# edervishaj/GANMF

Hardware: AMD Instinct MI355X
Metric: GANMF training steps/sec (higher is better)
Workload: dtype f32

## Files before the change

ganmf_amd/csrc/gemm_bf16k.hpp:

```cpp
#pragma once
#include "gemm_bf16s.hpp"

namespace ganmf {

typedef float f32x4k __attribute__((ext_vector_type(4)));

struct SplitItemK {
  const float* zp;
  const float* ptr;
  long long inc;
  long long second;
  int aux, dst;
  int dst1 = 0;
  bool km;
  __device__ inline void init(bool km_, const float* __restrict__ base, int ld_, int r0, int rlimit, int kbeg, const float* zero, int w,
                              const int* __restrict__ gather = nullptr) {
    km = km_;
    const int ld = ld_;
    zp = zero + (w & 255) * 8;
    if (!km) {
      using S = SplitStage<64, 64, false>;
      const int row = w / S::CH, c8 = w % S::CH;
      const bool ok = (r0 + row) < rlimit;
      const int src_row = (ok && gather) ? gather[r0 + row] : r0 + row;
      ptr = ok ? base + (size_t)src_row * ld + kbeg + 8 * c8 : zp;
      inc = ok ? 64 : 0;
      second = 4;
      aux = 0;
      dst = row * 32 + 4 * (c8 ^ S::swz(row));
      dst1 = 0;
    } else {
      using S = SplitStage<64, 64, true>;
      const int kp = w / S::RQ, rq = w % S::RQ;
      const bool ok = (r0 + 4 * rq) < ld;
      ptr = ok ? base + (size_t)(kbeg + 2 * kp) * ld + r0 + 4 * rq : zp;
      inc = ok ? (long long)64 * ld : 0;
      second = ok ? ld : 0;
      aux = 2 * kp;
      dst = (2 * kp) * S::KROW + 4 * ((rq >> 1) ^ S::swzk(2 * kp)) + 2 * (rq & 1);
      dst1 = (2 * kp + 1) * S::KROW + 4 * ((rq >> 1) ^ S::swzk(2 * kp + 1)) + 2 * (rq & 1) - dst;
    }
  }
  __device__ inline void addresses(int kleft, const float*& s0, const float*& s1) {
    const float* const z = zp;
    const float* a0 = ptr;
    const float* a1 = ptr + second;
    const int k0 = aux;
    ptr += inc;
    if (kleft < 64 && km) {
      asm volatile("; partial last K-tile");
      a0 = k0 < kleft ? a0 : z;
      a1 = k0 + 1 < kleft ? a1 : z;
    }
    s0 = a0; s1 = a1;
  }
  template <int NPIECE, bool F16>
  __device__ inline void split(const f32x4k (&v)[2], u32x4 (&pc)[3], const int tok, const float scale) const {
    const f32x4k a = v[0], b = v[1];
    if constexpr (NPIECE == 3) {
      unsigned h, m, l;
      split_bf16x3_tok(a.x, a.y, h, m, l, tok); pc[0][0] = h; pc[1][0] = m; pc[2][0] = l;
      split_bf16x3_tok(a.z, a.w, h, m, l, tok); pc[0][1] = h; pc[1][1] = m; pc[2][1] = l;
      split_bf16x3_tok(b.x, b.y, h, m, l, tok); pc[0][2] = h; pc[1][2] = m; pc[2][2] = l;
      split_bf16x3_tok(b.z, b.w, h, m, l, tok); pc[0][3] = h; pc[1][3] = m; pc[2][3] = l;
    } else if constexpr (F16) {
      const float sc = __uint_as_float(__float_as_uint(scale) | (unsigned)tok);
      pc[0][0] = cvt_pk_f16(a.x * sc, a.y * sc); pc[0][1] = cvt_pk_f16(a.z * sc, a.w * sc);
      pc[0][2] = cvt_pk_f16(b.x * sc, b.y * sc); pc[0][3] = cvt_pk_f16(b.z * sc, b.w * sc);
    } else {
      pc[0][0] = cvt_pk_bf16_tok(a.x, a.y, tok); pc[0][1] = cvt_pk_bf16_tok(a.z, a.w, tok);
      pc[0][2] = cvt_pk_bf16_tok(b.x, b.y, tok); pc[0][3] = cvt_pk_bf16_tok(b.z, b.w, tok);
    }
  }
};

constexpr int BF16K_OPER = 3 * (64 * 64 / 2) * 2;
template <int NPIECE> constexpr int bf16k_oper() { return NPIECE * (64 * 64 / 2) * 2; }
template <int NPIECE> constexpr int bf16k_smem_dw() { return 2 * bf16k_oper<NPIECE>() > 4 * 64 * 64 ? 2 * bf16k_oper<NPIECE>() : 4 * 64 * 64; }
static_assert(bf16k_oper<3>() == BF16K_OPER && bf16k_smem_dw<3>() == 2 * BF16K_OPER && bf16k_smem_dw<1>() == 4 * 64 * 64, "plane buffers");
template <int NPIECE> constexpr int bf16k_pd() { return 2; }

__device__ __forceinline__ int bf16k_wait_vm(int n, const f32x4k& v0, const f32x4k& v1) {
  int tok;
#define GANMF_BF16K_WAIT(N) asm volatile("s_waitcnt vmcnt(" #N ")\n\ts_mov_b32 %0, 0" : "=s"(tok) : "v"(v0), "v"(v1))
  if (n >= 8) { if (n >= 9) GANMF_BF16K_WAIT(9); else GANMF_BF16K_WAIT(8); }
  else if (n >= 4) { if (n >= 6) { if (n >= 7) GANMF_BF16K_WAIT(7); else GANMF_BF16K_WAIT(6); } else { if (n >= 5) GANMF_BF16K_WAIT(5); else GANMF_BF16K_WAIT(4); } }
  else { if (n >= 2) { if (n >= 3) GANMF_BF16K_WAIT(3); else GANMF_BF16K_WAIT(2); } else { if (n >= 1) GANMF_BF16K_WAIT(1); else GANMF_BF16K_WAIT(0); } }
#undef GANMF_BF16K_WAIT
  return tok;
}

template <bool AKM, bool BKM, int NPIECE, bool F16, int EXTRA, class Entry>
__device__ __forceinline__ void bf16k_mainloop(const GemmP& p, const int tm, const int tn, const int sp, const int bz, float* __restrict__ smem,
                                               f32x16& acc_out, Entry&& at_entry) {
  static_assert(NPIECE == 3 || NPIECE == 1, "pieces per operand");
  static_assert(!F16 || NPIECE == 1, "fp16 pieces only in the single-piece mode");
  static_assert(2 * (bf16k_pd<NPIECE>() - 1) + EXTRA <= 9, "bf16k_wait_vm covers 0 .. 9");
  constexpr int BM = 64, BN = 64, BK = 64, PD = bf16k_pd<NPIECE>();
  const float sa = (F16 && p.a_scale != 0.f) ? p.a_scale : 1.f, sb = (F16 && p.b_scale != 0.f) ? p.b_scale : 1.f;
  using FA = SplitStage<64, 64, AKM>;
  using FB = SplitStage<64, 64, BKM>;
  const unsigned lds0 = lds_addr(smem);
  const int tid = threadIdx.x;
  const int lane = tid & 63;
  const int wave = __builtin_amdgcn_readfirstlane(tid >> 6);
  const int kg = wave >> 2;
  const int wr = (wave >> 1) & 1, wc = wave & 1;
  const int li = lane & 31, lh = lane >> 5;
  const bool stage_a = wave < 8;
  const int m0 = tm * BM, n0 = tn * BN;
  const int kbeg = sp * p.k_per_split;
  const int kend = min(p.K, kbeg + p.k_per_split);
  const int nt = (kend - kbeg + BK - 1) / BK;

  f32x16 acc, accl;
#pragma unroll
  for (int r = 0; r < 16; ++r) { acc[r] = 0.f; accl[r] = 0.f; }

  SplitItemK it;
  if (stage_a) it.init(AKM, p.A + (size_t)bz * p.a_batch_stride, p.lda, m0, p.M, kbeg, p.zero_page, tid,
                       (AKM || !p.a_gather) ? nullptr : p.a_gather + (size_t)bz * p.a_gather_batch);
  else it.init(BKM, p.B, p.ldb, n0, p.N, kbeg, p.zero_page, tid - 512);
  constexpr int OPER = bf16k_oper<NPIECE>();
  unsigned my_planes[2], my_planes1[2], frag_a[2], frag_b[2];
#pragma unroll
  for (int b = 0; b < 2; ++b) {
    my_planes[b] = lds_base<NPIECE == 3>(lds0 + 4u * (unsigned)(b * OPER + (stage_a ? 0 : NPIECE * FA::PLANE) + it.dst));
    my_planes1[b] = lds_base<NPIECE == 3>(my_planes[b] + 4u * (unsigned)it.dst1);
    frag_a[b] = lds_base<NPIECE == 3>(lds0 + 4u * (unsigned)(b * OPER) + FA::frag_off(wr * 32, kg, li, lh));
    frag_b[b] = lds_base<NPIECE == 3>(lds0 + 4u * (unsigned)(b * OPER + NPIECE * FA::PLANE) + FB::frag_off(wc * 32, kg, li, lh));
  }
  const float my_scale = stage_a ? sa : sb;

  f32x4k rg[PD][2];
#pragma unroll
  for (int s = 0; s < PD; ++s) { rg[s][0] = f32x4k{0.f, 0.f, 0.f, 0.f}; rg[s][1] = f32x4k{0.f, 0.f, 0.f, 0.f}; }
  int kleft = kend - kbeg;
  auto load_tile = [&](auto ss) {
    constexpr int s = decltype(ss)::value;
    const float *s0, *s1;
    it.addresses(kleft, s0, s1);
    f32x4k l0, l1;
    asm volatile("global_load_dwordx4 %0, %1, off" : "=v"(l0) : "v"(s0) : "memory");
    asm volatile("global_load_dwordx4 %0, %1, off" : "=v"(l1) : "v"(s1) : "memory");
    rg[s][0] = l0; rg[s][1] = l1;
    kleft -= BK;
  };
  auto store_tile = [&](auto ss, auto bb, int nwait) {
    constexpr int s = decltype(ss)::value;
    constexpr int b = decltype(bb)::value;
    const f32x4k v[2] = {rg[s][0], rg[s][1]};
    const int tok = bf16k_wait_vm(nwait, v[0], v[1]);
    u32x4 pc[3];
#ifdef GANMF_PERSIST_DIAG_BUILD
    if ((p.diag & 32) && stage_a) {
      pc[0] = __builtin_bit_cast(u32x4, v[0]); pc[1] = __builtin_bit_cast(u32x4, v[1]); pc[2] = pc[0];
      pc[0][0] += (unsigned)tok;
    } else
#endif
    it.template split<NPIECE, F16>(v, pc, tok, my_scale);
    if (it.km) {
      typedef unsigned u32x2 __attribute__((ext_vector_type(2)));
#pragma unroll
      for (int q = 0; q < NPIECE; ++q) {
        lds_write<u32x2>(my_planes[b] + 4u * (unsigned)(q * FA::PLANE), u32x2{pc[q][0], pc[q][1]});
        lds_write<u32x2>(my_planes1[b] + 4u * (unsigned)(q * FA::PLANE), u32x2{pc[q][2], pc[q][3]});
      }
    } else {
#pragma unroll
      for (int q = 0; q < NPIECE; ++q) lds_write<u32x4>(my_planes[b] + 4u * (unsigned)(q * FA::PLANE), pc[q]);
    }
  };
  static_for<0, PD>([&](auto ss) { if (decltype(ss)::value < nt) load_tile(ss); });
  store_tile(std::integral_constant<int, 0>{}, std::integral_constant<int, 0>{}, 2 * (min(nt, PD) - 1));
  if constexpr (PD == 4) asm volatile("s_waitcnt vmcnt(0)" :: "v"(rg[0][0]), "v"(rg[0][1]), "v"(rg[1][0]), "v"(rg[1][1]), "v"(rg[2][0]), "v"(rg[2][1]), "v"(rg[3][0]), "v"(rg[3][1]));
  else asm volatile("s_waitcnt vmcnt(0)" :: "v"(rg[0][0]), "v"(rg[0][1]), "v"(rg[1][0]), "v"(rg[1][1]));
  static_assert(PD == 4 || PD == 2, "the wait above names every prefetch register");
  at_entry();
  __syncthreads();
#ifdef GANMF_PERSIST_DIAG_BUILD
  if (p.stamps && tid == 0) p.stamps[(size_t)blockIdx.x * 4 + 1] = __builtin_amdgcn_s_memrealtime();
#endif

  auto step = [&](auto ss, int t) {
    constexpr int s = decltype(ss)::value, s1 = (s + 1) % PD;
    constexpr int b = s & 1;
    u32x4 pa[3], pb[3];
#pragma unroll
    for (int q = 0; q < NPIECE; ++q) pa[q] = FA::frag_at(frag_a[b] + 4u * (unsigned)(q * FA::PLANE));
#pragma unroll
    for (int q = 0; q < NPIECE; ++q) pb[q] = FB::frag_at(frag_b[b] + 4u * (unsigned)(q * FB::PLANE));
#ifdef GANMF_PERSIST_DIAG_BUILD
    if (p.diag & 16) { if (t + PD < nt) kleft -= BK; } else
#endif
    if (t + PD < nt) load_tile(ss);
    constexpr int ta[6] = {1, 0, 2, 1, 0, 0}, tb[6] = {1, 2, 0, 0, 1, 0};
#ifdef GANMF_PERSIST_DIAG_BUILD
    if (!(p.diag & 4))
#endif
    {
      if constexpr (NPIECE == 3) {
#pragma unroll
        for (int t6 = 0; t6 < 6; ++t6) {
          if (t6 < 5)
            accl = __builtin_amdgcn_mfma_f32_32x32x16_bf16(__builtin_bit_cast(bf16x8, pa[ta[t6]]), __builtin_bit_cast(bf16x8, pb[tb[t6]]), accl, 0, 0, 0);
          else
            acc = __builtin_amdgcn_mfma_f32_32x32x16_bf16(__builtin_bit_cast(bf16x8, pa[ta[t6]]), __builtin_bit_cast(bf16x8, pb[tb[t6]]), acc, 0, 0, 0);
        }
      } else if constexpr (F16) {
        acc = __builtin_amdgcn_mfma_f32_32x32x16_f16(__builtin_bit_cast(f16x8, pa[0]), __builtin_bit_cast(f16x8, pb[0]), acc, 0, 0, 0);
      } else {
        acc = __builtin_amdgcn_mfma_f32_32x32x16_bf16(__builtin_bit_cast(bf16x8, pa[0]), __builtin_bit_cast(bf16x8, pb[0]), acc, 0, 0, 0);
      }
    }
#ifdef GANMF_PERSIST_DIAG_BUILD
    if (!(p.diag & 2))
#endif
    if (t + 1 < nt) store_tile(std::integral_constant<int, s1>{}, std::integral_constant<int, (s1 & 1)>{}, 2 * (min(t + PD, nt - 1) - (t + 1)) + (t + 1 < PD ? EXTRA : 0));
    __syncthreads();
  };
  for (int t = 0; t < nt; t += PD)
    static_for<0, PD>([&](auto ss) { if (t + decltype(ss)::value < nt) step(ss, t + decltype(ss)::value); });

  if constexpr (NPIECE == 3) acc += accl;
  if constexpr (F16) {
    if (sa != 1.f || sb != 1.f) acc *= 1.f / (sa * sb);
  }
  acc_out = acc;
}

template <bool AKM, bool BKM, int NPIECE = 3, bool F16 = false>
__device__ __forceinline__ void gemm_bf16k_body(const GemmP& p, const int bid, const int nblk, float* __restrict__ smem) {
  int tm, tn, sp, bz;
  tile_coords(p, bid, nblk, tm, tn, sp, bz);
  f32x16 acc[1][1];
#ifdef GANMF_PERSIST_DIAG_BUILD
  if (p.stamps && threadIdx.x == 0) p.stamps[(size_t)blockIdx.x * 4 + 0] = __builtin_amdgcn_s_memrealtime();
#endif
  bf16k_mainloop<AKM, BKM, NPIECE, F16, 0>(p, tm, tn, sp, bz, smem, acc[0][0], [] {});
#ifdef GANMF_PERSIST_DIAG_BUILD
  if (p.stamps && threadIdx.x == 0) p.stamps[(size_t)blockIdx.x * 4 + 2] = __builtin_amdgcn_s_memrealtime();
#endif
  static_assert(4 * 64 * 64 <= bf16k_smem_dw<NPIECE>(), "the workgroup's LDS must hold the four staged partial tiles");
  gemm_epilogue<64, 64, 1, 1, 4, AKM && BKM>(p, acc, smem, TileCoord{tm, tn, sp, bz, tm * 64, tn * 64});
#ifdef GANMF_PERSIST_DIAG_BUILD
  if (p.stamps) { asm volatile("s_waitcnt vmcnt(0)" ::: "memory"); __builtin_amdgcn_s_barrier(); if (threadIdx.x == 0) p.stamps[(size_t)blockIdx.x * 4 + 3] = __builtin_amdgcn_s_memrealtime(); }
#endif
}

template <bool AKM, bool BKM, int NPIECE = 3, bool F16 = false>
__global__ __launch_bounds__(1024) void gemm_bf16k_mfma(const GemmP p) {
  __shared__ __attribute__((aligned(16))) float smem[bf16k_smem_dw<NPIECE>()];
  gemm_bf16k_body<AKM, BKM, NPIECE, F16>(p, (int)blockIdx.x, (int)gridDim.x, smem);
}

template <int NPIECE, bool F16>
inline hipError_t gemm_bf16k_launch(hipStream_t st, const GemmP& p0, bool akm, bool bkm) {
  GemmP p = p0;
#ifdef GANMF_PERSIST_DIAG_BUILD
  if (getenv("GANMF_BF16K_DIAG")) p.diag = atoi(getenv("GANMF_BF16K_DIAG"));
#endif
  const int grid = p.tiles_m * p.tiles_n * p.nsplit * p.nbatch;
  if (grid <= 0) return hipSuccess;
#ifdef GANMF_PERSIST_DIAG_BUILD
  const bool stamping = gemm_stamps_on() && gemm_stamps_begin(p, grid, st);
  struct Report { const GemmP& p; int grid; hipStream_t st; bool akm, bkm, on; ~Report() { if (on) gemm_stamps_report(p, grid, st, akm, bkm, NPIECE == 3 ? "gemm_bf16k_mfma (split-bf16, 16 waves)" : "gemm_bf16k_mfma (one piece)"); } } report{p, grid, st, akm, bkm, stamping};
#endif
  {
    if (!akm && !bkm) GANMF_LAUNCH((gemm_bf16k_mfma<false, false, NPIECE, F16>), dim3(grid), dim3(1024), 0, st, p);
    else if (!akm && bkm) GANMF_LAUNCH((gemm_bf16k_mfma<false, true, NPIECE, F16>), dim3(grid), dim3(1024), 0, st, p);
    else if (akm && bkm) GANMF_LAUNCH((gemm_bf16k_mfma<true, true, NPIECE, F16>), dim3(grid), dim3(1024), 0, st, p);
    else return hipErrorInvalidValue;
  }
  return hipGetLastError();
}

}
```

ganmf_amd/csrc/gemm_bf16w.hpp:

```cpp
#pragma once
#include "gemm_bf16k.hpp"

namespace ganmf {

constexpr int BF16W_BM = 64, BF16W_BN = 32, BF16W_BK = 128, BF16W_KG = 8, BF16W_PD = 2;
constexpr int BF16W_PA = BF16W_BM * BF16W_BK / 2;
constexpr int BF16W_PB = BF16W_BN * BF16W_BK / 2;
constexpr int BF16W_OPER = 3 * (BF16W_PA + BF16W_PB);

__device__ __forceinline__ int bf16w_wait_vm(int n, const f32x4k& v0, const f32x4k& v1, const f32x4k& v2) {
  int tok;
#define GANMF_BF16W_WAIT(N) asm volatile("s_waitcnt vmcnt(" #N ")\n\ts_mov_b32 %0, 0" : "=s"(tok) : "v"(v0), "v"(v1), "v"(v2))
  if (n >= 9) GANMF_BF16W_WAIT(9);
  else if (n >= 6) GANMF_BF16W_WAIT(6);
  else if (n >= 3) GANMF_BF16W_WAIT(3);
  else GANMF_BF16W_WAIT(0);
#undef GANMF_BF16W_WAIT
  return tok;
}

template <int NPIECE> constexpr int bf16w_oper() { return NPIECE * (BF16W_PA + BF16W_PB); }
template <int NPIECE> constexpr int bf16w_smem_dw() {
  return 2 * bf16w_oper<NPIECE>() > BF16W_KG * BF16W_BM * BF16W_BN ? 2 * bf16w_oper<NPIECE>() : BF16W_KG * BF16W_BM * BF16W_BN;
}
static_assert(bf16w_oper<3>() == BF16W_OPER && bf16w_smem_dw<3>() == 2 * BF16W_OPER && bf16w_smem_dw<1>() == BF16W_KG * BF16W_BM * BF16W_BN, "plane buffers");

template <bool BKM, int NPIECE = 3, bool F16 = false>
__device__ __forceinline__ void bf16w_mainloop(const GemmP& p, const int tm, const int tn, const int bz, float* __restrict__ smem, f32x16& acc_out) {
  static_assert(NPIECE == 3 || NPIECE == 1, "pieces per operand");
  static_assert(!F16 || NPIECE == 1, "fp16 pieces only in the single-piece mode");
  constexpr int BM = BF16W_BM, BN = BF16W_BN, BK = BF16W_BK, PD = BF16W_PD, PA = BF16W_PA, PB = BF16W_PB, OPER = bf16w_oper<NPIECE>();
  const float sa = (F16 && p.a_scale != 0.f) ? p.a_scale : 1.f, sb = (F16 && p.b_scale != 0.f) ? p.b_scale : 1.f;
  typedef unsigned u32x2 __attribute__((ext_vector_type(2)));
  const unsigned lds0 = lds_addr(smem);
  const int tid = threadIdx.x;
  const int lane = tid & 63;
  const int wave = __builtin_amdgcn_readfirstlane(tid >> 6);
  const int kg = wave >> 1, wr = wave & 1;
  const int li = lane & 31, lh = lane >> 5;
  const int m0 = tm * BM, n0 = tn * BN;
  const int nt = (p.K + BK - 1) / BK;

  f32x16 acc, accl;
#pragma unroll
  for (int r = 0; r < 16; ++r) { acc[r] = 0.f; accl[r] = 0.f; }

  const int row = tid >> 5, kq = tid & 31;
  const int arow = tid >> 4, c8 = tid & 15;
  const float* const zp = p.zero_page + (tid & 255) * 8;
  const bool ok0 = m0 + arow < p.M, ok2 = n0 + row < p.N;
  const float* s0 = ok0 ? p.A + (size_t)bz * p.a_batch_stride + (size_t)(m0 + arow) * p.lda + 8 * c8 : zp;
  const int kb = tid >> 3, nq = tid & 7;
  const bool okn = n0 + 4 * nq < p.ldb;
  const float* s2 = !BKM ? (ok2 ? p.B + (size_t)(n0 + row) * p.ldb + 4 * kq : zp) : (okn ? p.B + (size_t)kb * p.ldb + n0 + 4 * nq : zp);
  const int i0 = ok0 ? BK : 0;
  const long long i2 = !BKM ? (ok2 ? BK : 0) : (okn ? (long long)BK * p.ldb : 0);
  int kleft = p.K;
  const bool in_a = (nt - 1) * BK + 8 * c8 < p.lda, in_b = (nt - 1) * BK + 4 * kq < p.ldb;
  const int dsta = arow * (BK / 2) + ((c8 ^ (arow & 15)) << 2);
  const int dst = row * (BK / 2) + ((((kq >> 1) ^ (row & 15))) << 2) + ((kq & 1) << 1);
  const int dstb = !BKM ? dst : kb * (BN / 2) + 2 * nq;

  f32x4k rg[PD][3];
#pragma unroll
  for (int s = 0; s < PD; ++s) { rg[s][0] = f32x4k{0.f, 0.f, 0.f, 0.f}; rg[s][1] = rg[s][0]; rg[s][2] = rg[s][0]; }
  int tload = 0;
  auto load_tile = [&](auto ss) {
    constexpr int s = decltype(ss)::value;
    const float* const zp_ = zp;
    const float* const s0_ = s0;
    const float* const s2_ = s2;
    const int kleft_ = kleft;
    const float* a0 = s0_;
    const float* b0 = s2_;
    if (tload >= nt - 1) {
      asm volatile("; last K-tile");
      const bool last = tload == nt - 1, past = tload >= nt;
      a0 = ((last && !in_a) || past) ? zp_ : s0_;
      b0 = !BKM ? (((last && !in_b) || past) ? zp_ : s2_) : ((kb < kleft_) ? s2_ : zp_);
    }
    kleft -= BK;
    f32x4k l0, l1, l2;
    asm volatile("global_load_dwordx4 %0, %1, off" : "=v"(l0) : "v"(a0) : "memory");
    asm volatile("global_load_dwordx4 %0, %1, off offset:16" : "=v"(l1) : "v"(a0) : "memory");
    asm volatile("global_load_dwordx4 %0, %1, off" : "=v"(l2) : "v"(b0) : "memory");
    rg[s][0] = l0; rg[s][1] = l1; rg[s][2] = l2;
    s0 += i0; s2 += i2;
    ++tload;
  };
  unsigned st_a[2], st_b[2];
#pragma unroll
  for (int b = 0; b < 2; ++b) {
    st_a[b] = lds_base<NPIECE == 3>(lds0 + 4u * (unsigned)(b * OPER + dsta));
    st_b[b] = lds_base<NPIECE == 3>(lds0 + 4u * (unsigned)(b * OPER + NPIECE * PA + dstb));
  }
  auto store_tile = [&](auto ss, auto bb, int nwait) {
    constexpr int s = decltype(ss)::value;
    constexpr int b = decltype(bb)::value;
    const f32x4k v0 = rg[s][0], v1 = rg[s][1], v2 = rg[s][2];
    const int tok = bf16w_wait_vm(nwait, v0, v1, v2);
    const unsigned o = st_a[b], ob = st_b[b];
    if constexpr (NPIECE == 3) {
      unsigned h0, m0_, l0, h1, m1, l1, h2, m2, l2, h3, m3, l3;
      split_bf16x3_tok(v0.x, v0.y, h0, m0_, l0, tok); split_bf16x3_tok(v0.z, v0.w, h1, m1, l1, tok);
      split_bf16x3_tok(v1.x, v1.y, h2, m2, l2, tok); split_bf16x3_tok(v1.z, v1.w, h3, m3, l3, tok);
      lds_write<u32x4>(o, u32x4{h0, h1, h2, h3});
      lds_write<u32x4>(o + 4u * PA, u32x4{m0_, m1, m2, m3});
      lds_write<u32x4>(o + 8u * PA, u32x4{l0, l1, l2, l3});
      split_bf16x3_tok(v2.x, v2.y, h0, m0_, l0, tok); split_bf16x3_tok(v2.z, v2.w, h1, m1, l1, tok);
      lds_write<u32x2>(ob, u32x2{h0, h1});
      lds_write<u32x2>(ob + 4u * PB, u32x2{m0_, m1});
      lds_write<u32x2>(ob + 8u * PB, u32x2{l0, l1});
    } else if constexpr (F16) {
      const float ca = __uint_as_float(__float_as_uint(sa) | (unsigned)tok), cb = __uint_as_float(__float_as_uint(sb) | (unsigned)tok);
      lds_write<u32x4>(o, u32x4{cvt_pk_f16(v0.x * ca, v0.y * ca), cvt_pk_f16(v0.z * ca, v0.w * ca),
                                cvt_pk_f16(v1.x * ca, v1.y * ca), cvt_pk_f16(v1.z * ca, v1.w * ca)});
      lds_write<u32x2>(ob, u32x2{cvt_pk_f16(v2.x * cb, v2.y * cb), cvt_pk_f16(v2.z * cb, v2.w * cb)});
    } else {
      lds_write<u32x4>(o, u32x4{cvt_pk_bf16_tok(v0.x, v0.y, tok), cvt_pk_bf16_tok(v0.z, v0.w, tok),
                                cvt_pk_bf16_tok(v1.x, v1.y, tok), cvt_pk_bf16_tok(v1.z, v1.w, tok)});
      lds_write<u32x2>(ob, u32x2{cvt_pk_bf16_tok(v2.x, v2.y, tok), cvt_pk_bf16_tok(v2.z, v2.w, tok)});
    }
  };
  static_for<0, PD>([&](auto ss) { load_tile(ss); });
  store_tile(std::integral_constant<int, 0>{}, std::integral_constant<int, 0>{}, 3 * (PD - 1));
  asm volatile("s_waitcnt vmcnt(0)" :: "v"(rg[0][0]), "v"(rg[0][1]), "v"(rg[0][2]), "v"(rg[1][0]), "v"(rg[1][1]), "v"(rg[1][2]));
  static_assert(PD == 2, "the wait above names every prefetch register");
  __syncthreads();
#ifdef GANMF_PERSIST_DIAG_BUILD
  if (p.stamps && tid == 0) p.stamps[(size_t)blockIdx.x * 4 + 1] = __builtin_amdgcn_s_memrealtime();
#endif

  unsigned fa[2], fb[2];
#pragma unroll
  for (int b = 0; b < 2; ++b) {
    fa[b] = lds_base<NPIECE == 3>(lds0 + 4u * (unsigned)(b * OPER + (wr * 32 + li) * (BK / 2) + (((2 * kg + lh) ^ (li & 15)) << 2)));
    if constexpr (!BKM) fb[b] = lds_base<NPIECE == 3>(lds0 + 4u * (unsigned)(b * OPER + NPIECE * PA + li * (BK / 2) + (((2 * kg + lh) ^ (li & 15)) << 2)));
    else fb[b] = 0u;
  }
  unsigned fbt[2];
#pragma unroll
  for (int b = 0; b < 2; ++b)
    fbt[b] = !BKM ? 0u : lds_base<NPIECE == 3>(lds0 + 4u * (unsigned)(b * OPER + NPIECE * PA) + (unsigned)(((16 * kg + 8 * lh + ((li & 15) >> 2)) * (BN / 2) * 4) + 32 * (li >> 4) + 8 * (li & 3)));
  auto step = [&](auto ss, int t) {
    constexpr int s = decltype(ss)::value, s1_ = (s + 1) % PD;
    constexpr int b = s & 1;
    u32x4 pa[3], pb[3];
#pragma unroll
    for (int q = 0; q < NPIECE; ++q) pa[q] = lds_read<u32x4>(fa[b] + 4u * (unsigned)(q * PA));
    if constexpr (!BKM) {
#pragma unroll
      for (int q = 0; q < NPIECE; ++q) pb[q] = lds_read<u32x4>(fb[b] + 4u * (unsigned)(q * PB));
    } else {
#if defined(__HIP_DEVICE_COMPILE__)
      typedef __attribute__((address_space(3))) s16x4* lds_s16x4_p;
      const unsigned base = fbt[b];
#pragma unroll
      for (int q = 0; q < NPIECE; ++q) {
        const s16x4 lo = __builtin_amdgcn_ds_read_tr16_b64_v4i16((lds_s16x4_p)(base + q * PB * 4));
        const s16x4 hi = __builtin_amdgcn_ds_read_tr16_b64_v4i16((lds_s16x4_p)(base + q * PB * 4 + 4 * (BN / 2) * 4));
        pb[q] = __builtin_bit_cast(u32x4, __builtin_shufflevector(lo, hi, 0, 1, 2, 3, 4, 5, 6, 7));
      }
#else
      (void)fbt;
#pragma unroll
      for (int q = 0; q < NPIECE; ++q) pb[q] = u32x4{0u, 0u, 0u, 0u};
#endif
    }
    if (t + PD < nt) load_tile(ss);
    constexpr int ta[6] = {1, 0, 2, 1, 0, 0}, tb[6] = {1, 2, 0, 0, 1, 0};
    if constexpr (NPIECE == 3) {
#pragma unroll
      for (int t6 = 0; t6 < 6; ++t6) {
        if (t6 < 5)
          accl = __builtin_amdgcn_mfma_f32_32x32x16_bf16(__builtin_bit_cast(bf16x8, pa[ta[t6]]), __builtin_bit_cast(bf16x8, pb[tb[t6]]), accl, 0, 0, 0);
        else
          acc = __builtin_amdgcn_mfma_f32_32x32x16_bf16(__builtin_bit_cast(bf16x8, pa[ta[t6]]), __builtin_bit_cast(bf16x8, pb[tb[t6]]), acc, 0, 0, 0);
      }
    } else if constexpr (F16) {
      acc = __builtin_amdgcn_mfma_f32_32x32x16_f16(__builtin_bit_cast(f16x8, pa[0]), __builtin_bit_cast(f16x8, pb[0]), acc, 0, 0, 0);
    } else {
      acc = __builtin_amdgcn_mfma_f32_32x32x16_bf16(__builtin_bit_cast(bf16x8, pa[0]), __builtin_bit_cast(bf16x8, pb[0]), acc, 0, 0, 0);
    }
    if (t + 1 < nt) store_tile(std::integral_constant<int, s1_>{}, std::integral_constant<int, (s1_ & 1)>{}, 3 * (min(t + PD, nt - 1) - (t + 1)));
    __syncthreads();
  };
  for (int t = 0; t < nt; t += PD)
    static_for<0, PD>([&](auto ss) { if (t + decltype(ss)::value < nt) step(ss, t + decltype(ss)::value); });

  if constexpr (NPIECE == 3) acc += accl;
  if constexpr (F16) {
    if (sa != 1.f || sb != 1.f) acc *= 1.f / (sa * sb);
  }
  acc_out = acc;
}

template <bool BKM, int NPIECE = 3, bool F16 = false>
__device__ __forceinline__ void gemm_bf16w_body(const GemmP& p, const int bid, const int nblk, float* __restrict__ smem) {
  int tm, tn, sp, bz;
  tile_coords(p, bid, nblk, tm, tn, sp, bz);
  f32x16 acc[1][1];
#ifdef GANMF_PERSIST_DIAG_BUILD
  if (p.stamps && threadIdx.x == 0) p.stamps[(size_t)blockIdx.x * 4 + 0] = __builtin_amdgcn_s_memrealtime();
#endif
  bf16w_mainloop<BKM, NPIECE, F16>(p, tm, tn, bz, smem, acc[0][0]);
#ifdef GANMF_PERSIST_DIAG_BUILD
  if (p.stamps && threadIdx.x == 0) p.stamps[(size_t)blockIdx.x * 4 + 2] = __builtin_amdgcn_s_memrealtime();
#endif
  static_assert(BF16W_KG * BF16W_BM * BF16W_BN <= bf16w_smem_dw<NPIECE>(), "the workgroup's LDS must hold the staged partial tiles");
  const int lane = threadIdx.x & 63, wave = __builtin_amdgcn_readfirstlane(threadIdx.x >> 6);
  const int kg = wave >> 1, wr = wave & 1, li = lane & 31, lh = lane >> 5;
  float* ct = smem + kg * (BF16W_BM * BF16W_BN);
#pragma unroll
  for (int r = 0; r < 16; ++r) ct[(wr * 32 + (r & 3) + 8 * (r >> 2) + 4 * lh) * BF16W_BN + li] = acc[0][0][r];
  gemm_epilogue<BF16W_BM, BF16W_BN, 1, 1, 4, false, BF16W_KG, true>(p, acc, smem, TileCoord{tm, tn, sp, bz, tm * BF16W_BM, tn * BF16W_BN});
#ifdef GANMF_PERSIST_DIAG_BUILD
  if (p.stamps) { asm volatile("s_waitcnt vmcnt(0)" ::: "memory"); __builtin_amdgcn_s_barrier(); if (threadIdx.x == 0) p.stamps[(size_t)blockIdx.x * 4 + 3] = __builtin_amdgcn_s_memrealtime(); }
#endif
}

template <bool BKM, int NPIECE = 3, bool F16 = false>
__global__ __launch_bounds__(1024) void gemm_bf16w_mfma(const GemmP p) {
  __shared__ __attribute__((aligned(16))) float smem[bf16w_smem_dw<NPIECE>()];
  gemm_bf16w_body<BKM, NPIECE, F16>(p, (int)blockIdx.x, (int)gridDim.x, smem);
}

inline bool gemm_bf16w_eligible(const GemmP& p, bool akm, bool bkm) {
  return !akm && std::max(p.nbatch, 1) == 1 && !p.a_gather && !p.a_planes && !p.b_planes && !p.epi.csr_indptr && !p.epi.sp_rows &&
         p.epi.kind != EPI_ADAM && p.K >= 1 && (p.lda % 64) == 0 && (p.ldb % 64) == 0;
}
constexpr int BF16W_ZERO_PAGE_FLOATS = 255 * 8 + 8;
static_assert(BF16W_ZERO_PAGE_FLOATS <= 2048 + 64, "gemm_bf16w reads past the library's zero page");

inline bool plan_bf16w(GemmPlan& pl, const GemmP& g, bool akm, bool bkm, bool force) {
  if (!gemm_bf16w_eligible(g, akm, bkm)) return false;
  const int tm = (g.M + BF16W_BM - 1) / BF16W_BM, tn = (g.N + BF16W_BN - 1) / BF16W_BN;
  const bool lp = pl.mode == MFMA_F16 || pl.mode == MFMA_BF16;
  const double k64 = lp ? 0.45 : 0.94, k32 = lp ? 0.75 : 1.3;
  if (!force) {
    if (!((pl.mode == MFMA_BF16X3 || lp) && pl.tile == 64 && pl.kg == 4 && pl.nsplit >= 2 && !pl.persist && !pl.skinny && !pl.skinny_n)) return false;
    if ((long long)tm * tn > GEMM_CUS) return false;
    const double est64 = 5.3 + k64 * ((pl.kps + 63) / 64) + 4.7, est32 = 4.4 + k32 * ((g.K + BF16W_BK - 1) / BF16W_BK);
    if (est32 > est64 - 0.5) return false;
  }
  const bool wants_sq = pl.sq_count > 0 || g.epi.sq_partials != nullptr;
  pl.est_us = 4.4 + k32 * ((g.K + BF16W_BK - 1) / BF16W_BK);
  pl.wide32 = 1; pl.skinny = 0; pl.skinny_n = 0; pl.persist = 0;
  if (!lp) pl.mode = MFMA_BF16X3;
  pl.tile = 64; pl.kg = BF16W_KG; pl.ring = 2; pl.bk = BF16W_BK;
  pl.tiles_m = tm; pl.tiles_n = tn; pl.nsplit = 1; pl.kps = g.K;
  pl.sq_count = wants_sq ? tm * tn : 0;
  return true;
}

inline hipError_t gemm_dispatch_bf16w(hipStream_t st, const GemmP& p0, bool bkm, int mode) {
  GemmP p = p0;
  const int grid = p.tiles_m * p.tiles_n * std::max(p.nbatch, 1);
  if (grid <= 0) return hipSuccess;
#ifdef GANMF_PERSIST_DIAG_BUILD
  const bool stamping = gemm_stamps_on() && gemm_stamps_begin(p, grid, st);
  struct Report { const GemmP& p; int grid; hipStream_t st; bool bkm, on; ~Report() { if (on) gemm_stamps_report(p, grid, st, false, bkm, "gemm_bf16w_mfma (64 x 32 tiles, 128-deep K-tiles)"); } } report{p, grid, st, bkm, stamping};
#endif
  if (p.nsplit != 1 || p.tiles_m != (p.M + BF16W_BM - 1) / BF16W_BM || p.tiles_n != (p.N + BF16W_BN - 1) / BF16W_BN) return hipErrorInvalidValue;
  if (!p.zero_page || (p.lda % 64) != 0 || (p.ldb % 64) != 0) return hipErrorInvalidValue;
  if (mode == MFMA_F16) {
    if (bkm) GANMF_LAUNCH((gemm_bf16w_mfma<true, 1, true>), dim3(grid), dim3(1024), 0, st, p);
    else GANMF_LAUNCH((gemm_bf16w_mfma<false, 1, true>), dim3(grid), dim3(1024), 0, st, p);
  } else if (mode == MFMA_BF16) {
    if (bkm) GANMF_LAUNCH((gemm_bf16w_mfma<true, 1, false>), dim3(grid), dim3(1024), 0, st, p);
    else GANMF_LAUNCH((gemm_bf16w_mfma<false, 1, false>), dim3(grid), dim3(1024), 0, st, p);
  } else {
    if (bkm) GANMF_LAUNCH(gemm_bf16w_mfma<true>, dim3(grid), dim3(1024), 0, st, p);
    else GANMF_LAUNCH(gemm_bf16w_mfma<false>, dim3(grid), dim3(1024), 0, st, p);
  }
  return hipGetLastError();
}

}
```

ganmf_amd/csrc/gemm_f32.hpp:

```cpp
#pragma once
#include <hip/hip_runtime.h>
#include <hip/hip_ext.h>

#include <algorithm>
#include <cstdio>
#include <cstdlib>
#include <vector>
#include <cmath>
#include <type_traits>

#include "adam_touch.hpp"

namespace ganmf {

struct LaunchProf { hipEvent_t start = nullptr, stop = nullptr; int count = 0; };
inline LaunchProf& launch_prof() { static thread_local LaunchProf lp; return lp; }
inline hipEvent_t& launch_stop_event() { static thread_local hipEvent_t ev = nullptr; return ev; }
inline long long& launch_count() { static thread_local long long n = 0; return n; }

template <class F, class... Args>
inline void launch_kernel(F kernel, const dim3& grid, const dim3& block, unsigned shmem, hipStream_t st, Args... args) {
  LaunchProf& lp = launch_prof();
  hipEvent_t& stop = launch_stop_event();
  ++launch_count();
  if (lp.start && lp.count++ == 0) hipExtLaunchKernelGGL(kernel, grid, block, shmem, st, lp.start, lp.stop, 0, args...);
  else if (stop) { hipExtLaunchKernelGGL(kernel, grid, block, shmem, st, nullptr, stop, 0, args...); stop = nullptr; }
  else hipLaunchKernelGGL(kernel, grid, block, shmem, st, args...);
}
#define GANMF_LAUNCH(...) ::ganmf::launch_kernel(__VA_ARGS__)

typedef float f32x16 __attribute__((ext_vector_type(16)));
typedef float f32x2 __attribute__((ext_vector_type(2)));
typedef unsigned u32x4 __attribute__((ext_vector_type(4)));
typedef __bf16 bf16x8 __attribute__((ext_vector_type(8)));

enum MfmaMode : int { MFMA_AUTO = -1, MFMA_F32 = 0, MFMA_BF16 = 1, MFMA_F16 = 2, MFMA_BF16X3 = 3 };

typedef __bf16 bf16x2 __attribute__((ext_vector_type(2)));

__device__ inline unsigned cvt_pk_bf16(float x0, float x1) {
  unsigned r;
  asm("v_cvt_pk_bf16_f32 %0, %1, %2" : "=v"(r) : "v"(x0), "v"(x1));
  return r;
}

__device__ inline unsigned cvt_pk_bf16_tok(float x0, float x1, int tok) {
  unsigned r;
  asm("v_cvt_pk_bf16_f32 %0, %1, %2 ; behind wait token %3" : "=v"(r) : "v"(x0), "v"(x1), "s"(tok));
  return r;
}
__device__ inline void split_bf16x3_tok(float x0, float x1, unsigned& hi, unsigned& mid, unsigned& lo, int tok) {
  hi = cvt_pk_bf16_tok(x0, x1, tok);
  float r0 = x0 - __uint_as_float(hi << 16), r1 = x1 - __uint_as_float(hi & 0xffff0000u);
  mid = cvt_pk_bf16(r0, r1);
  r0 -= __uint_as_float(mid << 16);
  r1 -= __uint_as_float(mid & 0xffff0000u);
  lo = cvt_pk_bf16(r0, r1);
}

__device__ inline unsigned cvt_pk_f16(float x0, float x1) {
  unsigned r;
  x0 = __builtin_amdgcn_fmed3f(x0, -65504.f, 65504.f);
  x1 = __builtin_amdgcn_fmed3f(x1, -65504.f, 65504.f);
  asm("v_cvt_pk_f16_f32 %0, %1, %2" : "=v"(r) : "v"(x0), "v"(x1));
  return r;
}

__device__ inline void split_bf16x3(float x0, float x1, unsigned& hi, unsigned& mid, unsigned& lo) {
  hi = cvt_pk_bf16(x0, x1);
  float r0 = x0 - __uint_as_float(hi << 16), r1 = x1 - __uint_as_float(hi & 0xffff0000u);
  mid = cvt_pk_bf16(r0, r1);
  r0 -= __uint_as_float(mid << 16);
  r1 -= __uint_as_float(mid & 0xffff0000u);
  lo = cvt_pk_bf16(r0, r1);
}

template <int I, int N, class F>
__device__ inline void static_for(F&& f) {
  if constexpr (I < N) {
    f(std::integral_constant<int, I>{});
    static_for<I + 1, N>(f);
  }
}

constexpr int LD_ALIGN = 64;

enum GemmEpi : int {
  EPI_STORE = 0,
  EPI_SUB_AUX_SQ = 1,
  EPI_SUB_SCALED_AUX = 2,
  EPI_ROWSCALE = 3,
  EPI_G_DE = 4,
  EPI_ACT = 5,
  EPI_MUL_ACTGRAD = 6,
  EPI_ADAM = 7,
  EPI_GRAM_STATS = 8,
};

constexpr float ADAM_B1 = 0.9f, ADAM_B2 = 0.999f, ADAM_EPS = 1e-8f;

enum ActKind : int { ACT_LINEAR = 0, ACT_TANH = 1, ACT_RELU = 2, ACT_SIGMOID = 3 };

__device__ inline float act_apply(int act, float z) {
  switch (act) {
    case ACT_TANH: return tanhf(z);
    case ACT_RELU: return fmaxf(z, 0.f);
    case ACT_SIGMOID: return 1.f / (1.f + expf(-z));
    default: return z;
  }
}
__device__ inline float act_grad_out(int act, float a) {
  switch (act) {
    case ACT_TANH: return 1.f - a * a;
    case ACT_RELU: return a > 0.f ? 1.f : 0.f;
    case ACT_SIGMOID: return a * (1.f - a);
    default: return 1.f;
  }
}

struct EpiD {
  int kind;
  const float* aux;
  int ldaux;
  long long aux_batch_stride;
  const float* rowscale;
  float c;
  const float* er;
  const float* ef;
  float cfm;
  float* sq_partials;
  int sq_stride;
  int sq_m_half;
  int act;
  const float* r1_u;
  const float* r1_w;
  int r1_ld;
  float* adam_theta;
  float* adam_theta_out;
  float* adam_m;
  float* adam_v;
  const float* adam_alpha;
  float adam_reg;
  const long long* csr_indptr;
  const int* csr_indices;
  const float* csr_data;
  const int* csr_rows;
  const float* sp_rows;
  int sp_ld, sp_bias_row, sp_bias_parts;
  unsigned short* planes;
  long long plane_stride;
  double* gram_partials;
};

__device__ inline float4 csr_quad(const EpiD& e, int m, int col) {
  const int r = e.csr_rows[m];
  long long lo = e.csr_indptr[r];
  const long long en = e.csr_indptr[r + 1];
  long long hi = en;
  while (lo < hi) {
    const long long mid = (lo + hi) >> 1;
    if (e.csr_indices[mid] < col) lo = mid + 1; else hi = mid;
  }
  float4 x = make_float4(0.f, 0.f, 0.f, 0.f);
  for (long long j = lo; j < en; ++j) {
    const int c = e.csr_indices[j] - col;
    if (c > 3) break;
    const float v = e.csr_data[j];
    if (c == 0) x.x = v; else if (c == 1) x.y = v; else if (c == 2) x.z = v; else x.w = v;
  }
  return x;
}

__device__ inline float4 sparse_rows_quad(const EpiD& e, int row, int col) {
  if (row > e.sp_bias_row) return make_float4(0.f, 0.f, 0.f, 0.f);
  float4 s = *reinterpret_cast<const float4*>(e.sp_rows + (size_t)row * e.sp_ld + col);
  if (row == e.sp_bias_row)
    for (int q = 1; q < e.sp_bias_parts; ++q) {
      const float4 d = *reinterpret_cast<const float4*>(e.sp_rows + (size_t)(row + q) * e.sp_ld + col);
      s.x += d.x; s.y += d.y; s.z += d.z; s.w += d.w;
    }
  return s;
}

__device__ __forceinline__ float adam_step(float x, float ma, float v) {
#ifdef GANMF_ADAM_IEEE
  return x - ma / (sqrtf(v) + ADAM_EPS);
#else
  return __builtin_fmaf(-ma, __builtin_amdgcn_rcpf(__builtin_amdgcn_sqrtf(v) + ADAM_EPS), x);
#endif
}

__device__ inline void adam_update(float g, float alpha, float reg, float& th, float& m, float& v, float& sq) {
  const float x = th;
  sq += x * x;
  const float gr = g + reg * x;
  m += (gr - m) * (1.f - ADAM_B1);
  v += (gr * gr - v) * (1.f - ADAM_B2);
  th = adam_step(x, m * alpha, v);
}

__device__ inline float epi_apply(const EpiD& e, float v, int row, int col, int ldc, const float* __restrict__ aux,
                                  float& sq) {
  switch (e.kind) {
    case EPI_SUB_AUX_SQ:
      if (aux) v -= aux[(size_t)row * e.ldaux + col];
      sq += v * v;
      break;
    case EPI_SUB_SCALED_AUX:
      v -= e.c * aux[(size_t)row * e.ldaux + col];
      break;
    case EPI_ROWSCALE:
      v *= e.rowscale[row];
      break;
    case EPI_G_DE: {
      const float d = e.ef[(size_t)row * ldc + col] - e.er[(size_t)row * ldc + col];
      v = e.c * v + e.cfm * d;
      sq += d * d;
      break;
    }
    case EPI_ACT:
      if (e.r1_u) v += e.r1_u[(size_t)row * e.r1_ld] * e.r1_w[col];
      v = act_apply(e.act, v);
      break;
    case EPI_MUL_ACTGRAD:
      v *= act_grad_out(e.act, aux[(size_t)row * e.ldaux + col]);
      break;
    default: break;
  }
  return v;
}

struct GemmP {
  const float* A;
  const float* B;
  float* C;
  int lda, ldb, ldc;
  int M, N, K;
  const float* zero_page;
  int nsplit;
  int k_per_split;
  long long c_split_stride;
  int nbatch;
  long long a_batch_stride, c_batch_stride;
  EpiD epi;
  int tiles_m, tiles_n;
  unsigned* counters;
  float* Cf;
  long long cf_batch_stride;
  int c_pad_writable;
  const int* a_gather;
  int a_gather_batch;
  float a_scale, b_scale;
  int xb_m, xb_n, xb_band;
  int diag;
  unsigned long long* stamps;
  const unsigned short* a_planes;
  const unsigned short* b_planes;
  long long a_pstride, b_pstride;
  int n_fastest;
  int adam_touch;
};

#define GANMF_WAIT_VMCNT(N) asm volatile("s_waitcnt vmcnt(%0)" ::"n"(N) : "memory")

template <int BM, int BN, int NTHR>
struct AdamTouchRegs {
  static constexpr int NR = (adam_touch_slots(BM, BN) + NTHR - 1) / NTHR;
  float v[NR];
};

template <int BM, int BN, int NTHR>
__device__ __forceinline__ void adam_touch_issue(const GemmP& p, int m0, int n0, int tid, AdamTouchRegs<BM, BN, NTHR>& k) {
#pragma unroll
  for (int j = 0; j < AdamTouchRegs<BM, BN, NTHR>::NR; ++j) {
    k.v[j] = 0.f;
    const AdamTouch t = adam_touch_slot(BM, BN, j * NTHR + tid, m0, n0, p.M, p.N, p.ldc);
    if (t.arr >= 0) {
      const float* __restrict__ b = t.arr == 0 ? p.epi.adam_theta : t.arr == 1 ? p.epi.adam_m : p.epi.adam_v;
      k.v[j] = b[t.off];
    }
  }
}

template <int BM, int BN, int NTHR>
__device__ __forceinline__ void adam_touch_keep(const AdamTouchRegs<BM, BN, NTHR>& k) {
#pragma unroll
  for (int j = 0; j < AdamTouchRegs<BM, BN, NTHR>::NR; ++j) asm volatile("" ::"v"(k.v[j]));
}

template <int R, int BK, bool KM, int NTHR = 256>
struct Stage {
  static constexpr int F4 = R * BK / 4;
  static constexpr int NP = F4 / NTHR;
  static constexpr int SZ = R * BK;
  static constexpr int S = BK / 4;
  static constexpr int RC4 = R / 4;
  static_assert(F4 % NTHR == 0 && NP >= 1, "tile too small for the workgroup");
  static_assert(BK == 32 || BK == 64, "BK must be 32 or 64");

  __device__ static inline int swz(int row) { return (row / (64 / BK)) & (S - 1); }

  const float* zp;
  const float* ptr[NP];
  int aux[NP];

  __device__ inline void init(const float* __restrict__ base, int ld, int r0, int rlimit, int kbeg,
                              const float* zero, int tid, const int* __restrict__ gather = nullptr) {
    zero += (tid & 255) * 4;
    zp = zero;
#pragma unroll
    for (int j = 0; j < NP; ++j) {
      const int pos = j * NTHR + tid;
      if constexpr (!KM) {
        const int row = pos / S, slot = pos % S;
        const int c4 = slot ^ swz(row);
        const bool ok = (r0 + row) < rlimit;
        const int src_row = (ok && gather) ? gather[r0 + row] : r0 + row;
        ptr[j] = ok ? base + (size_t)src_row * ld + kbeg + 4 * c4 : zero;
        aux[j] = ok ? BK : 0;
      } else {
        const int krow = pos / RC4, c4 = pos % RC4;
        const bool ok = (r0 + 4 * c4) < ld;
        ptr[j] = base + (size_t)(kbeg + krow) * ld + r0 + 4 * c4;
        aux[j] = ok ? krow : -1;
      }
    }
  }

  template <int J>
  __device__ inline void issue_piece(float* s, int ld, int kleft, int wave) {
    const float* src;
    if constexpr (!KM) {
      src = kleft > 0 ? ptr[J] : zp;
      ptr[J] += aux[J];
    } else {
      src = (aux[J] >= 0 && aux[J] < kleft) ? ptr[J] : zp;
      ptr[J] += (size_t)BK * ld;
    }
    __builtin_amdgcn_global_load_lds((const __attribute__((address_space(1))) void*)src,
                                     (__attribute__((address_space(3))) void*)(s + (J * NTHR + wave * 64) * 4),
                                     16, 0, 0);
  }
  template <int J>
  __device__ inline void issue_piece_asm(float* s, int ld, int kleft, int wave) {
    const float* src;
    if constexpr (!KM) {
      src = kleft > 0 ? ptr[J] : zp;
      ptr[J] += aux[J];
    } else {
      src = (aux[J] >= 0 && aux[J] < kleft) ? ptr[J] : zp;
      ptr[J] += (size_t)BK * ld;
    }
    const unsigned dst = __builtin_amdgcn_readfirstlane(
        (unsigned)(size_t)(__attribute__((address_space(3))) void*)(s + (J * NTHR + wave * 64) * 4));
    unsigned keep;
    asm volatile("s_mov_b32 %0, m0\n\ts_mov_b32 m0, %2\n\ts_nop 0\n\tglobal_load_lds_dwordx4 %1, off\n\ts_mov_b32 m0, %0"
                 : "=&s"(keep) : "v"(src), "s"(dst) : "memory");
  }
  template <int J0, int J1>
  __device__ inline void issue_range_asm(float* s, int ld, int kleft, int wave) {
    if constexpr (J0 < J1) {
      issue_piece_asm<J0>(s, ld, kleft, wave);
      issue_range_asm<J0 + 1, J1>(s, ld, kleft, wave);
    }
  }
  template <int J0, int J1>
  __device__ inline void issue_range(float* s, int ld, int kleft, int wave) {
    if constexpr (J0 < J1) {
      issue_piece<J0>(s, ld, kleft, wave);
      issue_range<J0 + 1, J1>(s, ld, kleft, wave);
    }
  }
  __device__ inline void issue(float* s, int ld, int kleft, int wave) {
    issue_range<0, NP>(s, ld, kleft, wave);
  }

  __device__ static inline float4 frag(const float* __restrict__ s, int rb, int c, int i, int h) {
    if constexpr (!KM) {
      return *reinterpret_cast<const float4*>(s + (rb + i) * BK + 4 * ((2 * c + h) ^ swz(i)));
    } else {
      const float* q = s + (c * 8 + 4 * h) * R + rb + i;
      return make_float4(q[0], q[R], q[2 * R], q[3 * R]);
    }
  }
};

__device__ inline void tile_coords(const GemmP& p, int bid, int nblk, int& tm, int& tn, int& sp, int& bz) {
  tile_order(TileGrid{p.tiles_m, p.tiles_n, p.nsplit, p.xb_m, p.xb_n, p.xb_band, p.n_fastest}, bid, nblk, tm, tn, sp, bz);
}

#ifndef GANMF_ADAM_HOIST
#define GANMF_ADAM_HOIST 1
#endif

struct TileCoord { int tm, tn, sp, bz, m0, n0; };

__device__ inline void gram_tile_coords(const GemmP& p, int bid, int nblk, int& tm, int& tn);
template <int BM, int BN, int TM, int TN>
__device__ inline void gram_epilogue(const GemmP& p, const f32x16 (&acc)[TM][TN], float* smem, const TileCoord& tc_);
template <int BM, int BN, int TM, int TN>
__device__ inline void rowsq_epilogue(const GemmP& p, const f32x16 (&acc)[TM][TN], float* smem, const TileCoord& tc_);

template <int BM, int BN, int TM, int TN, int KG = 1, bool ADAM_OK = true, int NIMG = KG, bool STAGED = false>
__device__ inline void gemm_epilogue(const GemmP& p, const f32x16 (&acc)[TM][TN], float* smem, const TileCoord& tc_) {
  constexpr int WM = BM / 2, WN = BN / 2;
  constexpr int NTHR = 256 * KG;
  const int tid = threadIdx.x, lane = tid & 63;
  const int wave = __builtin_amdgcn_readfirstlane(tid >> 6);
  const int kg = wave >> 2;
  const int wr = (wave >> 1) & 1, wc = wave & 1;
  const int li = lane & 31, lh = lane >> 5;
  const int tm = tc_.tm, tn = tc_.tn, sp = tc_.sp, bz = tc_.bz, m0 = tc_.m0, n0 = tc_.n0;
  float* __restrict__ ct = smem + kg * (BM * BN);
  const bool deferred = p.nsplit > 1;
  const EpiD& e = p.epi;
  const bool csr0 = e.csr_indptr != nullptr && bz == 0 && e.kind == EPI_SUB_AUX_SQ;
  const float* __restrict__ aux = (e.aux && !csr0) ? e.aux + (size_t)bz * e.aux_batch_stride : nullptr;
  constexpr int C4 = BN / 4, RPP = NTHR / C4 < BM ? NTHR / C4 : BM;
  constexpr bool SPARE = NTHR / C4 > BM;
  static_assert(BM % RPP == 0, "row pass must cover the tile in whole steps");
  static_assert(!SPARE || !ADAM_OK, "the hoisted Adam streams assume every thread owns a row");
  const int tc = tid % C4, tr = tid / C4;
  const int col = n0 + tc * 4;
  float4 auxv = make_float4(0.f, 0.f, 0.f, 0.f);
  bool aux_pre = false;
  if constexpr (BM == RPP) {
    const int row = m0 + tr;
    if (!deferred && aux && (e.kind == EPI_SUB_AUX_SQ || e.kind == EPI_SUB_SCALED_AUX || e.kind == EPI_MUL_ACTGRAD) && row < p.M && col + 3 < p.N &&
        (!SPARE || tr < BM)) {
      auxv = *reinterpret_cast<const float4*>(aux + (size_t)row * e.ldaux + col);
      aux_pre = true;
    }
  }
  if constexpr (!STAGED) {
#pragma unroll
    for (int a = 0; a < TM; ++a)
#pragma unroll
      for (int b = 0; b < TN; ++b)
#pragma unroll
        for (int r = 0; r < 16; ++r)
          ct[(wr * WM + a * 32 + (r & 3) + 8 * (r >> 2) + 4 * lh) * BN + wc * WN + b * 32 + li] = acc[a][b][r];
  }
  __syncthreads();

  float* __restrict__ C = p.C + (size_t)sp * p.c_split_stride + (size_t)bz * p.c_batch_stride;
  const bool sp_add = !(p.nsplit > 1) && e.sp_rows != nullptr;
  float sq = 0.f;
  ct = smem;
  const bool adam = ADAM_OK && !deferred && e.kind == EPI_ADAM;
  const float alpha = adam ? *e.adam_alpha : 0.f;
  float* __restrict__ theta_out = e.adam_theta_out ? e.adam_theta_out : e.adam_theta;
#ifdef GANMF_PERSIST_DIAG_BUILD
  const bool inlaunch = deferred && p.counters != nullptr;
#else
  constexpr bool inlaunch = false;
#endif
  const bool publish = inlaunch;
  typedef unsigned u32x4 __attribute__((ext_vector_type(4)));
  const __amdgpu_buffer_rsrc_t slab_rsrc = __builtin_amdgcn_make_buffer_rsrc((void*)C, (short)0, 0x7fffffff, 0x00020000);
#ifdef GANMF_PERSIST_DIAG_BUILD
  if (adam && (p.diag & 8)) return;
#endif
  if (adam && GANMF_ADAM_HOIST) {
    constexpr int J = BM / RPP, JC = 1;
    static_assert(J % JC == 0, "row steps in whole chunks");
    for (int j0 = 0; j0 < J; j0 += JC) {
      float4 t4[JC], m4[JC], v4[JC];
#pragma unroll
      for (int jj = 0; jj < JC; ++jj) {
        const int row = m0 + tr + (j0 + jj) * RPP;
        if (row < p.M && col + 3 < p.N) {
          const size_t off = (size_t)row * p.ldc + col;
          t4[jj] = *reinterpret_cast<const float4*>(e.adam_theta + off);
          m4[jj] = *reinterpret_cast<const float4*>(e.adam_m + off);
          v4[jj] = *reinterpret_cast<const float4*>(e.adam_v + off);
        }
      }
#pragma unroll
      for (int jj = 0; jj < JC; ++jj) {
        const int row_l = tr + (j0 + jj) * RPP, row = m0 + row_l;
        if (row < p.M && col < p.N) {
          float4 v = *reinterpret_cast<const float4*>(ct + row_l * BN + tc * 4);
#pragma unroll
          for (int g = 1; g < NIMG; ++g) {
            const float4 w = *reinterpret_cast<const float4*>(ct + g * (BM * BN) + row_l * BN + tc * 4);
            v.x += w.x; v.y += w.y; v.z += w.z; v.w += w.w;
          }
          if (sp_add) {
            const float4 x = sparse_rows_quad(e, row, col);
            v.x += x.x; v.y += x.y; v.z += x.z; v.w += x.w;
          }
          const size_t off = (size_t)row * p.ldc + col;
          if (col + 3 < p.N) {
            adam_update(v.x, alpha, e.adam_reg, t4[jj].x, m4[jj].x, v4[jj].x, sq);
            adam_update(v.y, alpha, e.adam_reg, t4[jj].y, m4[jj].y, v4[jj].y, sq);
            adam_update(v.z, alpha, e.adam_reg, t4[jj].z, m4[jj].z, v4[jj].z, sq);
            adam_update(v.w, alpha, e.adam_reg, t4[jj].w, m4[jj].w, v4[jj].w, sq);
            *reinterpret_cast<float4*>(theta_out + off) = t4[jj];
            *reinterpret_cast<float4*>(e.adam_m + off) = m4[jj];
            *reinterpret_cast<float4*>(e.adam_v + off) = v4[jj];
          } else {
            const float o[4] = {v.x, v.y, v.z, v.w};
            for (int q = 0; q < 4 && col + q < p.N; ++q) {
              float th = e.adam_theta[off + q];
              adam_update(o[q], alpha, e.adam_reg, th, e.adam_m[off + q], e.adam_v[off + q], sq);
              theta_out[off + q] = th;
            }
          }
        }
      }
    }
  } else
#pragma unroll 4
  for (int j = 0; j < BM / RPP; ++j) {
    const int row_l = tr + j * RPP, row = m0 + row_l;
    if (row < p.M && col < p.N && (!SPARE || row_l < BM)) {
      float4 v = *reinterpret_cast<const float4*>(ct + row_l * BN + tc * 4);
#pragma unroll
      for (int g = 1; g < NIMG; ++g) {
        const float4 w = *reinterpret_cast<const float4*>(ct + g * (BM * BN) + row_l * BN + tc * 4);
        v.x += w.x; v.y += w.y; v.z += w.z; v.w += w.w;
      }
      if (sp_add) {
        const float4 x = sparse_rows_quad(e, row, col);
        v.x += x.x; v.y += x.y; v.z += x.z; v.w += x.w;
      }
      if (csr0 && !deferred) {
        const float4 x = csr_quad(e, row, col);
        v.x -= x.x; v.y -= x.y; v.z -= x.z; v.w -= x.w;
      }
      float o[4] = {v.x, v.y, v.z, v.w};
      if (adam) {
        const size_t off = (size_t)row * p.ldc + col;
        if (col + 3 < p.N) {
          float4 t4 = *reinterpret_cast<float4*>(e.adam_theta + off);
          float4 m4 = *reinterpret_cast<float4*>(e.adam_m + off);
          float4 v4 = *reinterpret_cast<float4*>(e.adam_v + off);
          adam_update(o[0], alpha, e.adam_reg, t4.x, m4.x, v4.x, sq);
          adam_update(o[1], alpha, e.adam_reg, t4.y, m4.y, v4.y, sq);
          adam_update(o[2], alpha, e.adam_reg, t4.z, m4.z, v4.z, sq);
          adam_update(o[3], alpha, e.adam_reg, t4.w, m4.w, v4.w, sq);
          *reinterpret_cast<float4*>(theta_out + off) = t4;
          *reinterpret_cast<float4*>(e.adam_m + off) = m4;
          *reinterpret_cast<float4*>(e.adam_v + off) = v4;
        } else {
          for (int q = 0; q < 4 && col + q < p.N; ++q) {
            float th = e.adam_theta[off + q];
            adam_update(o[q], alpha, e.adam_reg, th, e.adam_m[off + q], e.adam_v[off + q], sq);
            theta_out[off + q] = th;
          }
        }
        continue;
      }
      if (publish) {
        const int boff = (int)(((size_t)row * p.ldc + col) * sizeof(float));
        if (col + 3 < p.N) {
          u32x4 bits;
          bits[0] = __float_as_uint(o[0]); bits[1] = __float_as_uint(o[1]);
          bits[2] = __float_as_uint(o[2]); bits[3] = __float_as_uint(o[3]);
          __builtin_amdgcn_raw_buffer_store_b128(bits, slab_rsrc, boff, 0, 16 );
        } else {
// ... 625 lines not shown
```

ganmf_amd/csrc/lib/abi_core.inc:

```

int ganmf_abi_version(void) { return GANMF_ABI_VERSION; }
const char* ganmf_last_error(void) { return g_err.c_str(); }

static uint32_t g_crc_tab[8][256];
static std::once_flag g_crc_once;
static void crc_init() {
  for (uint32_t i = 0; i < 256; ++i) {
    uint32_t c = i;
    for (int k = 0; k < 8; ++k) c = (c & 1) ? (c >> 1) ^ 0x82F63B78u : c >> 1;
    g_crc_tab[0][i] = c;
  }
  for (uint32_t i = 0; i < 256; ++i)
    for (int t = 1; t < 8; ++t) g_crc_tab[t][i] = (g_crc_tab[t - 1][i] >> 8) ^ g_crc_tab[0][g_crc_tab[t - 1][i] & 0xff];
}
uint32_t ganmf_crc32c(uint32_t crc, const void* data, uint64_t n) {
  std::call_once(g_crc_once, crc_init);
  const uint8_t* p = static_cast<const uint8_t*>(data);
  uint32_t c = ~crc;
  while (n >= 8) {
    uint64_t w;
    memcpy(&w, p, 8);
    w ^= c;
    c = g_crc_tab[7][w & 0xff] ^ g_crc_tab[6][(w >> 8) & 0xff] ^ g_crc_tab[5][(w >> 16) & 0xff] ^
        g_crc_tab[4][(w >> 24) & 0xff] ^ g_crc_tab[3][(w >> 32) & 0xff] ^ g_crc_tab[2][(w >> 40) & 0xff] ^
        g_crc_tab[1][(w >> 48) & 0xff] ^ g_crc_tab[0][(w >> 56) & 0xff];
    p += 8; n -= 8;
  }
  while (n--) c = (c >> 8) ^ g_crc_tab[0][(c ^ *p++) & 0xff];
  return ~c;
}

int ganmf_device_count(void) {
  int n = 0;
  if (hipGetDeviceCount(&n) != hipSuccess) return 0;
  return n;
}

static int create_impl(const ganmf_cfg* cfg, ganmf_handle* h);

int ganmf_create(const ganmf_cfg* cfg, ganmf_handle** out) {
  if (!cfg || !out) return fail(-1, "ganmf_create: null argument");
  if (cfg->abi_version != GANMF_ABI_VERSION) return fail(-1, "ganmf_create: ABI version %d != %d", cfg->abi_version, GANMF_ABI_VERSION);
  if (cfg->model != GANMF_MODEL_GANMF && cfg->model != GANMF_MODEL_DISGANMF && cfg->model != GANMF_MODEL_MF && cfg->model != GANMF_MODEL_ITEMSIM && cfg->model != GANMF_MODEL_CFGAN && cfg->model != GANMF_MODEL_CAAE) return fail(-1, "ganmf_create: unknown model %d", cfg->model);
  if (cfg->model == GANMF_MODEL_DISGANMF && (cfg->d_layers < 1 || cfg->d_layers > 16 || cfg->d_act < 0 || cfg->d_act > 3))
    return fail(-1, "ganmf_create: DisGANMF needs 1 <= d_layers <= 16 and a known activation");
  if (cfg->model == GANMF_MODEL_CFGAN) {
    if (cfg->d_layers < 1 || cfg->d_layers > 16 || cfg->d_act < 0 || cfg->d_act > 3)
      return fail(-1, "ganmf_create: CFGAN needs 1 <= d_layers <= 16 and a known activation");
    if (cfg->world_size > 1) return fail(-1, "ganmf_create: GANMF_MODEL_CFGAN is single-GPU (world_size %d)", cfg->world_size);
    if (cfg->flags & (GANMF_FLAG_MFMA_BF16 | GANMF_FLAG_MFMA_F16))
      return fail(-1, "ganmf_create: GANMF_MODEL_CFGAN runs the fp32-accurate products only (the bf16 / fp16 MFMA flags are refused)");
    if (cfg->num_items > (1LL << 29)) return fail(-1, "ganmf_create: CFGAN's discriminator input is 2 x num_items wide: dimension too large");
  }
  if (cfg->model == GANMF_MODEL_CAAE) {
    if (cfg->world_size > 1) return fail(-1, "ganmf_create: GANMF_MODEL_CAAE is single-GPU (world_size %d)", cfg->world_size);
    if (cfg->flags & (GANMF_FLAG_MFMA_BF16 | GANMF_FLAG_MFMA_F16))
      return fail(-1, "ganmf_create: GANMF_MODEL_CAAE runs the fp32-accurate products only (the bf16 / fp16 MFMA flags are refused)");
    if (cfg->num_factors > GANMF_CAAE_MAX_FACTORS) return fail(-1, "ganmf_create: GANMF_MODEL_CAAE holds at most %d factors", GANMF_CAAE_MAX_FACTORS);
  }
  if (cfg->num_users < 1 || cfg->num_items < 1 || cfg->num_factors < 1 || cfg->emb_dim < 1 || cfg->batch_size < 1)
    return fail(-1, "ganmf_create: non-positive dimension");
  if (cfg->num_users > (1LL << 30) || cfg->num_items > (1LL << 30)) return fail(-1, "ganmf_create: dimension too large");
  int ndev = 0;
  HIP_TRY(hipGetDeviceCount(&ndev));
  if (ndev < 1) return fail(-2, "ganmf_create: no HIP device (the HIP path is the only path; there is no CPU fallback)");
  if (cfg->device < 0 || cfg->device >= ndev) return fail(-1, "ganmf_create: device %d out of range [0,%d)", cfg->device, ndev);
  HIP_TRY(hipSetDevice(cfg->device));
  ganmf_handle* h = new ganmf_handle();
  const int rc = create_impl(cfg, h);
  if (rc != 0) {
    const std::string msg = g_err;
    ganmf_destroy(h);
    (void)hipGetLastError();
    g_err = msg;
    *out = nullptr;
    return rc;
  }
  *out = h;
  return 0;
}

static int create_impl(const ganmf_cfg* cfg, ganmf_handle* h) {
  h->cfg = *cfg;
  h->dev = cfg->device;
  h->U = (int)cfg->num_users; h->N = (int)cfg->num_items; h->k = cfg->num_factors; h->e = cfg->emb_dim;
  h->B = (int)std::min<int64_t>(cfg->batch_size, cfg->num_users);
  h->ldN = round_up(h->N + 2, LD_ALIGN); h->ldk = round_up(h->k + 1, LD_ALIGN); h->lde = round_up(h->e + 1, LD_ALIGN);
  h->tune.tile = tune_env_int("tile", 0);
  if (h->tune.tile != 0 && h->tune.tile != 64 && h->tune.tile != 128) h->tune.tile = 0;
  h->tune.ring = tune_env_int("ring", 0);
  if (h->tune.ring != 0 && h->tune.ring != 2 && h->tune.ring != 3 && h->tune.ring != 4) h->tune.ring = 0;
  h->tune.nsplit = std::max(0, tune_env_int("nsplit", 0));
  h->tune.mode = env_mfma_mode((cfg->flags & GANMF_FLAG_MFMA_F16) ? MFMA_F16 : (cfg->flags & GANMF_FLAG_MFMA_BF16) ? MFMA_BF16 : (cfg->flags & GANMF_FLAG_MFMA_F32) ? MFMA_F32 : MFMA_DEFAULT);
  h->tune.persist = tune_env_int("persist", -1);
  if (h->tune.persist > 1) h->tune.persist = experiment_int("GANMF_PERSIST_WAVES", 1);
  h->tune.kg = tune_env_int("kg", 0);
  h->tune.tile_order = tune_env_int("tile_order", 0);
  h->pass_stage = tune_env_int("pass_stage", 1) != 0;
  h->skinny = tune_env_int("skinny", 1) != 0;
  h->skinny_n = h->skinny && tune_env_int("skinny_n", 1) != 0;
  h->lazy_rows = tune_env_int("lazy_rows", 1) != 0;
#ifdef GANMF_ASM_PREFETCH_UNTESTED
  constexpr int kAsmPrefetchDefault = 0;
#else
  constexpr int kAsmPrefetchDefault = 1;
#endif
  h->bf16w = tune_env_int("bf16w", kAsmPrefetchDefault);
  h->wgrad_xb = std::max(0, tune_env_int("wgrad_xb", 16));
  h->wd_lane = std::max(0, tune_env_int("wd_lane", 0));
  h->g_rows_staged = std::max(0, std::min(2, tune_env_int("g_rows_staged", 1)));
  h->pair_kg = tune_env_int("pair_kg", 4) == 1 ? 1 : 4;
  h->wgrad_seam = tune_env_int("wgrad_seam", 0);
  h->adam_touch = tune_env_int("adam_touch", 1) != 0 ? 1 : 0;
  h->gram_arith = tune_env_int("gram", 1) == 0 ? 0 : 1;
  HIP_TRY(hipMalloc((void**)&h->seam_cnt, 2 * sizeof(unsigned long long)));
  HIP_TRY(hipMemset(h->seam_cnt, 0, 2 * sizeof(unsigned long long)));
  if (h->tune.kg != 0 && h->tune.kg != 1 && h->tune.kg != 2 && h->tune.kg != 4) h->tune.kg = 0;
  h->debug_plan = env_int("GANMF_DEBUG_PLAN", 0) != 0;
  h->fused_mode = experiment_int("GANMF_FUSED_X3", 1) ? MFMA_BF16X3 : MFMA_F32;
  h->fused_tile = experiment_int("GANMF_FUSED_TILE", 64) == 128 ? 128 : 64;
  h->fused_bk = experiment_int("GANMF_FUSED_BK", 32);
  HIP_TRY(hipStreamCreateWithFlags(&h->st, hipStreamNonBlocking));
  HIP_TRY(hipStreamCreateWithFlags(&h->st2, hipStreamNonBlocking));
  const bool lane_fence = env_int("GANMF_LANE_EVENT_FENCE", cfg->world_size > 1 ? 1 : 0) != 0;
  const unsigned lane_flags = lane_fence ? hipEventDisableTiming : (hipEventDisableTiming | hipEventDisableSystemFence);
  HIP_TRY(hipEventCreateWithFlags(&h->ev_fork, lane_flags));
  HIP_TRY(hipEventCreateWithFlags(&h->ev_join, lane_flags));
  HIP_TRY(hipEventCreateWithFlags(&h->ev_mid, lane_flags));
  HIP_TRY(hipEventCreateWithFlags(&h->ev_we, lane_flags));
  HIP_TRY(hipEventCreateWithFlags(&h->ev_wd, lane_flags));
  h->fuse_adam = experiment_int("GANMF_FUSE_ADAM", 1) != 0;
  const int multi_env = env_int("GANMF_MULTI", 127);
  h->multi = multi_env & 31;
  h->defer_gub = (multi_env & 32) != 0;
  h->dis_fuse_hidden = (multi_env & 64) != 0;
  h->x3kg = env_int("GANMF_X3KG", kAsmPrefetchDefault ? 7 : 0);
  h->dcoef_spread = experiment_int("GANMF_DCOEF_SPREAD", 1) != 0;
  h->pair_ring = experiment_int("GANMF_PAIR_RING", 2) == 3 ? 3 : 2;
  h->inkernel_reduce = experiment_int("GANMF_INKERNEL_REDUCE", 0) != 0;
  h->inlaunch_max = experiment_int("GANMF_INLAUNCH_MAX", 4);
  h->inlaunch_tags = experiment_int("GANMF_INLAUNCH_TAGS", 0);
  h->force_coll = env_int("GANMF_FORCE_COLLECTIVES", 0) != 0;
  h->score_presplit = env_int("GANMF_SCORE_PRESPLIT", 1) != 0;
  h->fork_attach = experiment_int("GANMF_FORK_ATTACH", 1) != 0;
  h->adam_nfast = experiment_int("GANMF_ADAM_NFAST", 3);
  h->red_elems = experiment_int("GANMF_RED_ELEMS", 0);
  h->merge_decode = experiment_int("GANMF_MERGE_DECODE", 1) != 0;
  TRY(dalloc((float**)&h->counters, COUNTER_CAP));
  TRY(dalloc((float**)&h->counters2, COUNTER_CAP));
  const int U = h->U, N = h->N, k = h->k, e = h->e, B = h->B;
  const bool dis = cfg->model == GANMF_MODEL_DISGANMF;
  const bool sim = cfg->model == GANMF_MODEL_ITEMSIM;
  const bool cfgan = cfg->model == GANMF_MODEL_CFGAN;
  const bool caae = cfg->model == GANMF_MODEL_CAAE;
  const bool mf = cfg->model == GANMF_MODEL_MF || sim || caae;
  if (caae && low_precision(h)) return fail(-1, "ganmf_create: GANMF_MODEL_CAAE runs the fp32-accurate products only (GANMF_MFMA asks for bf16 / f16)");
  const int world = std::max(1, (int)cfg->world_size);
  if (!sim && !cfgan) {
    TRY(alloc_tensor(h->Ue, U, k, false, 1));
    TRY(alloc_tensor(h->V, N, k, true, world));
    TRY(dalloc(&h->V_alt, h->V.cap));
  }
  if (mf) {
  } else if (cfgan) {
    TRY(cfgan_create(h));
  } else if (!dis) {
    TRY(alloc_tensor(h->We, N + 1, e, false, world));
    TRY(alloc_tensor(h->Wd, e + 1, N, false, world, h->ldN));
    h->gD_elems = h->We.cap + h->Wd.cap;
    TRY(dalloc(&h->gD, h->gD_elems));
    h->We.g = h->gD;
    h->Wd.g = h->We.g + h->We.cap;
  } else {
    h->L = cfg->d_layers; h->act = cfg->d_act;
    h->Wl.resize(h->L);
    h->dis_fused.assign(h->L, 0);
    h->dis_regn.assign(h->L, ADAM_GRID);
    h->gD_elems = 0;
    for (int l = 0; l < h->L; ++l) {
      TRY(alloc_tensor(h->Wl[l], l == 0 ? N + 2 : e + 1, e, false, world));
      h->gD_elems += h->Wl[l].cap;
    }
    TRY(alloc_tensor(h->Wo, 1, e + 1, false, world));
    h->gD_elems += h->Wo.cap;
    TRY(dalloc(&h->gD, h->gD_elems));
    float* gp = h->gD;
    for (int l = 0; l < h->L; ++l) { h->Wl[l].g = gp; gp += h->Wl[l].cap; }
    h->Wo.g = gp;
  }
  TRY(dalloc(&h->zero_page, 2048 + 64));
  TRY(dalloc((float**)&h->perm, (size_t)3 * U));
  h->pos = h->perm + U;
  h->pos_step = h->perm + 2 * (size_t)U;
  if (!mf && !cfgan) {
    TRY(dalloc(&h->XF, (size_t)2 * B * h->ldN));
    h->XF_own = h->XF;
    TRY(dalloc(&h->Ub, (size_t)B * h->ldk));
    h->Ub_own = h->Ub;
    TRY(dalloc(&h->dF, (size_t)B * h->ldN));
    TRY(dalloc(&h->gUb, (size_t)B * h->ldk));
    h->gUb_own = h->gUb;
    std::vector<float> ones((size_t)2 * B, 1.0f);
    HIP_TRY(hipMemcpy2D(h->XF + N, (size_t)h->ldN * 4, ones.data(), 4, 4, (size_t)2 * B, hipMemcpyHostToDevice));
    if (!dis) {
      TRY(dalloc(&h->E, (size_t)2 * B * h->lde));
      TRY(dalloc(&h->Es, (size_t)2 * B * h->lde));
      TRY(dalloc(&h->Dl, (size_t)2 * B * h->ldN));
      TRY(dalloc(&h->dE, (size_t)2 * B * h->lde));
      HIP_TRY(hipMemcpy2D(h->E + e, (size_t)h->lde * 4, ones.data(), 4, 4, (size_t)2 * B, hipMemcpyHostToDevice));
#ifdef GANMF_PERSIST_DIAG_BUILD
      h->wgrad_stream = env_int("GANMF_WGRAD_STREAM", 0) != 0;
#endif
      if (h->wgrad_stream) {
        h->ps_N = (long long)2 * B * h->ldN; h->ps_e = (long long)2 * B * h->lde;
        TRY(dalloc((float**)&h->pl_XF, (size_t)(3 * h->ps_N + 1) / 2));
        TRY(dalloc((float**)&h->pl_Dl, (size_t)(3 * h->ps_N + 1) / 2));
        TRY(dalloc((float**)&h->pl_Es, (size_t)(3 * h->ps_e + 1) / 2));
        TRY(dalloc((float**)&h->pl_dE, (size_t)(3 * h->ps_e + 1) / 2));
        TRY(dalloc(&h->wgs_dump, 2048 + 64));
      }
    } else {
      h->Al.resize(h->L, nullptr);
      for (int l = 0; l < h->L; ++l) {
        TRY(dalloc(&h->Al[l], (size_t)2 * B * h->lde));
        HIP_TRY(hipMemcpy2D(h->Al[l] + e, (size_t)h->lde * 4, ones.data(), 4, 4, (size_t)2 * B, hipMemcpyHostToDevice));
      }
      TRY(dalloc(&h->dz0, (size_t)2 * B * h->lde));
      TRY(dalloc(&h->dz1, (size_t)2 * B * h->lde));
      TRY(dalloc(&h->dlogit, (size_t)2 * B));
    }
  }
  TRY(dalloc(&h->rs, (size_t)2 * B));
  h->tab_cap = (int)(U / std::max(B, 1)) + 2;
  TRY(dalloc(&h->scal, (size_t)S_TAB + 4 * (size_t)h->tab_cap));
  TRY(dalloc(&h->sqp, (size_t)2 * std::max(GEMM_RED_GRID, ((B + 63) / 64) * ((N + 63) / 64)) + 16));
  {
    auto t64 = [](int a, int b) { return ((a + 63) / 64) * ((b + 63) / 64); };
    h->reg_cap = std::max({ADAM_GRID, (int)GEMM_RED_GRID, t64(N + 2, e), t64(e + 1, N), t64(N, k), t64(B, N), t64(B, e)});
    h->reg_cap = round_up(h->reg_cap + (e + 63) / 64, 64);
    h->dis_cap = round_up(std::max({h->reg_cap, B, dis_dz_top_blocks(e) + 1}), 64);
  }
  const float pw[4] = {ADAM_B1, ADAM_B2, ADAM_B1, ADAM_B2};
  HIP_TRY(hipMemcpy(h->scal, pw, sizeof pw, hipMemcpyHostToDevice));
  HIP_TRY(hipDeviceSynchronize());
  return 0;
}

int ganmf_destroy(ganmf_handle* h) {
  if (!h) return 0;
  hipSetDevice(h->dev);
  if (h->st) hipStreamSynchronize(h->st);
  if (h->has_comm && !h->local && !h->comm_aborted) ncclCommDestroy(h->comm);
  if (h->local) {
    std::lock_guard<std::mutex> lk(h->local->mu);
    h->local->failed = true;
    h->local->cv.notify_all();
  }
  free_tensor(h->We, false); free_tensor(h->Wd, false); hipFree(h->zero_page); hipFree(h->Es); hipFree(h->seam_cnt);
  for (auto& t : h->Wl) free_tensor(t, false);
  free_tensor(h->Wo, false);
  for (float* a : h->Al) hipFree(a);
  hipFree(h->dz0); hipFree(h->dz1); hipFree(h->dlogit);
  free_tensor(h->Ue, false); free_tensor(h->V, true); hipFree(h->V_alt);
  hipFree(h->gD); hipFree(h->indptr); hipFree(h->indices); hipFree(h->data); hipFree(h->perm);
  hipFree(h->csc_colptr); hipFree(h->csc_rowidx); hipFree(h->csc_val); hipFree(h->sp_rows);
  if (h->stage_i) hipHostFree(h->stage_i);
  if (h->stage_f) hipHostFree(h->stage_f);
  hipFree(h->test_indptr); hipFree(h->test_indices); hipFree(h->test_gain); hipFree(h->eval_buf);
  hipFree(h->cand_indptr); hipFree(h->cand_indices);
  hipFree(h->test_rating); hipFree(h->eval_w); hipFree(h->eval_rmse); hipFree(h->eval_counts); hipFree(h->eval_grp);
  hipFree(h->XF_own); hipFree(h->XF_pass); hipFree(h->Ub_pass); hipFree(h->Ub_own); hipFree(h->Ub_sched); hipFree(h->lazy_tab);
  for (auto& ch : h->lazy_chunks) hipFree(ch.first);
  if (h->lazy_stage) hipHostFree(h->lazy_stage);
  h->lazy_chunks.clear();
  hipFree(h->E); hipFree(h->Dl); hipFree(h->dE); hipFree(h->dF); hipFree(h->gUb_own);
  hipFree(h->slab); hipFree(h->rs); hipFree(h->scal); hipFree(h->sqp);
  hipFree(h->seen_indptr); hipFree(h->seen_indices); hipFree(h->item_mask); hipFree(h->topk_items); hipFree(h->topk_vals); hipFree(h->sc_ids);
  hipFree(h->colbuf); hipFree(h->parts_all); hipFree(h->sc_rows); hipFree(h->sc_out); hipFree(h->sc_pa); hipFree(h->sc_pb);
  hipFree(h->sim_mat); hipFree(h->sim_pool); hipFree(h->sim_part); hipFree(h->sim_zero);
  hipFree(h->rank_mask); hipFree(h->div_mat);
  for (AlsSide& s : h->als) { hipFree(s.indptr); hipFree(s.indices); hipFree(s.conf); }
  hipFree(h->als_G); hipFree(h->als_bad);
  hipFree(h->knn_indptr); hipFree(h->knn_nbr); hipFree(h->knn_val); hipFree(h->knn_dense);
  hipFree(h->slim.S); hipFree(h->slim.st0); hipFree(h->slim.st1); hipFree(h->slim.indptr); hipFree(h->slim.items); hipFree(h->slim.eligible);
  hipFree(h->svd_P[0]); hipFree(h->svd_P[1]); hipFree(h->svd_G); hipFree(h->svd_X); hipFree(h->svd_Wl);
  hipFree(h->svd_lam); hipFree(h->svd_flag);
  hipFree(h->dr_ids); hipFree(h->dr_X); hipFree(h->dr_Ub); hipFree(h->dr_E); hipFree(h->dr_A); hipFree(h->dr_part); hipFree(h->dr_val);
  cfgan_free(h);
  caae_free(h);
  for (auto& r : h->recs) { hipEventDestroy(r.a); hipEventDestroy(r.b); }
  if (h->st2) hipStreamSynchronize(h->st2);
  if (h->ev_fork) hipEventDestroy(h->ev_fork);
  if (h->ev_join) hipEventDestroy(h->ev_join);
  if (h->ev_mid) hipEventDestroy(h->ev_mid);
  if (h->ev_t0) hipEventDestroy(h->ev_t0);
  if (h->ev_t1) hipEventDestroy(h->ev_t1);
  if (h->ev_we) hipEventDestroy(h->ev_we);
  if (h->ev_wd) hipEventDestroy(h->ev_wd);
  if (h->st2) hipStreamDestroy(h->st2);
  if (h->st) hipStreamDestroy(h->st);
  hipFree(h->slab2); hipFree(h->counters); hipFree(h->counters2);
  hipFree(h->pl_XF); hipFree(h->pl_Dl); hipFree(h->pl_Es); hipFree(h->pl_dE); hipFree(h->wgs_dump); hipFree(h->wgs_table);
  delete h;
  return 0;
}

int ganmf_comm_unique_id(uint8_t out128[128]) {
  static_assert(sizeof(ncclUniqueId) == 128, "ncclUniqueId is expected to be 128 bytes");
  ncclUniqueId id;
  NCCL_TRY(ncclGetUniqueId(&id));
  memcpy(out128, &id, 128);
  return 0;
}

int ganmf_comm_init_local(ganmf_handle* h, int32_t group_id) {
  if (!h) return fail(-1, "null handle");
  TRY(not_cfgan(h, "ganmf_comm_init_local"));
  if (h->has_comm) return fail(-1, "ganmf_comm_init_local: handle already has a communicator");
  const int world = h->cfg.world_size, rank = h->cfg.rank;
  if (world < 1 || world > LOCAL_MAX_WORLD || rank < 0 || rank >= world)
    return fail(-1, "ganmf_comm_init_local: world_size %d / rank %d out of range (max %d)", world, rank, LOCAL_MAX_WORLD);
  std::lock_guard<std::mutex> lk(g_local_mu);
  std::shared_ptr<LocalGroup>& slot = g_local_groups[group_id];
  if (!slot || slot->joined == slot->world || slot->failed) {
    slot = std::make_shared<LocalGroup>();
    slot->world = world; slot->dev = h->dev;
  }
  if (slot->world != world || slot->dev != h->dev)
    return fail(-1, "ganmf_comm_init_local: group %d is for world_size %d on device %d", group_id, slot->world, slot->dev);
  ++slot->joined;
  h->local = slot;
  h->has_comm = true;
  return 0;
}

int ganmf_comm_init(ganmf_handle* h, const uint8_t id128[128]) {
  if (!h) return fail(-1, "null handle");
  TRY(not_cfgan(h, "ganmf_comm_init"));
  HIP_TRY(hipSetDevice(h->dev));
  ncclUniqueId id;
  memcpy(&id, id128, 128);
  NCCL_TRY(ncclCommInitRank(&h->comm, h->cfg.world_size, id, h->cfg.rank));
  h->has_comm = true;
  return 0;
}

int ganmf_comm_info(ganmf_handle* h, int32_t* world_size, int32_t* rank) {
  if (!h || !world_size || !rank) return fail(-1, "ganmf_comm_info: null argument");
  *world_size = 0; *rank = -1;
  if (!h->has_comm) return 0;
  if (h->local) { *world_size = h->local->world; *rank = h->cfg.rank; return 0; }
  int n = 0, r = -1;
  std::lock_guard<std::mutex> comm_lk(h->comm_mu);
  if (h->comm_aborted.load(std::memory_order_acquire)) return fail(-3, "ganmf_comm_info: communicator aborted (ganmf_comm_abort)");
  NCCL_TRY(ncclCommCount(h->comm, &n));
  NCCL_TRY(ncclCommUserRank(h->comm, &r));
  *world_size = n; *rank = r;
  return 0;
}

int ganmf_comm_abort(ganmf_handle* h) {
  if (!h) return fail(-1, "ganmf_comm_abort: null handle");
  if (!h->has_comm) return 0;
  if (h->local) {
    std::lock_guard<std::mutex> lk(h->local->mu);
    h->local->failed = true;
    h->local->cv.notify_all();
    return 0;
  }
  if (!h->comm_aborted.exchange(true, std::memory_order_acq_rel)) {
    std::lock_guard<std::mutex> comm_lk(h->comm_mu);
    NCCL_TRY(ncclCommAbort(h->comm));
  }
  return 0;
}

int ganmf_set_urm_csr(ganmf_handle* h, const int64_t* indptr, const int32_t* indices, const float* data,
                      int64_t n_rows, int64_t n_cols) {
  if (!h || !indptr || ((!indices || !data) && indptr[n_rows] > 0)) return fail(-1, "ganmf_set_urm_csr: null argument");
  if (n_rows != h->U || n_cols != h->N) return fail(-1, "ganmf_set_urm_csr: shape %lldx%lld != handle %dx%d", (long long)n_rows, (long long)n_cols, h->U, h->N);
  int64_t nnz = indptr[n_rows];
  if (indptr[0] != 0 || nnz < 0) return fail(-1, "ganmf_set_urm_csr: bad indptr");
  for (int64_t r = 0; r < n_rows; ++r)
    if (indptr[r + 1] < indptr[r]) return fail(-1, "ganmf_set_urm_csr: indptr not monotone at row %lld", (long long)r);
  for (int64_t j = 0; j < nnz; ++j)
    if (indices[j] < 0 || indices[j] >= n_cols) return fail(-1, "ganmf_set_urm_csr: column index %d out of range at %lld", indices[j], (long long)j);
  std::vector<int64_t> c_indptr;
  std::vector<int> c_indices;
  std::vector<float> c_data;
  bool canonical = true;
  for (int64_t r = 0; r < n_rows && canonical; ++r)
    for (int64_t j = indptr[r] + 1; j < indptr[r + 1]; ++j)
      if (indices[j] <= indices[j - 1]) { canonical = false; break; }
  if (!canonical) {
    c_indptr.assign((size_t)n_rows + 1, 0);
    c_indices.reserve((size_t)nnz);
    c_data.reserve((size_t)nnz);
    std::vector<int64_t> order;
    for (int64_t r = 0; r < n_rows; ++r) {
      order.resize((size_t)(indptr[r + 1] - indptr[r]));
      for (size_t i = 0; i < order.size(); ++i) order[i] = indptr[r] + (int64_t)i;
      std::stable_sort(order.begin(), order.end(), [&](int64_t a, int64_t b) { return indices[a] < indices[b]; });
      for (size_t i = 0; i < order.size(); ++i) {
        const int64_t j = order[i];
        if (i > 0 && indices[j] == c_indices.back()) c_data.back() += data[j];
        else { c_indices.push_back(indices[j]); c_data.push_back(data[j]); }
      }
      c_indptr[(size_t)r + 1] = (int64_t)c_indices.size();
    }
    indptr = c_indptr.data();
    indices = c_indices.data();
    data = c_data.data();
    nnz = (int64_t)c_indices.size();
  }
  HIP_TRY(hipSetDevice(h->dev));
  if (h->indptr) { hipFree(h->indptr); hipFree(h->indices); hipFree(h->data); h->indptr = nullptr; }
  HIP_TRY(hipMalloc((void**)&h->indptr, (n_rows + 1) * sizeof(long long)));
  HIP_TRY(hipMalloc((void**)&h->indices, std::max<int64_t>(nnz, 1) * sizeof(int)));
  HIP_TRY(hipMalloc((void**)&h->data, std::max<int64_t>(nnz, 1) * sizeof(float)));
  HIP_TRY(hipMemcpy(h->indptr, indptr, (n_rows + 1) * sizeof(long long), hipMemcpyHostToDevice));
  if (nnz) {
    HIP_TRY(hipMemcpy(h->indices, indices, nnz * sizeof(int), hipMemcpyHostToDevice));
    HIP_TRY(hipMemcpy(h->data, data, nnz * sizeof(float), hipMemcpyHostToDevice));
  }
  h->nnz = nnz;
  h->has_urm = true;
  h->ca.iu_src = nullptr;
  const double density = (double)nnz / ((double)n_rows * (double)n_cols);
  const int force = env_int("GANMF_SPARSE", -1);
  h->sparse_g = h->cfg.model == GANMF_MODEL_GANMF && (force >= 0 ? force != 0 : density < 0.005);
  const int force_d = env_int("GANMF_SPARSE_D", -1);
  const double flops_saved = 4.0 * (double)h->B * (double)h->N * (double)h->e;
  h->sparse_d = h->cfg.model == GANMF_MODEL_GANMF && force != 0 &&
                (force_d >= 0 ? force_d != 0 : (density < 0.005 && flops_saved >= 2.0e9));
  if (h->debug_plan)
    fprintf(stderr, "[ganmf urm] set_urm_csr %lldx%lld nnz=%lld%s density %.5f -> sparse_g %d sparse_d %d\n", (long long)n_rows,
            (long long)n_cols, (long long)nnz, canonical ? "" : " (made canonical)", density, (int)h->sparse_g, (int)h->sparse_d);
  hipFree(h->csc_colptr); hipFree(h->csc_rowidx); hipFree(h->csc_val);
  h->csc_colptr = nullptr; h->csc_rowidx = nullptr; h->csc_val = nullptr;
  if (h->sparse_d) {
    std::vector<long long> colptr((size_t)n_cols + 1, 0);
    for (int64_t j = 0; j < nnz; ++j) ++colptr[(size_t)indices[j] + 1];
    for (int64_t c = 0; c < n_cols; ++c) colptr[c + 1] += colptr[c];
    std::vector<long long> fill(colptr.begin(), colptr.end() - 1);
    std::vector<int> rowidx((size_t)std::max<int64_t>(nnz, 1));
    std::vector<float> val((size_t)std::max<int64_t>(nnz, 1));
    for (int64_t r = 0; r < n_rows; ++r)
      for (int64_t j = indptr[r]; j < indptr[r + 1]; ++j) {
        const long long at = fill[indices[j]]++;
        rowidx[at] = (int)r; val[at] = data[j];
      }
    HIP_TRY(hipMalloc((void**)&h->csc_colptr, (size_t)(n_cols + 1) * sizeof(long long)));
    HIP_TRY(hipMalloc((void**)&h->csc_rowidx, rowidx.size() * sizeof(int)));
    HIP_TRY(hipMalloc((void**)&h->csc_val, val.size() * sizeof(float)));
    HIP_TRY(hipMemcpy(h->csc_colptr, colptr.data(), (size_t)(n_cols + 1) * sizeof(long long), hipMemcpyHostToDevice));
    HIP_TRY(hipMemcpy(h->csc_rowidx, rowidx.data(), rowidx.size() * sizeof(int), hipMemcpyHostToDevice));
    HIP_TRY(hipMemcpy(h->csc_val, val.data(), val.size() * sizeof(float), hipMemcpyHostToDevice));
    if (!h->sp_rows) TRY(dalloc(&h->sp_rows, (size_t)(h->N + CSC_BIAS_PARTS) * h->lde));
  }
  return 0;
}

int ganmf_tensor_shape(ganmf_handle* h, int tensor_id, int64_t* rows, int64_t* cols) {
  View v;
  if (h) TRY(needs_tensors(h, "ganmf_tensor_shape"));
  if (!h || !find_view(h, tensor_id, &v)) return fail(-1, "unknown tensor id %d", tensor_id);
  if (rows) *rows = v.rows;
  if (cols) *cols = v.cols;
  return 0;
}

static int copy_view(ganmf_handle* h, int tensor_id, int slot, float* host, int64_t n, bool to_device, const char* who) {
  View v;
  if (h) TRY(needs_tensors(h, who));
  if (!h || !host || !find_view(h, tensor_id, &v)) return fail(-1, "%s: unknown tensor id %d", who, tensor_id);
  if (n != (int64_t)v.rows * v.cols) return fail(-1, "%s: tensor %d has %lld elements, got %lld", who, tensor_id, (long long)v.rows * v.cols, (long long)n);
  if ((slot == GANMF_SLOT_ADAM_M || slot == GANMF_SLOT_ADAM_V) && h->has_comm && h->cfg.world_size > 1 && tensor_id != GANMF_T_USER_EMB)
    return fail(-1, "%s: the Adam moments of replicated tensor %d are sharded over the %d ranks of a data-parallel run "
                    "(each rank holds its slice only); only user_embeddings' moments are whole on their rank", who, tensor_id, h->cfg.world_size);
  HIP_TRY(hipSetDevice(h->dev));
  HIP_TRY(hipStreamSynchronize(h->st));
  for (int i = 0; i < v.nseg; ++i) {
    const Seg& sg = v.seg[i];
    float* d = slot_ptr(sg.t, slot);
    if (!d) return fail(-1, "%s: bad slot %d", who, slot);
    d += (size_t)sg.row0 * sg.t->ld + sg.col0;
    float* hp = host + (size_t)sg.host_row0 * v.cols;
    const size_t hpitch = (size_t)sg.cols * 4, dpitch = (size_t)sg.t->ld * 4;
    if (to_device) HIP_TRY(hipMemcpy2D(d, dpitch, hp, hpitch, (size_t)sg.cols * 4, sg.rows, hipMemcpyHostToDevice));
    else HIP_TRY(hipMemcpy2D(hp, hpitch, d, dpitch, (size_t)sg.cols * 4, sg.rows, hipMemcpyDeviceToHost));
  }
  return 0;
}

int ganmf_set_tensor(ganmf_handle* h, int tensor_id, int slot, const float* host, int64_t n) {
  if (h) ++h->param_version;
  return copy_view(h, tensor_id, slot, const_cast<float*>(host), n, true, "ganmf_set_tensor");
}

int ganmf_get_tensor(ganmf_handle* h, int tensor_id, int slot, float* host, int64_t n) {
  return copy_view(h, tensor_id, slot, host, n, false, "ganmf_get_tensor");
}

int ganmf_get_adam_powers(ganmf_handle* h, float out4[4]) {
  if (!h) return fail(-1, "null handle");
  HIP_TRY(hipSetDevice(h->dev));
  HIP_TRY(hipStreamSynchronize(h->st));
  HIP_TRY(hipMemcpy(out4, h->scal, 4 * sizeof(float), hipMemcpyDeviceToHost));
  return 0;
}

int ganmf_set_adam_powers(ganmf_handle* h, const float in4[4]) {
  if (!h) return fail(-1, "null handle");
  HIP_TRY(hipSetDevice(h->dev));
  HIP_TRY(hipStreamSynchronize(h->st));
  HIP_TRY(hipMemcpy(h->scal, in4, 4 * sizeof(float), hipMemcpyHostToDevice));
  return 0;
}
```

ganmf_amd/csrc/lib/abi_misc.inc:

```
int ganmf_snapshot_best(ganmf_handle* h) {
  if (!h) return fail(-1, "null handle");
  TRY(needs_tensors(h, "ganmf_snapshot_best"));
  HIP_TRY(hipSetDevice(h->dev));
  for (Tensor* t : all_tensors(h))
    HIP_TRY(hipMemcpyAsync(t->best, t->p, t->padded() * sizeof(float), hipMemcpyDeviceToDevice, h->st));
  HIP_TRY(hipStreamSynchronize(h->st));
  return 0;
}

int ganmf_restore_best(ganmf_handle* h) {
  if (!h) return fail(-1, "null handle");
  TRY(needs_tensors(h, "ganmf_restore_best"));
  HIP_TRY(hipSetDevice(h->dev));
  ++h->param_version;
  for (Tensor* t : all_tensors(h))
    HIP_TRY(hipMemcpyAsync(t->p, t->best, t->padded() * sizeof(float), hipMemcpyDeviceToDevice, h->st));
  HIP_TRY(hipStreamSynchronize(h->st));
  return 0;
}

int ganmf_stream_timer(ganmf_handle* h, int stop, double* ms) {
  if (!h) return fail(-1, "null handle");
  HIP_TRY(hipSetDevice(h->dev));
  if (!h->ev_t0) { HIP_TRY(hipEventCreate(&h->ev_t0)); HIP_TRY(hipEventCreate(&h->ev_t1)); }
  if (!stop) { HIP_TRY(hipEventRecord(h->ev_t0, h->st)); return 0; }
  if (!ms) return fail(-1, "ganmf_stream_timer: null result pointer");
  HIP_TRY(hipEventRecord(h->ev_t1, h->st));
  HIP_TRY(hipEventSynchronize(h->ev_t1));
  float f = 0.f;
  HIP_TRY(hipEventElapsedTime(&f, h->ev_t0, h->ev_t1));
  *ms = (double)f;
  return 0;
}

int ganmf_profile_enable(ganmf_handle* h, int on) {
  if (!h) return fail(-1, "null handle");
  HIP_TRY(hipSetDevice(h->dev));
  HIP_TRY(hipStreamSynchronize(h->st));
  for (auto& r : h->recs) { hipEventDestroy(r.a); hipEventDestroy(r.b); }
  h->recs.clear();
  h->prof = on != 0;
  return 0;
}

int ganmf_profile_read(ganmf_handle* h, ganmf_prof_entry* out, int32_t cap, int32_t* n_out) {
  if (!h || !out || !n_out) return fail(-1, "null argument");
  HIP_TRY(hipSetDevice(h->dev));
  HIP_TRY(hipStreamSynchronize(h->st));
  std::vector<ganmf_prof_entry> acc(T_COUNT);
  for (int i = 0; i < T_COUNT; ++i) {
    memset(&acc[i], 0, sizeof acc[i]);
    snprintf(acc[i].name, sizeof acc[i].name, "%s", kTagName[i]);
  }
  for (auto& r : h->recs) {
    float ms = 0.f;
    if (hipEventElapsedTime(&ms, r.a, r.b) != hipSuccess) continue;
    acc[r.tag].launches += 1; acc[r.tag].ms += ms; acc[r.tag].flops += r.flops; acc[r.tag].bytes += r.bytes;
  }
  int n = 0;
  for (int i = 0; i < T_COUNT && n < cap; ++i)
    if (acc[i].launches) out[n++] = acc[i];
  *n_out = n;
  return 0;
}

static int gemm_f32_entry(int device, const float* A, const float* B, float* C, int64_t M, int64_t N, int64_t K,
                          int a_kmajor, int b_kmajor, int tile, int nsplit, int iters, float* ms,
                          const int32_t* a_gather, int64_t a_rows, int bk, float* adam_m) {
  if (!A || !B || !C || M < 1 || N < 1 || K < 1) return fail(-1, "ganmf_gemm_f32: bad argument");
  if (a_gather && (a_kmajor || a_rows < 1)) return fail(-1, "ganmf_gemm_f32_ex: a row list needs a K-contiguous A with a_rows >= 1 rows");
  if (bk != 0 && bk != 32) return fail(-1, "ganmf_gemm_f32_ex: bk must be 0 or 32");
  if (adam_m && (iters > 1 || ms)) return fail(-1, "ganmf_gemm_f32_ex: the Adam epilogue updates its state: one launch, no timing (iters = 1, ms = NULL)");
  if (a_gather)
    for (int64_t r = 0; r < M; ++r)
      if (a_gather[r] < 0 || a_gather[r] >= a_rows) return fail(-1, "ganmf_gemm_f32_ex: row id out of range");
  if (a_kmajor && !b_kmajor) return fail(-1, "ganmf_gemm_f32: the TT layout is not part of the GANMF path");
  if (tile != 0 && tile != 64 && tile != 128) return fail(-1, "ganmf_gemm_f32: tile must be 0, 64 or 128");
  HIP_TRY(hipSetDevice(device));
  const int ar = a_kmajor ? K : (a_gather ? (int)a_rows : M), ac = a_kmajor ? M : K;
  const int br = b_kmajor ? K : N, bc = b_kmajor ? N : K;
  const int lda = round_up(ac, LD_ALIGN), ldb = round_up(bc, LD_ALIGN), ldc = round_up((int)N, LD_ALIGN);
  float *dA = nullptr, *dB = nullptr, *dC = nullptr, *slab = nullptr, *zp = nullptr, *dIds = nullptr, *dMom = nullptr, *dAlpha = nullptr;
  TRY(dalloc(&zp, 2048 + 64));
  TRY(dalloc(&dA, (size_t)ar * lda)); TRY(dalloc(&dB, (size_t)br * ldb)); TRY(dalloc(&dC, (size_t)M * ldc));
  HIP_TRY(hipMemcpy2D(dA, (size_t)lda * 4, A, (size_t)ac * 4, (size_t)ac * 4, ar, hipMemcpyHostToDevice));
  HIP_TRY(hipMemcpy2D(dB, (size_t)ldb * 4, B, (size_t)bc * 4, (size_t)bc * 4, br, hipMemcpyHostToDevice));
  GemmP g{};
  g.A = dA; g.lda = lda; g.B = dB; g.ldb = ldb; g.C = dC; g.ldc = ldc;
  g.M = (int)M; g.N = (int)N; g.K = (int)K; g.nbatch = 1; g.epi.kind = EPI_STORE; g.zero_page = zp; g.c_pad_writable = 1;
  if (a_gather) {
    TRY(dalloc(&dIds, (size_t)M));
    HIP_TRY(hipMemcpy(dIds, a_gather, (size_t)M * 4, hipMemcpyHostToDevice));
    g.a_gather = reinterpret_cast<const int*>(dIds);
  }
  if (adam_m) {
    const float alpha = 1e-3f;
    TRY(dalloc(&dMom, 2 * (size_t)M * ldc)); TRY(dalloc(&dAlpha, 64));
    HIP_TRY(hipMemcpy(dAlpha, &alpha, 4, hipMemcpyHostToDevice));
    g.epi.kind = EPI_ADAM; g.epi.adam_theta = dC; g.epi.adam_m = dMom; g.epi.adam_v = dMom + (size_t)M * ldc;
    g.epi.adam_alpha = dAlpha; g.epi.adam_reg = 0.f;
  }
  GemmTune tune;
  tune.tile = tile; tune.nsplit = adam_m ? 1 : nsplit; tune.bk = bk;
  tune.mode = env_mfma_mode(MFMA_DEFAULT);
  tune.ring = tune_env_int("ring", 0);
  if (tune.ring != 0 && tune.ring != 2 && tune.ring != 3 && tune.ring != 4) tune.ring = 0;
  tune.persist = tune_env_int("persist", -1);
  if (tune.persist > 1) tune.persist = experiment_int("GANMF_PERSIST_WAVES", 1);
  tune.kg = tune_env_int("kg", 0);
  tune.tile_order = tune_env_int("tile_order", 0);
  if (tune.kg != 0 && tune.kg != 1 && tune.kg != 2 && tune.kg != 4) tune.kg = 0;
  GemmPlan pl = gemm_plan(g.M, g.N, g.K, 1, false, tune, adam_m != nullptr);
  pl.persist = gemm_persist_eligible(g, a_kmajor, b_kmajor, pl, tune.persist) ? (tune.persist >= 2 ? tune.persist : 1) : 0;
  if (tune_env_int("skinny", 1) && tile == 0 && nsplit == 0) { if (!plan_skinny(pl, g, a_kmajor != 0) && tune_env_int("skinny_n", 1)) plan_skinny_n(pl, g, a_kmajor != 0); }
  if (env_int("GANMF_X3KG", 0) && pl.mode == MFMA_F32 && pl.tile == 64 && pl.kg == 4 && pl.ring == 3 && !pl.persist) pl.mode = MFMA_BF16X3;
  if (tune_env_int("bf16w", 0) && tile == 0 && nsplit == 0) plan_bf16w(pl, g, a_kmajor != 0, b_kmajor != 0, tune_env_int("bf16w", 0) >= 2);
  if (env_int("GANMF_DEBUG_PLAN", 0))
    fprintf(stderr, "[ganmf plan] %-28s M=%d N=%d K=%d batch=1 -> tile %d ring %d kg %d nsplit %d (kps %d) mfma %s wgs %d est %.1f us%s\n", "ganmf_gemm_f32",
            g.M, g.N, g.K, pl.tile, pl.ring, pl.kg, pl.nsplit, pl.kps,
            pl.mode == MFMA_BF16X3 ? "bf16x3" : pl.mode == MFMA_BF16 ? "bf16" : pl.mode == MFMA_F16 ? "f16" : "f32", pl.tiles_m * pl.tiles_n * pl.nsplit, pl.est_us,
            pl.skinny ? " (skinny-K stream)" : pl.skinny_n ? " (skinny-N stream)" : pl.wide32 ? " (64 x 32 tiles, 128-deep K-tiles)" : pl.persist ? " (persistent tile walk)" : "");
  if (a_gather && !(pl.tile == 64 && pl.kg == 4 && !pl.persist && !pl.skinny && !pl.skinny_n && !pl.wide32))
    return fail(-1, "ganmf_gemm_f32_ex: a row list needs a 16-wave 64 x 64 plan (tile = 64, GANMF_TUNE kg=4,ring=3)");
  bf16raw *plA = nullptr, *plB = nullptr;
#ifdef GANMF_PERSIST_DIAG_BUILD
  if (tune_env_int("planes", 0) && !a_kmajor) {
    const size_t ea = (size_t)ar * lda, eb = (size_t)br * ldb;
    TRY(dalloc((float**)&plA, (3 * ea + 1) / 2 + 64));
    TRY(dalloc((float**)&plB, (3 * eb + 1) / 2 + 64));
    GANMF_LAUNCH(planes_of_kernel, dim3(512), dim3(256), 0, (hipStream_t) nullptr, (const float*)dA, plA, (long long)ea, (long long)(ea / 4));
    GANMF_LAUNCH(planes_of_kernel, dim3(512), dim3(256), 0, (hipStream_t) nullptr, (const float*)dB, plB, (long long)eb, (long long)(eb / 4));
    HIP_TRY(hipDeviceSynchronize());
    g.a_planes = plA; g.a_pstride = (long long)ea; g.b_planes = plB; g.b_pstride = (long long)eb;
  }
#endif
  const size_t slab_elems = gemm_slab_elems(pl, g.M, ldc, 1);
  if (slab_elems) TRY(dalloc(&slab, slab_elems));
  unsigned* counters = nullptr;
  const bool inl = experiment_int("GANMF_INKERNEL_REDUCE", 0) != 0;
  if (inl) TRY(dalloc((float**)&counters, COUNTER_CAP));
  hipStream_t st = nullptr;
  HIP_TRY(gemm_run(st, g, a_kmajor, b_kmajor, pl, slab, slab_elems, counters, COUNTER_CAP));
  HIP_TRY(hipDeviceSynchronize());
  if (iters > 1 || ms) {
    hipEvent_t a, b;
    hipEventCreate(&a); hipEventCreate(&b);
    hipEventRecord(a, st);
    for (int i = 0; i < std::max(iters, 1); ++i) gemm_run(st, g, a_kmajor, b_kmajor, pl, slab, slab_elems, counters, COUNTER_CAP);
    hipEventRecord(b, st);
    hipEventSynchronize(b);
    float t = 0.f;
    hipEventElapsedTime(&t, a, b);
    if (ms) *ms = t / std::max(iters, 1);
    hipEventDestroy(a); hipEventDestroy(b);
  }
  HIP_TRY(hipMemcpy2D(C, (size_t)N * 4, dC, (size_t)ldc * 4, (size_t)N * 4, M, hipMemcpyDeviceToHost));
  if (adam_m) HIP_TRY(hipMemcpy2D(adam_m, (size_t)N * 4, dMom, (size_t)ldc * 4, (size_t)N * 4, M, hipMemcpyDeviceToHost));
  hipFree(dA); hipFree(dB); hipFree(dC); hipFree(zp); hipFree(plA); hipFree(plB); hipFree(dIds); hipFree(dMom); hipFree(dAlpha);
  if (slab) hipFree(slab);
  if (counters) hipFree(counters);
  return 0;
}

int ganmf_gemm_f32(int device, const float* A, const float* B, float* C, int64_t M, int64_t N, int64_t K,
                   int a_kmajor, int b_kmajor, int tile, int nsplit, int iters, float* ms) {
  return gemm_f32_entry(device, A, B, C, M, N, K, a_kmajor, b_kmajor, tile, nsplit, iters, ms, nullptr, 0, 0, nullptr);
}

int ganmf_gemm_f32_ex(int device, const float* A, const float* B, float* C, int64_t M, int64_t N, int64_t K,
                      int a_kmajor, int b_kmajor, int tile, int nsplit, int iters, float* ms,
                      const int32_t* a_gather, int64_t a_rows, int bk, float* adam_m) {
  return gemm_f32_entry(device, A, B, C, M, N, K, a_kmajor, b_kmajor, tile, nsplit, iters, ms, a_gather, a_rows, bk, adam_m);
}
```

ganmf_amd/csrc/lib/abi_train.inc:

```
int ganmf_train_epoch(ganmf_handle* h, const int32_t* perm, int64_t n, int32_t d_steps, int32_t g_steps,
                      int64_t n_steps_per_pass, const int32_t* global_batch_rows, float* d_losses,
                      float* g_losses) {
  return ganmf_train_epoch_ragged(h, perm, n, d_steps, g_steps, n_steps_per_pass, global_batch_rows, nullptr, d_losses, g_losses);
}

int ganmf_train_epoch_ragged(ganmf_handle* h, const int32_t* perm, int64_t n, int32_t d_steps, int32_t g_steps,
                             int64_t n_steps_per_pass, const int32_t* global_batch_rows,
                             const int32_t* local_batch_rows, float* d_losses, float* g_losses) {
  if (!h || (!perm && n > 0)) return fail(-1, "ganmf_train_epoch: null argument");
  TRY(needs_tensors(h, "ganmf_train_epoch"));
  TRY(not_cfgan(h, "ganmf_train_epoch"));
  if (h->cfg.model == GANMF_MODEL_MF) return fail(-1, "ganmf_train_epoch: a GANMF_MODEL_MF handle holds factors only and has no adversarial training; its factors come from ganmf_als_half_sweep or ganmf_set_tensor");
  if (!h->has_urm) return fail(-1, "ganmf_train_epoch: ganmf_set_urm_csr has not been called");
  if (n < 0 || n > h->U) return fail(-1, "ganmf_train_epoch: n=%lld out of range", (long long)n);
  if (d_steps < 0 || g_steps < 0) return fail(-1, "ganmf_train_epoch: negative step count");
  const bool dist = h->has_comm && h->cfg.world_size > 1;
  if (dist && !global_batch_rows) return fail(-1, "ganmf_train_epoch: global_batch_rows required when world_size > 1");
  HIP_TRY(hipSetDevice(h->dev));
  ++h->param_version;
  prealloc_pass_buffers(h, local_batch_rows != nullptr);
  static const bool time_it = experiment_int("GANMF_TIME_EPOCH", 0) != 0;
  const auto tp0 = std::chrono::steady_clock::now();
  auto since = [&]() { return std::chrono::duration<double, std::micro>(std::chrono::steady_clock::now() - tp0).count(); };
  double t_prep = 0, t_first = 0, t_enq = 0, t_sync = 0;
  const int B = h->B;
  const int64_t local_steps = local_batch_rows ? n_steps_per_pass : (n + B - 1) / B;
  const int64_t per_pass = std::max(local_steps, n_steps_per_pass);
  if (per_pass == 0) return 0;
  std::vector<int64_t> slice_at(per_pass);
  std::vector<int> slice_nb(per_pass);
  {
    int64_t at = 0;
    for (int64_t i = 0; i < per_pass; ++i) {
      int nb;
      if (local_batch_rows) {
        nb = local_batch_rows[i];
        if (nb < 0 || nb > B || at + nb > n) return fail(-1, "ganmf_train_epoch_ragged: local_batch_rows[%lld]=%d (batch_size %d, %lld of %lld rows used)", (long long)i, nb, B, (long long)at, (long long)n);
      } else {
        nb = (int)std::max<int64_t>(0, std::min<int64_t>(B, n - i * B));
        at = std::min<int64_t>(i * B, n);
      }
      slice_at[i] = at; slice_nb[i] = nb;
      at += nb;
    }
    if (local_batch_rows && at != n) return fail(-1, "ganmf_train_epoch_ragged: local_batch_rows sum to %lld, n = %lld", (long long)at, (long long)n);
  }
  TRY(ensure_stage(h, (size_t)3 * h->U, 0));
  int* const stage_perm = h->stage_i;
  int* const pos = h->stage_i + h->U;
  int* const pos_step = h->stage_i + 2 * (size_t)h->U;
  std::fill(pos, pos + h->U, -1);
  for (int64_t i = 0; i < per_pass; ++i) std::fill(pos_step + slice_at[i], pos_step + slice_at[i] + slice_nb[i], (int)i);
  for (int64_t i = 0; i < n; ++i) {
    const int r = perm[i];
    if (r < 0 || r >= h->U) return fail(-1, "ganmf_train_epoch: row id %d out of range at %lld", r, (long long)i);
    if (pos[r] != -1) return fail(-1, "ganmf_train_epoch: row id %d appears twice in the permutation", r);
    pos[r] = (int)i;
    stage_perm[i] = r;
  }
  std::vector<int> bglob(per_pass);
  for (int64_t i = 0; i < per_pass; ++i) {
    const int nb = slice_nb[i];
    bglob[i] = global_batch_rows ? global_batch_rows[i] : nb;
    if (bglob[i] < nb || bglob[i] < 1) return fail(-1, "ganmf_train_epoch: global_batch_rows[%lld]=%d < local %d", (long long)i, bglob[i], nb);
  }
  t_prep = since();
  HIP_TRY(hipMemcpyAsync(h->perm, stage_perm, (size_t)3 * h->U * sizeof(int), hipMemcpyHostToDevice, h->st));
  const int64_t nd = (int64_t)d_steps * per_pass, ng = (int64_t)g_steps * per_pass;
  TRY(parts_begin(h, nd, ng));
  t_first = since();
  const int64_t nfull = (local_batch_rows || d_steps == 0) ? 0 : n / B;
  GemmPlan stage_pl{};
  bool stage_front = false;
  const bool staged = nfull > 0 && stage_pass_plan(h, nfull, &stage_pl, &stage_front);
  const bool lazy = g_steps > 0 && lazy_pass_ok(h, per_pass, n);
  bool gen_front = false;
  if (g_steps > 0 && h->g_rows_staged == 1) (void)generator_plan(h, B, &gen_front);
  const int64_t nfull_g = (local_batch_rows || g_steps == 0 || !lazy || h->sparse_g || !h->g_rows_staged || gen_front) ? 0 : n / B;
  GemmPlan gonly_pl{};
  bool gonly_front = false;
  const bool rows_only = !staged && d_steps == 0 && nfull_g > 0 && !h->sparse_d && stage_pass_plan(h, nfull_g, &gonly_pl, &gonly_front);
  const bool gx = nfull_g > 0 && (staged || rows_only);
  struct PassGuard {
    ganmf_handle* h;
    bool g_opened_early = false;
    ~PassGuard() {
      h->front_staged = false; h->x_staged = false; h->XF = h->XF_own; h->d_alpha = S_ALPHA_D;
      if (h->lazy_pass) lazy_pass_abort(h);
      if (g_opened_early) {
        GANMF_LAUNCH(restore_g_powers_kernel, dim3(1), dim3(64), 0, h->st, h->scal);
        (void)hipGetLastError();
      }
    }
  } guard{h};
  if (staged) {
    const bool dis = h->cfg.model == GANMF_MODEL_DISGANMF;
    TRY(stage_pass(h, h->perm, nfull, stage_pl, stage_front, dis ? h->N + 1 : -1, dis ? (int)h->cfg.row_offset : 0, lazy ? (int)per_pass : 0,
                   &guard.g_opened_early));
  } else if (rows_only) {
    const bool dis = h->cfg.model == GANMF_MODEL_DISGANMF;
    TRY(stage_pass(h, h->perm, nfull_g, gonly_pl, gonly_front, dis ? h->N + 1 : -1, dis ? (int)h->cfg.row_offset : 0, 0, nullptr, false));
  }
  int64_t idx = 0;
  for (int p = 0; p < d_steps; ++p) {
    const int tab = S_TAB + (p & 1) * h->tab_cap;
    if (staged && p > 0) {
      GANMF_LAUNCH(open_steps_kernel, dim3(1), dim3(64), 0, h->st, h->scal, 0, tab, (int)nfull, h->cfg.d_lr);
      HIP_TRY(hipGetLastError());
    }
    for (int64_t i = 0; i < per_pass; ++i, ++idx) {
      const int64_t a = slice_at[i];
      const int nb = slice_nb[i];
      const bool st = staged && i < nfull;
      h->front_staged = st;
      h->XF = st ? h->XF_pass + (size_t)i * 2 * B * h->ldN : h->XF_own;
      if (st) h->d_alpha = tab + (int)i;
      else if (staged) h->d_alpha = S_ALPHA_D;
      TRY(any_d_step(h, h->perm + std::min<int64_t>(a, std::max<int64_t>(n - 1, 0)), nb, bglob[i], idx));
    }
  }
  if (staged) { h->front_staged = false; h->XF = h->XF_own; h->d_alpha = S_ALPHA_D; }
  idx = 0;
  for (int p = 0; p < g_steps; ++p) {
    if (lazy) TRY(lazy_pass_begin(h, p, per_pass, n, staged && p == 0));
    guard.g_opened_early = false;
    for (int64_t i = 0; i < per_pass; ++i, ++idx) {
      const int64_t a = slice_at[i];
      const int nb = slice_nb[i];
      if (lazy) { h->lazy_step = (int)i; h->g_alpha = lazy_tab_slot(h, p) + (int)i; h->Ub = h->Ub_sched + (size_t)std::min<int64_t>(a, std::max<int64_t>(n - 1, 0)) * h->ldk; }
      const bool xst = gx && i < nfull_g;
      h->x_staged = xst;
      h->XF = xst ? h->XF_pass + (size_t)i * 2 * B * h->ldN : h->XF_own;
      TRY(any_g_step(h, h->perm + std::min<int64_t>(a, std::max<int64_t>(n - 1, 0)), nb, (int)a, bglob[i], idx));
    }
    if (lazy) TRY(lazy_pass_end(h, p, per_pass));
  }
  h->x_staged = false; h->XF = h->XF_own;
  TRY(dp_join(h));
  TRY(arenas_finish(h, nd, ng));
  if (dist && nd > 0) {
    if (h->cfg.model == GANMF_MODEL_DISGANMF) TRY(allreduce(h, h->d_parts, (size_t)nd * 4));
    else {
      const int grid = (int)std::min<int64_t>(256, (nd + 255) / 256);
      GANMF_LAUNCH(col_copy_kernel, dim3(grid), dim3(256), 0, h->st, h->d_parts, h->colbuf, (long long)nd, 2, 1);
      HIP_TRY(hipGetLastError());
      TRY(allreduce(h, h->colbuf, (size_t)nd));
      GANMF_LAUNCH(col_copy_kernel, dim3(grid), dim3(256), 0, h->st, h->d_parts, h->colbuf, (long long)nd, 2, 0);
      HIP_TRY(hipGetLastError());
    }
  }
  if (dist && ng > 0) TRY(allreduce(h, h->g_parts, (size_t)ng * 4));
  const size_t ndp = (size_t)std::max<int64_t>(nd, 1) * 4, ngp = (size_t)std::max<int64_t>(ng, 1) * 4;
  TRY(ensure_stage(h, 0, ndp + ngp + 4));
  HIP_TRY(hipMemcpyAsync(h->stage_f, h->d_parts, (ndp + ngp) * sizeof(float), hipMemcpyDeviceToHost, h->st));
  const size_t seam_at = (ndp + ngp + 1) & ~(size_t)1;
  if (h->wgrad_seam) HIP_TRY(hipMemcpyAsync(h->stage_f + seam_at, h->seam_cnt + 1, sizeof(unsigned long long), hipMemcpyDeviceToHost, h->st));
  t_enq = since();
  HIP_TRY(hipStreamSynchronize(h->st));
  t_sync = since();
  if (h->wgrad_seam) {
    unsigned long long gave_up = 0;
    memcpy(&gave_up, h->stage_f + seam_at, sizeof gave_up);
    if (gave_up) return fail(-2, "wgrad_seam_kernel: a weight-gradient block gave up waiting for the slab sum of dE (results of this call are invalid)");
  }
  const std::vector<float> dp(h->stage_f, h->stage_f + ndp), gp(h->stage_f + ndp, h->stage_f + ndp + ngp);
  finish_losses(h, dp, gp, bglob, nd, ng, per_pass, d_losses, g_losses);
  if (time_it)
    fprintf(stderr, "[ganmf epoch] %lld D + %lld G steps: host prep %.0f us, first step enqueued at %.0f, all enqueued at %.0f, synced at %.0f, done at %.0f us\n",
            (long long)nd, (long long)ng, t_prep, t_first, t_enq, t_sync, since());
  return 0;
}

int ganmf_train_step(ganmf_handle* h, int kind, const int32_t* uids, int32_t n, float* loss) {
  if (!h || !uids) return fail(-1, "ganmf_train_step: null argument");
  TRY(needs_tensors(h, "ganmf_train_step"));
  TRY(not_cfgan(h, "ganmf_train_step"));
  if (h->cfg.model == GANMF_MODEL_MF) return fail(-1, "ganmf_train_step: a GANMF_MODEL_MF handle holds factors only and has no adversarial training; its factors come from ganmf_als_half_sweep or ganmf_set_tensor");
  if (!h->has_urm) return fail(-1, "ganmf_train_step: ganmf_set_urm_csr has not been called");
  if (n < 1 || n > h->B) return fail(-1, "ganmf_train_step: batch of %d rows (handle batch_size %d)", n, h->B);
  if (kind != 0 && kind != 1) return fail(-1, "ganmf_train_step: kind must be 0 (D) or 1 (G)");
  if (h->has_comm && h->cfg.world_size > 1) return fail(-1, "ganmf_train_step: single-GPU entry; use ganmf_train_epoch");
  HIP_TRY(hipSetDevice(h->dev));
  ++h->param_version;
  std::vector<int> pos(h->U, -1);
  for (int i = 0; i < n; ++i) {
    if (uids[i] < 0 || uids[i] >= h->U) return fail(-1, "ganmf_train_step: row id %d out of range", uids[i]);
    if (pos[uids[i]] != -1) return fail(-1, "ganmf_train_step: duplicate row id %d", uids[i]);
    pos[uids[i]] = i;
  }
  HIP_TRY(hipMemcpyAsync(h->perm, uids, n * sizeof(int), hipMemcpyHostToDevice, h->st));
  HIP_TRY(hipMemcpyAsync(h->pos, pos.data(), (size_t)h->U * sizeof(int), hipMemcpyHostToDevice, h->st));
  TRY(parts_begin(h, kind == 0, kind == 1));
  if (kind == 0) TRY(any_d_step(h, h->perm, n, n, 0));
  else TRY(any_g_step(h, h->perm, n, 0, n, 0));
  TRY(dp_join(h));
  TRY(arenas_finish(h, kind == 0, kind == 1));
  std::vector<float> dp(4), gp(4);
  HIP_TRY(hipMemcpyAsync(dp.data(), h->d_parts, 4 * sizeof(float), hipMemcpyDeviceToHost, h->st));
  HIP_TRY(hipMemcpyAsync(gp.data(), h->g_parts, 4 * sizeof(float), hipMemcpyDeviceToHost, h->st));
  HIP_TRY(hipStreamSynchronize(h->st));
  std::vector<int> bglob(1, n);
  float dl = 0.f, gl = 0.f;
  finish_losses(h, dp, gp, bglob, kind == 0 ? 1 : 0, kind == 1 ? 1 : 0, 1, &dl, &gl);
  if (loss) *loss = kind == 0 ? dl : gl;
  return 0;
}
```

ganmf_amd/csrc/lib/handle.inc:

```

constexpr int LOCAL_MAX_WORLD = 8;
struct LocalPtrs { float* p[LOCAL_MAX_WORLD]; };
enum LocalOp : int { LOCAL_ALLREDUCE = 0, LOCAL_REDUCE_SCATTER = 1, LOCAL_ALLGATHER = 2 };
__global__ void local_collective_kernel(LocalPtrs b, int world, size_t count, int op) {
  const size_t slice = count / (size_t)world;
  for (size_t i = (size_t)blockIdx.x * blockDim.x + threadIdx.x; i < count; i += (size_t)gridDim.x * blockDim.x) {
    if (op == LOCAL_ALLGATHER) {
      const float v = b.p[i / slice][i];
      for (int r = 0; r < world; ++r) b.p[r][i] = v;
      continue;
    }
    float s = b.p[0][i];
    for (int r = 1; r < world; ++r) s += b.p[r][i];
    if (op == LOCAL_ALLREDUCE) { for (int r = 0; r < world; ++r) b.p[r][i] = s; }
    else b.p[i / slice][i] = s;
  }
}
struct LocalGroup {
  std::mutex mu;
  std::condition_variable cv;
  int world = 0, dev = -1, arrived = 0, joined = 0;
  long long generation = 0;
  size_t count = 0;
  int op = 0;
  bool failed = false;
  LocalPtrs bufs{};
};

struct AlsSide {
  long long* indptr = nullptr;
  int* indices = nullptr;
  float* conf = nullptr;
  int64_t rows = 0, nnz = 0;
  bool canonical = false;
};

struct SlimState {
  bool ready = false;
  int symmetric = 0, sgd = 0;
  double lr = 0, li = 0, lj = 0, gamma = 0, b1 = 0, b2 = 0, b1_pow = 0, b2_pow = 0;
  uint64_t seed = 0;
  int64_t epoch = 0;
  size_t cells = 0;
  double *S = nullptr, *st0 = nullptr, *st1 = nullptr;
  long long* indptr = nullptr;
  int* items = nullptr;
  int* eligible = nullptr;
  int n_eligible = 0;
};

struct ProfileMlp {
  int g = 0, Lg = 0, act = 0, ldg = 0;
  int out_act = -1;
  std::vector<Tensor> Gl;
  Tensor Go;
  std::vector<float*> Hl;
  float *sc_C = nullptr, *sc_H0 = nullptr, *sc_H1 = nullptr, *sc_F = nullptr;
  size_t sc_rows = 0;
  std::vector<Tensor*> tensors() {
    std::vector<Tensor*> v;
    for (auto& t : Gl) v.push_back(&t);
    v.push_back(&Go);
    return v;
  }
};

struct CfganState {
  bool ready = false;
  int d_batch = 0, g_batch = 0, scheme = 0, Bm = 0, ldx = 0, words = 0;
  float zr_coef = 0.f;
  uint64_t seed = 0;
  ProfileMlp gen;
  float *C = nullptr, *fake = nullptr, *dfake = nullptr, *DX = nullptr, *dh0 = nullptr, *dh1 = nullptr;
  float *zr_part = nullptr, *loss_rows = nullptr, *sq = nullptr, *loss_dev = nullptr;
  size_t loss_cap = 0;
  unsigned* planes = nullptr;
  int* k_rows = nullptr;
  float* cache = nullptr;
  long long cache_version = -1;
};

struct CaaeState {
  bool ready = false;
  int Bm = 0, n_s = 0, words = 0, d_bsize = 0;
  float lmbda = 0.f, beta = 0.f, lr = 0.f;
  uint64_t seed = 0;
  ProfileMlp gen[2];
  Tensor bias;
  int* k_rows = nullptr;
  float* cdf[2] = {nullptr, nullptr};
  int* iu = nullptr;
  const void* iu_src = nullptr;
  int *perm = nullptr, *tu = nullptr, *ti = nullptr;
  long long order_cap = 0;
  int* neg = nullptr;
  size_t neg_cap = 0;
  int* users = nullptr;
  unsigned* nu = nullptr;
  int* items = nullptr;
  int step_slots = 0, rec_passes = 0, rec_steps[2] = {0, 0};
  long long rec_nnz = 0;
  int* xt = nullptr;
  int* first = nullptr;
  int *xu = nullptr, *xi = nullptr;
  unsigned* xn = nullptr;
  float *Pg = nullptr, *Qi = nullptr, *Qj = nullptr, *coef = nullptr, *lt = nullptr, *rt = nullptr;
  float *C = nullptr, *R = nullptr, *Rp = nullptr, *cdfb = nullptr, *dz = nullptr, *dh0 = nullptr, *dh1 = nullptr;
  float *lse = nullptr, *reward = nullptr, *la = nullptr, *ae = nullptr, *sq = nullptr, *loss_dev = nullptr;
  size_t loss_cap = 0;
  float* lse_all = nullptr;
};

struct ganmf_handle {
  ganmf_cfg cfg;
  int dev = 0;
  hipStream_t st = nullptr;
  hipStream_t st2 = nullptr;
  hipEvent_t ev_fork = nullptr, ev_join = nullptr, ev_mid = nullptr;
  hipEvent_t ev_t0 = nullptr, ev_t1 = nullptr;
  hipEvent_t ev_we = nullptr, ev_wd = nullptr;
  int U = 0, N = 0, k = 0, e = 0, B = 0;
  int ldN = 0, ldk = 0, lde = 0;
  int L = 0, act = 0;
  std::vector<Tensor> Wl;
  Tensor Wo;
  std::vector<float*> Al;
  float *dz0 = nullptr, *dz1 = nullptr, *dlogit = nullptr;
  Tensor We, Wd, Ue, V;
  float* gD = nullptr;
  size_t gD_elems = 0;
  long long* indptr = nullptr;
  int* indices = nullptr;
  float* data = nullptr;
  long long nnz = 0;
  bool has_urm = false;
  bool sparse_g = false;
  bool sparse_d = false;
  long long* csc_colptr = nullptr;
  int* csc_rowidx = nullptr;
  float* csc_val = nullptr;
  float* sp_rows = nullptr;
  int* perm = nullptr;
  int* pos = nullptr;
  int* stage_i = nullptr;
  float* stage_f = nullptr;
  size_t stage_i_cap = 0, stage_f_cap = 0;
  float *XF = nullptr, *Ub = nullptr, *E = nullptr, *Es = nullptr, *Dl = nullptr, *dE = nullptr, *dF = nullptr, *gUb = nullptr;
  float* XF_own = nullptr;
  float* XF_pass = nullptr;
  size_t XF_pass_elems = 0;
  float* Ub_pass = nullptr;
  size_t Ub_pass_elems = 0;
  bool skinny = true;
  int bf16w = 1;
  bool skinny_n = true;
  bool pass_stage = true;
  bool pass_buffers_tried = false;
  bool x_staged = false;
  bool front_staged = false;
  int tab_cap = 0;
  bool lazy_rows = true;
  bool lazy_pass = false;
  int g_alpha = S_ALPHA_G;
  float* Ub_own = nullptr;
  float* gUb_own = nullptr;
  float* Ub_sched = nullptr;
  size_t Ub_sched_elems = 0;
  int* pos_step = nullptr;
  std::vector<std::pair<float*, size_t>> lazy_chunks;
  size_t lazy_chunk = 0, lazy_used = 0;
  std::vector<LazyStep> lazy_steps;
  int lazy_step = 0;
  LazyStep* lazy_stage = nullptr;
  size_t lazy_stage_cap = 0;
  LazyStep* lazy_tab = nullptr;
  size_t lazy_tab_cap = 0;
  float* zero_page = nullptr;
  float* slab = nullptr;
  size_t slab_elems = 0;
  float* slab2 = nullptr;
  size_t slab2_elems = 0;
  unsigned *counters = nullptr, *counters2 = nullptr;
  int x3kg = 7;
  bool inkernel_reduce = true;
  int inlaunch_tags = 0;
  int inlaunch_max = 4;
  float* rs = nullptr;
  float* scal = nullptr;
  float *sqp = nullptr;
  int sqp_stride = 0;
  int reg_cap = 0;
  int pair_ring = 2;
  bool dis_colsum_pending = false;
  ColSumP dis_colsum{};
  bool dis_uid_done = false;
  int dis_cap = 0;
  float* dis_slot = nullptr;
  std::vector<char> dis_fused;
  std::vector<int> dis_regn;
  bool defer_gub = true;
  int multi = 31;
  float* V_alt = nullptr;
  bool fuse_adam = true;
  bool dis_fuse_hidden = true;
  bool dcoef_spread = true;
  float* parts_all = nullptr;
  float *d_parts = nullptr, *g_parts = nullptr;
  float* colbuf = nullptr;
  float *d_arena = nullptr, *g_arena = nullptr;
  int64_t parts_cap = 0;
  long long* seen_indptr = nullptr;
  int* seen_indices = nullptr;
  int64_t seen_rows = 0, seen_cols = 0;
  unsigned char* item_mask = nullptr;
  size_t item_mask_cap = 0;
  int64_t item_mask_w = 0;
  bool mask_cold = false;
  std::vector<unsigned char> filter_host, ignore_host;
  int64_t ignore_w = 0;
  unsigned char* rank_mask = nullptr;
  size_t rank_mask_cap = 0;
  int* topk_items = nullptr;
  float* topk_vals = nullptr;
  size_t topk_cap = 0;
  float* div_mat = nullptr;
  int64_t div_w = 0;
  long long* test_indptr = nullptr;
  int* test_indices = nullptr;
  double* test_gain = nullptr;
  int64_t test_rows = 0, test_cols = 0;
  double* eval_buf = nullptr;
  size_t eval_cap = 0;
  int64_t test_nnz = 0;
  float* test_rating = nullptr;
  bool test_rating_ok = false;
  double* eval_w = nullptr;
  int64_t eval_w_width = 0;
  float* eval_rmse = nullptr;
  size_t eval_rmse_cap = 0;
  unsigned* eval_counts = nullptr;
  size_t eval_counts_cap = 0;
  int* eval_grp = nullptr;
  size_t eval_grp_cap = 0;
  long long* cand_indptr = nullptr;
  int* cand_indices = nullptr;
  std::vector<long long> cand_indptr_host;
  int64_t cand_rows = 0, cand_cols = 0;
  int* sc_ids = nullptr;
  size_t sc_ids_cap = 0;
  float *sc_rows = nullptr, *sc_out = nullptr;
  size_t sc_rows_cap = 0, sc_out_cap = 0;
  unsigned *sc_pa = nullptr, *sc_pb = nullptr;
  size_t sc_pa_cap = 0, sc_pb_cap = 0;
  const float* sc_pb_src = nullptr;
  long long sc_pb_version = -1, param_version = 0;
  int sc_pb_rows = 0;
  float *sim_mat = nullptr, *sim_pool = nullptr;
  double* sim_part = nullptr;
  int* sim_zero = nullptr;
  size_t sim_mat_cap = 0, sim_pool_cap = 0, sim_part_cap = 0, sim_zero_cap = 0;
  int* dr_ids = nullptr;
  float *dr_X = nullptr, *dr_Ub = nullptr, *dr_E = nullptr, *dr_A = nullptr;
  double *dr_part = nullptr, *dr_val = nullptr;
  size_t dr_ids_cap = 0, dr_X_cap = 0, dr_Ub_cap = 0, dr_E_cap = 0, dr_A_cap = 0, dr_part_cap = 0, dr_val_cap = 0;
  int64_t disc_block = 0;
  AlsSide als[2];
  float* als_G = nullptr;
  int* als_bad = nullptr;
  long long* knn_indptr = nullptr;
  int* knn_nbr = nullptr;
  float* knn_val = nullptr;
  int64_t knn_nnz = -1;
  float* knn_dense = nullptr;
  size_t knn_dense_cap = 0;
  SlimState slim;
  CfganState cf;
  CaaeState ca;
  float* svd_P[2] = {nullptr, nullptr};
  float *svd_G = nullptr, *svd_X = nullptr, *svd_Wl = nullptr, *svd_lam = nullptr;
  int* svd_flag = nullptr;
  int svd_ldl = 0;
  int gram_arith = 1;
  bool score_presplit = true;
  ncclComm_t comm = nullptr;
  bool has_comm = false;
  std::atomic<bool> comm_aborted{false};
  std::mutex comm_mu;
  std::shared_ptr<LocalGroup> local;
  int d_alpha = S_ALPHA_D;
  int side_pending = 0;
  bool merge_decode = true;
  int red_elems = 0;
  bf16raw *pl_XF = nullptr, *pl_Dl = nullptr, *pl_Es = nullptr, *pl_dE = nullptr;
  long long ps_N = 0, ps_e = 0;
  float* wgs_dump = nullptr;
  int* wgs_table = nullptr;
  int wgs_key[5] = {0, 0, 0, 0, 0}, wgs_rounds = 0;
  size_t wgs_table_cap = 0;
  bool wgrad_stream = false;
  int adam_nfast = 3;
  int wgrad_xb = 16;
  int wgrad_seam = 0;
  int adam_touch = 1;
  unsigned long long* seam_cnt = nullptr;
  unsigned long long seam_target = 0;
  int pair_kg = 4;
  bool gub_x3 = false;
  int g_rows_staged = 1;
  int wd_lane = 0;
  long long fork_armed_at = 0;
  bool fork_attach = true;
  bool force_coll = false;
  GemmTune tune;
  bool debug_plan = false;
  int fused_bk = 0;
  int fused_tile = 64;
  int fused_mode = MFMA_BF16X3;
  std::vector<long long> seen_plans;
  bool prof = false;
  std::vector<ProfRec> recs;
};
```

ganmf_amd/csrc/lib/step_ganmf.inc:

```
GemmPlan generator_plan(ganmf_handle* h, int nb, bool* front) {
  const int N = h->N, k = h->k;
  GemmP g{};
  g.A = h->Ub; g.lda = h->ldk; g.B = h->V.p; g.ldb = h->ldk;
  g.C = h->XF + (size_t)nb * h->ldN; g.ldc = h->ldN;
  g.M = nb; g.N = N; g.K = k; g.epi.kind = EPI_STORE; g.nbatch = 1;
  g.zero_page = h->zero_page;
  GemmPlan pl = gemm_plan(g.M, g.N, g.K, 1, false, h->tune, (h->multi & 1) != 0 && k <= 256);
  pl.persist = gemm_persist_eligible(g, false, false, pl, h->tune.persist) ? 1 : 0;
  *front = (h->multi & 1) && plan_is_f32_64_kg(pl, 4) && pl.nsplit == 1;
  if (!*front && (h->multi & 1) && (h->x3kg & 4) && low_precision(h) && plan_is_lp_64(pl) && pl.nsplit == 1) { pl.kg = 4; *front = true; }
  if (*front) return pl;
  return plan_gemm(h, T_GEMM_GEN, g, false, false, nullptr);
}

inline int lazy_tab_slot(const ganmf_handle* h, int p);
bool stage_pass_plan(ganmf_handle* h, int64_t nfull, GemmPlan* pl, bool* front) {
  if (!h->pass_stage || nfull < 4 || h->sparse_d || nfull > h->tab_cap) return false;
  *pl = generator_plan(h, h->B, front);
  if (!*front && (pl->persist || pl->nsplit != 1)) return false;
  const size_t need = (size_t)nfull * 2 * h->B * h->ldN;
  if (need > h->XF_pass_elems) {
    size_t free_b = 0, total_b = 0;
    if (hipMemGetInfo(&free_b, &total_b) != hipSuccess) return false;
    if ((need - h->XF_pass_elems) * sizeof(float) > free_b / 4) return false;
  }
  return true;
}

static bool lazy_chunk_alloc(ganmf_handle* h, size_t elems) {
  float* p = nullptr;
  if (hipMalloc((void**)&p, elems * sizeof(float)) != hipSuccess) return false;
  if (hipMemsetAsync(p, 0, elems * sizeof(float), h->st) != hipSuccess) { hipFree(p); return false; }
  h->lazy_chunks.emplace_back(p, elems);
  return true;
}
struct BestEffort {
  std::string saved;
  BestEffort() : saved(g_err) {}
  ~BestEffort() { (void)hipGetLastError(); g_err = saved; }
};
static bool fits_quarter_of_free(size_t bytes) {
  size_t free_b = 0, total_b = 0;
  return hipMemGetInfo(&free_b, &total_b) == hipSuccess && bytes <= free_b / 4;
}
void prealloc_pass_buffers(ganmf_handle* h, bool ragged) {
  if (h->pass_buffers_tried) return;
  h->pass_buffers_tried = true;
  const int64_t nfull = h->U / std::max(h->B, 1);
  if (nfull < 4) return;
  BestEffort guard;
  GemmPlan pl{};
  bool front = false;
  if (!ragged && stage_pass_plan(h, nfull, &pl, &front)) {
    const size_t need = (size_t)nfull * 2 * h->B * h->ldN;
    if (need > h->XF_pass_elems) {
      hipFree(h->XF_pass); h->XF_pass = nullptr; h->XF_pass_elems = 0;
      if (dalloc(&h->XF_pass, need) == 0) h->XF_pass_elems = need;
      else h->XF_pass = nullptr;
    }
    const size_t need_u = front ? 0 : (size_t)nfull * h->B * h->ldk;
    if (need_u > h->Ub_pass_elems && fits_quarter_of_free((need_u - h->Ub_pass_elems) * sizeof(float))) {
      hipFree(h->Ub_pass); h->Ub_pass = nullptr; h->Ub_pass_elems = 0;
      if (dalloc(&h->Ub_pass, need_u) == 0) h->Ub_pass_elems = need_u;
      else h->Ub_pass = nullptr;
    }
  }
  if (h->lazy_rows && h->cfg.g_reg == 0.f) {
    const size_t need = (size_t)h->U * h->ldk;
    if (need > h->Ub_sched_elems && fits_quarter_of_free((need - h->Ub_sched_elems) * sizeof(float))) {
      hipFree(h->Ub_sched); h->Ub_sched = nullptr; h->Ub_sched_elems = 0;
      if (dalloc(&h->Ub_sched, need) == 0) h->Ub_sched_elems = need;
      else h->Ub_sched = nullptr;
    }
    if (h->lazy_chunks.empty()) {
      const size_t want = std::min<size_t>((size_t)128 << 20, std::max<size_t>((size_t)16 << 20, (size_t)(nfull + 1) * 16 * h->B * h->ldk));
      if (fits_quarter_of_free(want * sizeof(float))) lazy_chunk_alloc(h, want);
    }
    const size_t T = (size_t)nfull + 2;
    if (2 * T > h->lazy_stage_cap && hipHostMalloc((void**)&h->lazy_stage, 2 * (T + 16) * sizeof(LazyStep), hipHostMallocDefault) == hipSuccess)
      h->lazy_stage_cap = 2 * (T + 16);
    if (2 * T > h->lazy_tab_cap && hipMalloc((void**)&h->lazy_tab, 2 * (T + 16) * sizeof(LazyStep)) == hipSuccess) h->lazy_tab_cap = 2 * (T + 16);
  }
}

int stage_pass(ganmf_handle* h, const int* rows_dev, int64_t nfull, const GemmPlan& pl0, bool front, int uid_col, int row_offset, int open_g,
               bool* g_opened, bool gen = true) {
  const int N = h->N, k = h->k, B = h->B;
  const size_t need = (size_t)nfull * 2 * B * h->ldN;
  if (need > h->XF_pass_elems) {
    HIP_TRY(hipStreamSynchronize(h->st));
    HIP_TRY(hipStreamSynchronize(h->st2));
    hipFree(h->XF_pass); h->XF_pass = nullptr; h->XF_pass_elems = 0;
    TRY(dalloc(&h->XF_pass, need));
    h->XF_pass_elems = need;
  }
  const size_t need_u = (front || !gen) ? 0 : (size_t)nfull * B * h->ldk;
  if (need_u > h->Ub_pass_elems) {
    HIP_TRY(hipStreamSynchronize(h->st));
    hipFree(h->Ub_pass); h->Ub_pass = nullptr; h->Ub_pass_elems = 0;
    TRY(dalloc(&h->Ub_pass, need_u));
    h->Ub_pass_elems = need_u;
  }
  const int rows = (int)(nfull * B);
  {
    DensP d{h->indptr, h->indices, h->data, rows_dev, rows, N, h->XF_pass, h->ldN, h->Ue.p, h->ldk, (front || !gen) ? nullptr : h->Ub_pass,
            h->scal, 0, 0, 0.f, uid_col, row_offset};
    d.stage_b = B;
    d.open_d_slot = S_TAB; d.open_d_count = gen ? (int)nfull : 0; d.lr_d = h->cfg.d_lr;
    d.open_g_slot = lazy_tab_slot(h, 0); d.open_g_count = open_g; d.lr_g = h->cfg.g_lr;
    d.nseg = std::max(1, std::min(16, (h->ldN + 8191) / 8192));
    Scope s(h, T_DENSIFY, 0, 4.0 * rows * (N + 2 * k));
    GANMF_LAUNCH(densify_rows_kernel, dim3(rows * d.nseg), dim3(256), 0, h->st, d);
    HIP_TRY(hipGetLastError());
    if (open_g > 0 && g_opened) *g_opened = true;
  }
  if (!gen) return 0;
  GemmP g{};
  g.B = h->V.p; g.ldb = h->ldk; g.lda = h->ldk;
  g.C = h->XF_pass + (size_t)B * h->ldN; g.ldc = h->ldN; g.c_batch_stride = (long long)2 * B * h->ldN;
  g.M = B; g.N = N; g.K = k; g.epi.kind = EPI_STORE; g.nbatch = (int)nfull;
  g.zero_page = h->zero_page;
  if (front) {
    g.A = h->Ue.p; g.a_gather = rows_dev; g.a_gather_batch = B;
    GemmPlan pl = pl0;
    if (combined_x3(h)) pl.mode = MFMA_BF16X3;
    fill_plan(g, pl);
    Scope s(h, T_GEMM_GEN, nfull * gemm_flops(g.M, g.N, g.K), gemm_bytes((double)nfull * g.M, g.N, g.K));
    HIP_TRY(gemm_dispatch(h->st, g, false, false, pl));
    return 0;
  }
  g.A = h->Ub_pass; g.a_batch_stride = (long long)B * h->ldk;
  return run_gemm(h, T_GEMM_GEN, T_RED_GEN, g, false, false, nullptr, 0, 0, nullptr, nullptr, nullptr, nullptr, &pl0);
}

int rows_and_generator(ganmf_handle* h, const int* rows_dev, int nb, int which, int aslot, int uid_col, int row_offset) {
  if (which == 0 && h->front_staged) return 0;
  const bool xs = which == 1 && h->x_staged && h->lazy_pass;
  const int N = h->N, k = h->k;
  const bool lazy = which == 1 && h->lazy_pass;
  DensP d{h->indptr, h->indices, h->data, rows_dev, nb, N, h->XF, h->ldN, h->Ue.p, h->ldk, lazy ? nullptr : h->Ub, h->scal, which,
          lazy ? -1 : aslot, which ? h->cfg.g_lr : h->cfg.d_lr, uid_col, row_offset};
  GemmP g{};
  g.A = h->Ub; g.lda = h->ldk; g.B = h->V.p; g.ldb = h->ldk;
  g.C = h->XF + (size_t)nb * h->ldN; g.ldc = h->ldN;
  g.M = nb; g.N = N; g.K = k; g.epi.kind = EPI_STORE; g.nbatch = 1;
  g.zero_page = h->zero_page;
  bool is_front = false;
  GemmPlan pl = generator_plan(h, nb, &is_front);
  if (is_front) {
    if (h->debug_plan) {
      const long long key = ((long long)T_GEMM_GEN << 48) ^ ((long long)g.M << 32) ^ ((long long)g.N << 16) ^ g.K;
      if (std::find(h->seen_plans.begin(), h->seen_plans.end(), key) == h->seen_plans.end()) {
        h->seen_plans.push_back(key);
        fprintf(stderr, "[ganmf plan] %-28s M=%d N=%d K=%d batch=1 -> tile 64 ring 3 kg 4 nsplit 1 (kps %d) mfma %s wgs %d est %.1f us (one launch with the %d CSR rows)\n",
                kTagName[T_GEMM_GEN], g.M, g.N, g.K, pl.kps, pl.mode == MFMA_F16 ? "f16" : pl.mode == MFMA_BF16 ? "bf16" : combined_x3(h) ? "bf16x3" : "f32",
                pl.tiles_m * pl.tiles_n, pl.est_us, nb);
      }
    }
    Scope s(h, T_FRONT, gemm_flops(g.M, g.N, g.K), gemm_bytes(g.M, g.N, g.K) + 4.0 * nb * (N + 2 * k));
    if (!lazy) { g.A = h->Ue.p; g.a_gather = rows_dev; }
    fill_plan(g, pl);
    const int nrow_blocks = xs ? 0 : nb;
    if (pl.mode == MFMA_F16) GANMF_LAUNCH(front_lp_kernel<true>, dim3(pl.tiles_m * pl.tiles_n + nrow_blocks), dim3(1024), 0, h->st, g, d);
    else if (pl.mode == MFMA_BF16) GANMF_LAUNCH(front_lp_kernel<false>, dim3(pl.tiles_m * pl.tiles_n + nrow_blocks), dim3(1024), 0, h->st, g, d);
    else if (combined_x3(h)) GANMF_LAUNCH((front_kernel<4, true>), dim3(pl.tiles_m * pl.tiles_n + nrow_blocks), dim3(1024), 0, h->st, g, d);
    else GANMF_LAUNCH(front_kernel<4>, dim3(pl.tiles_m * pl.tiles_n + nrow_blocks), dim3(1024), 0, h->st, g, d);
    HIP_TRY(hipGetLastError());
    return 0;
  }
  if (!xs) {
    Scope s(h, T_DENSIFY, 0, 4.0 * nb * (N + 2 * k));
    d.nseg = std::max(1, std::min(16, (h->ldN + 8191) / 8192));
    GANMF_LAUNCH(densify_rows_kernel, dim3(nb * d.nseg), dim3(256), 0, h->st, d);
    HIP_TRY(hipGetLastError());
  }
  return run_gemm(h, T_GEMM_GEN, T_RED_GEN, g, false, false);
}

int step_front(ganmf_handle* h, const int* rows_dev, int nb, int which) {
  const int N = h->N, k = h->k, e = h->e;
  const int aslot = which ? h->g_alpha : h->d_alpha;
  const bool lazy = which == 1 && h->lazy_pass;
  if ((which == 1 && h->sparse_g) || (which == 0 && h->sparse_d)) {
    TRY(dp_join(h, PEND_WE));
    {
      Scope s(h, T_DENSIFY, 0, 4.0 * nb * (2 * k + e) + 4.0 * (double)h->nnz / std::max(h->U, 1) * nb * e);
      GANMF_LAUNCH(sparse_front_kernel, dim3(nb), dim3(256), 0, h->st, h->indptr, h->indices, h->data, rows_dev, nb, N,
                         h->XF, h->ldN, h->Ue.p, h->ldk, lazy ? nullptr : h->Ub, h->scal, which, lazy ? -1 : aslot, which ? h->cfg.g_lr : h->cfg.d_lr, h->We.p, h->lde, e, h->E);
      HIP_TRY(hipGetLastError());
    }
    {
      GemmP g{};
      g.A = h->Ub; g.lda = h->ldk; g.B = h->V.p; g.ldb = h->ldk;
      g.C = h->XF + (size_t)nb * h->ldN; g.ldc = h->ldN;
      g.M = nb; g.N = N; g.K = k; g.epi.kind = EPI_STORE;
      TRY(run_gemm(h, T_GEMM_GEN, T_RED_GEN, g, false, false));
    }
    {
      TRY(dp_join(h, PEND_WE));
      GemmP g{};
      g.A = h->XF + (size_t)nb * h->ldN; g.lda = h->ldN; g.B = h->We.p; g.ldb = h->lde;
      g.C = h->E + (size_t)nb * h->lde; g.ldc = h->lde; g.M = nb; g.N = e; g.K = N + 1; g.epi.kind = EPI_STORE;
      TRY(run_gemm(h, T_GEMM_ENC, T_RED_ENC, g, false, true));
    }
    return 0;
  }
  TRY(rows_and_generator(h, rows_dev, nb, which, aslot, -1, 0));
  {
    TRY(dp_join(h, PEND_WE));
    GemmP g{};
    g.A = h->XF; g.lda = h->ldN; g.B = h->We.p; g.ldb = h->lde;
    g.C = h->E; g.ldc = h->lde; g.M = 2 * nb; g.N = e; g.K = N + 1; g.epi.kind = EPI_STORE;
    TRY(run_gemm(h, T_GEMM_ENC, T_RED_ENC, g, false, true));
  }
  return 0;
}

int d_step(ganmf_handle* h, const int* rows_dev, int nb, int b_global, float* parts, float* arena) {
  float* regWe = arena + 2 * (size_t)h->reg_cap;
  float* regWd = arena + 3 * (size_t)h->reg_cap;
  const int N = h->N, e = h->e;
  const bool dist = h->has_comm;
  if ((dist || h->wd_lane) && !h->front_staged) h->d_alpha = h->d_alpha == S_ALPHA_D ? S_ALPHA_D_ALT : S_ALPHA_D;
  const int aslot = h->d_alpha;
  const float inv_bn = 1.0f / ((float)b_global * (float)N);
  int sqn = 0;
  bool fused = false;
  int regn[2] = {ADAM_GRID, ADAM_GRID};
  if (nb > 0) {
    TRY(step_front(h, rows_dev, nb, 0));
    TRY(dp_join(h, PEND_WD));
    {
      GemmP g{};
      g.A = h->E; g.lda = h->lde; g.B = h->Wd.p; g.ldb = h->ldN;
      g.C = h->Dl; g.ldc = h->ldN; g.M = nb; g.N = N; g.K = e + 1;
      g.nbatch = 2; g.a_batch_stride = (long long)nb * h->lde; g.c_batch_stride = (long long)nb * h->ldN;
      g.epi.kind = EPI_SUB_AUX_SQ; g.epi.aux = h->XF; g.epi.ldaux = h->ldN;
      g.epi.aux_batch_stride = (long long)nb * h->ldN; g.epi.sq_partials = h->sqp;
      if (h->sparse_d) {
        g.epi.csr_indptr = h->indptr; g.epi.csr_indices = h->indices; g.epi.csr_data = h->data; g.epi.csr_rows = rows_dev;
      }
      bool merged = false;
      if (!h->sparse_d && nb % 64 == 0 && h->merge_decode) {
        const GemmPlan p1 = gemm_plan(2 * nb, g.N, g.K, 1, true, h->tune), p2 = gemm_plan(g.M, g.N, g.K, 2, true, h->tune);
        if (p1.tile == 64 && p2.tile == 64 && p1.nsplit == 1 && p2.nsplit == 1 && p1.mode == p2.mode && p1.kg == p2.kg && p1.ring == p2.ring) {
          GemmP q = g;
          q.M = 2 * nb; q.nbatch = 1; q.a_batch_stride = 0; q.c_batch_stride = 0; q.epi.aux_batch_stride = 0;
          q.epi.sq_m_half = nb / 64;
          int cnt = 0;
          TRY(run_gemm(h, T_GEMM_DEC, T_RED_DEC, q, false, true, &cnt, 4.0 * 2 * nb * N));
          sqn = p2.sq_count;
          merged = true;
        }
      }
      if (!merged)
      TRY(run_gemm(h, T_GEMM_DEC, T_RED_DEC, g, false, true, &sqn, 4.0 * 2 * nb * N));
    }
  } else {
    GANMF_LAUNCH(open_step_kernel, dim3(1), dim3(64), 0, h->st, h->scal, 0, aslot, h->cfg.d_lr);
    HIP_TRY(hipGetLastError());
  }
  if (dist) {
    MultiRed mr{};
    mr.count = 2; mr.out = h->scal;
    mr.e[0] = {h->sqp, sqn, S_SUM_REAL, 0};
    mr.e[1] = {h->sqp + sqn, sqn, S_SUM_FAKE, 0};
    {
      Scope s(h, T_MULTIRED, 0, 0);
      GANMF_LAUNCH(multi_reduce_kernel, dim3(S_SUM_FAKE + 1), dim3(256), 0, h->st, mr);
      HIP_TRY(hipGetLastError());
    }
    TRY(allreduce(h, h->scal + S_SUM_REAL, 2));
  }
  const DCoefP dc{h->scal, h->sqp, sqn, sqn, dist ? 1 : 0, h->cfg.m, nb, inv_bn, h->E, h->Es, h->lde, h->rs, parts};
  const long long dc_total = (long long)2 * nb * (h->lde / 4);
  bool dcoef_done = false;
  GemmP gde{};
  GemmPlan pde;
  if (nb > 0 && (h->multi & 4) && (h->multi & 8)) {
    gde.A = h->Dl; gde.lda = h->ldN; gde.B = h->Wd.p; gde.ldb = h->ldN;
    gde.C = h->dE; gde.ldc = h->lde; gde.M = 2 * nb; gde.N = e; gde.K = N; gde.nbatch = 1;
    gde.epi.kind = EPI_ROWSCALE; gde.epi.rowscale = h->rs; gde.zero_page = h->zero_page;
    pde = gemm_plan(gde.M, gde.N, gde.K, 1, false, h->tune);
    pde.persist = 0;
    GemmPlan pskn = pde;
    const bool de_stream = h->skinny_n && plan_skinny_n(pskn, gde, false);
    if (!de_stream && plan_is_f32_64_kg(pde, 4) && pde.nsplit > 1 && !(h->inkernel_reduce && pde.nsplit <= h->inlaunch_max)) {
      TRY(ensure_slab(h, gemm_slab_elems(pde, gde.M, gde.ldc, 1), 0));
      Scope s(h, T_DE_DCOEF, gemm_flops(gde.M, gde.N, gde.K), gemm_bytes(gde.M, gde.N, gde.K) + 8.0 * 2 * nb * e);
      GemmP q = gde;
      fill_plan(q, pde);
      q.C = h->slab; q.c_split_stride = (long long)gde.M * gde.ldc; q.c_batch_stride = (long long)gde.M * gde.ldc;
      const int ng = pde.tiles_m * pde.tiles_n * pde.nsplit;
      const int nd = h->dcoef_spread ? 0 : (int)std::max<long long>(1, std::min<long long>(32, (dc_total + 4095) / 4096));
      if (combined_x3(h)) GANMF_LAUNCH((de_dcoef_kernel<4, true>), dim3(ng + nd), dim3(1024), 0, h->st, q, dc, nd);
      else GANMF_LAUNCH(de_dcoef_kernel<4>, dim3(ng + nd), dim3(1024), 0, h->st, q, dc, nd);
      HIP_TRY(hipGetLastError());
      dcoef_done = true;
    }
  }
  if (!dcoef_done) {
    Scope s(h, T_DCOEF, 0, 8.0 * 2 * nb * e);
    const int grid = (int)std::max<long long>(1, std::min<long long>(128, (dc_total + 1023) / 1024));
    GANMF_LAUNCH(d_coef_kernel, dim3(grid), dim3(256), 0, h->st, dc);
    HIP_TRY(hipGetLastError());
  }
  if (nb > 0) {
    const bool regD = h->cfg.d_reg != 0.f;
    fused = h->fuse_adam && !dist;
    GemmTune ft;
    ft.tile = h->fused_tile; ft.ring = 2; ft.nsplit = 1;
    ft.mode = h->tune.mode != MFMA_AUTO ? h->tune.mode : h->fused_mode;
    ft.bk = h->fused_bk;
    const GemmTune* wg_tune = &ft;
    const int start = (int)(rows_dev - h->perm);
    auto sparse_gWe = [&](GemmP& g) {
      if (!h->sparse_d) return;
      g.A = h->XF + (size_t)nb * h->ldN; g.B = h->dE + (size_t)nb * h->lde; g.K = nb;
      g.epi.sp_rows = h->sp_rows; g.epi.sp_ld = h->lde; g.epi.sp_bias_row = N; g.epi.sp_bias_parts = CSC_BIAS_PARTS;
    };
    auto sparse_rows = [&]() -> int {
      if (!h->sparse_d) return 0;
      Scope s(h, T_DENSIFY, 0, 4.0 * ((double)h->nnz / std::max(h->U, 1) * nb * e + 2.0 * (N + CSC_BIAS_PARTS) * e));
      GANMF_LAUNCH(csc_rows_kernel, dim3(N + CSC_BIAS_PARTS), dim3(256), 0, h->st, h->csc_colptr, h->csc_rowidx, h->csc_val,
                   h->pos, start, nb, N, h->dE, h->lde, e, h->sp_rows);
      HIP_TRY(hipGetLastError());
      return 0;
    };
    RedP dE_red{};
    auto gemm_gWd = [&]() -> int {
      GemmP g{};
      g.A = h->Es; g.lda = h->lde; g.B = h->Dl; g.ldb = h->ldN;
      g.C = h->Wd.g; g.ldc = h->ldN; g.M = e + 1; g.N = N; g.K = 2 * nb; g.epi.kind = EPI_STORE;
      g.a_scale = grad_scale(h, b_global);
      if (fused) {
        g.epi.kind = EPI_ADAM; g.epi.adam_theta = h->Wd.p; g.epi.adam_m = h->Wd.m; g.epi.adam_v = h->Wd.v;
        g.epi.adam_alpha = h->scal + aslot; g.epi.adam_reg = h->cfg.d_reg;
        g.epi.sq_partials = regD ? regWd : nullptr;
      }
      return run_gemm(h, T_GEMM_GWD, T_RED_GWD, g, true, true, &regn[1], fused ? 24.0 * h->Wd.count() : 0, 0, wg_tune, nullptr,
                      nullptr, dE_red.part ? &dE_red : nullptr);
    };
    if (dcoef_done) {
      dE_red = RedP{};
      dE_red.part = h->slab; dE_red.nsplit = pde.nsplit; dE_red.out = gde.C; dE_red.ld = gde.ldc; dE_red.M = gde.M; dE_red.N = gde.N;
      dE_red.batch_stride = 0; dE_red.epi = gde.epi; dE_red.epi.sq_stride = GEMM_RED_GRID;
      dE_red.split_stride = (long long)gde.M * gde.ldc;
    } else {
      GemmP g{};
      g.A = h->Dl; g.lda = h->ldN; g.B = h->Wd.p; g.ldb = h->ldN;
// ... 243 lines not shown
    }
    if (dist) {
      TRY(dp_update(h, T_ADAM_D, h->We, aslot, h->cfg.d_reg, regD ? regWe : nullptr, 1));
      TRY(dp_mark(h, PEND_WE));
      const bool armed = fork_arm(h);
      TRY(gemm_gWd());
      TRY(fork_wait(h, armed));
      TRY(dp_update(h, T_ADAM_D, h->Wd, aslot, h->cfg.d_reg, regD ? regWd : nullptr, 1));
      TRY(dp_mark(h, PEND_WD));
      (void)regn; (void)parts;
      return 0;
    }
  } else {
    TRY(dp_join(h));
    HIP_TRY(hipMemsetAsync(h->gD, 0, h->gD_elems * sizeof(float), h->st));
    if (dist) {
      const bool regD = h->cfg.d_reg != 0.f;
      TRY(lane_fork(h));
      TRY(dp_update(h, T_ADAM_D, h->We, aslot, h->cfg.d_reg, regD ? regWe : nullptr, 1));
      TRY(dp_mark(h, PEND_WE));
      TRY(dp_update(h, T_ADAM_D, h->Wd, aslot, h->cfg.d_reg, regD ? regWd : nullptr, 1));
      TRY(dp_mark(h, PEND_WD));
    }
  }
  const bool reg = h->cfg.d_reg != 0.f;
  if (!dist && !fused) {
    TRY(adam_dense(h, T_ADAM_D, h->We, h->We.g, aslot, h->cfg.d_reg, reg ? regWe : nullptr));
    TRY(adam_dense(h, T_ADAM_D, h->Wd, h->Wd.g, aslot, h->cfg.d_reg, reg ? regWd : nullptr));
  }
  (void)regn; (void)parts;
  return 0;
}

inline int lazy_tab_slot(const ganmf_handle* h, int p) { return S_TAB + (2 + (p & 1)) * h->tab_cap; }
bool lazy_pass_ok(const ganmf_handle* h, int64_t per_pass, int64_t n) {
  if (!(h->lazy_rows && h->cfg.g_reg == 0.f && per_pass >= 4 && per_pass <= h->tab_cap && n > 0)) return false;
  const GemmPlan pl = gemm_plan(h->B, h->k, h->N, 1, false, h->tune);
  const size_t per_step = (size_t)(std::max(pl.nsplit, 1) + 1) * h->B * h->ldk + 128;
  size_t have = 0;
  for (const auto& ch : h->lazy_chunks) have += ch.second;
  const size_t need = (size_t)per_pass * per_step;
  if (need <= have) return true;
  size_t free_b = 0, total_b = 0;
  if (hipMemGetInfo(&free_b, &total_b) != hipSuccess) return false;
  return (need - have) * sizeof(float) <= free_b / 4;
}
int lazy_block(ganmf_handle* h, size_t elems, float** out) {
  elems = (elems + 63) / 64 * 64;
  while (h->lazy_chunk < h->lazy_chunks.size() && h->lazy_used + elems > h->lazy_chunks[h->lazy_chunk].second) { ++h->lazy_chunk; h->lazy_used = 0; }
  if (h->lazy_chunk == h->lazy_chunks.size()) {
    const size_t want = std::max<size_t>(elems, (size_t)16 << 20);
    if (!lazy_chunk_alloc(h, want)) HIP_TRY(hipErrorOutOfMemory);
    h->lazy_used = 0;
  }
  *out = h->lazy_chunks[h->lazy_chunk].first + h->lazy_used;
  h->lazy_used += elems;
  return 0;
}
void lazy_pass_abort(ganmf_handle* h) {
  h->lazy_pass = false; h->Ub = h->Ub_own; h->gUb = h->gUb_own; h->g_alpha = S_ALPHA_G;
}
int lazy_pass_begin(ganmf_handle* h, int p, int64_t per_pass, int64_t n, bool opened) {
  const size_t need = (size_t)n * h->ldk;
  if (need > h->Ub_sched_elems) {
    HIP_TRY(hipStreamSynchronize(h->st));
    HIP_TRY(hipStreamSynchronize(h->st2));
    hipFree(h->Ub_sched); h->Ub_sched = nullptr; h->Ub_sched_elems = 0;
    TRY(dalloc(&h->Ub_sched, need));
    h->Ub_sched_elems = need;
  }
  const int tab = lazy_tab_slot(h, p);
  if (!opened) {
    GANMF_LAUNCH(open_steps_kernel, dim3(1), dim3(64), 0, h->st, h->scal, 1, tab, (int)per_pass, h->cfg.g_lr);
    HIP_TRY(hipGetLastError());
  }
  {
    Scope s(h, T_ADAM_U, 0, 16.0 * n * h->ldk);
    const long long total = (long long)n * (h->ldk / 4);
    const int grid = (int)std::max<long long>(1, std::min<long long>(8192, (total + 255) / 256));
    GANMF_LAUNCH(adam_rows_advance_kernel, dim3(grid), dim3(256), 0, h->st, h->Ue.p, h->Ue.m, h->Ue.v, h->perm, h->pos_step, (int)n,
                 h->ldk, h->scal, tab, h->cfg.g_reg, h->Ub_sched);
    HIP_TRY(hipGetLastError());
  }
  h->lazy_steps.assign((size_t)per_pass, LazyStep{nullptr, 0, 1, 0, 0});
  h->lazy_chunk = 0; h->lazy_used = 0;
  h->lazy_pass = true;
  return 0;
}
int lazy_pass_end(ganmf_handle* h, int p, int64_t per_pass) {
  const size_t T = (size_t)per_pass;
  if (2 * T > h->lazy_stage_cap) {
    HIP_TRY(hipStreamSynchronize(h->st));
    if (h->lazy_stage) hipHostFree(h->lazy_stage);
    h->lazy_stage = nullptr; h->lazy_stage_cap = 0;
    HIP_TRY(hipHostMalloc((void**)&h->lazy_stage, 2 * (T + 16) * sizeof(LazyStep), hipHostMallocDefault));
    h->lazy_stage_cap = 2 * (T + 16);
  }
  if (2 * T > h->lazy_tab_cap) {
    HIP_TRY(hipStreamSynchronize(h->st));
    hipFree(h->lazy_tab); h->lazy_tab = nullptr; h->lazy_tab_cap = 0;
    HIP_TRY(hipMalloc((void**)&h->lazy_tab, 2 * (T + 16) * sizeof(LazyStep)));
    h->lazy_tab_cap = 2 * (T + 16);
  }
  if (p >= 2) HIP_TRY(hipStreamSynchronize(h->st));
  LazyStep* const host = h->lazy_stage + (size_t)(p & 1) * (h->lazy_stage_cap / 2);
  LazyStep* const dev = h->lazy_tab + (size_t)(p & 1) * (h->lazy_tab_cap / 2);
  std::copy(h->lazy_steps.begin(), h->lazy_steps.end(), host);
  HIP_TRY(hipMemcpyAsync(dev, host, T * sizeof(LazyStep), hipMemcpyHostToDevice, h->st));
  {
    Scope s(h, T_ADAM_U, 0, 24.0 * h->Ue.count());
    const long long total = (long long)h->U * (h->ldk / 4);
    const int grid = (int)std::max<long long>(1, std::min<long long>(8192, (total + 255) / 256));
    GANMF_LAUNCH(adam_rows_flush_kernel, dim3(grid), dim3(256), 0, h->st, h->Ue.p, h->Ue.m, h->Ue.v, h->pos, h->pos_step, dev,
                 (int)per_pass, h->U, h->ldk, h->scal, lazy_tab_slot(h, p), h->cfg.g_reg);
    HIP_TRY(hipGetLastError());
  }
  lazy_pass_abort(h);
  return 0;
}

int gen_update(ganmf_handle* h, int nb, int start, int b_global, int* regn_v, float* reg_u, float* reg_v) {
  const int N = h->N, k = h->k;
  const bool reg = h->cfg.g_reg != 0.f;
  const bool dist = h->has_comm;
  const bool fused = h->fuse_adam && !dist && nb > 0;
  *regn_v = ADAM_GRID;
  const bool lazy = h->lazy_pass;
  h->gub_x3 = (long long)((N + 63) / 64) * ((k + 63) / 64) >= 2 * GEMM_CUS && experiment_int("GANMF_GV_STAGED", 1) != 0;
  SlabRef gub{h->gUb, 1, 0};
  auto gemm_gUb = [&]() -> int {
    GemmP g{};
    g.A = h->dF; g.lda = h->ldN; g.B = h->V.p; g.ldb = h->ldk;
    g.C = h->gUb; g.ldc = h->ldk; g.M = nb; g.N = k; g.K = N; g.epi.kind = EPI_STORE;
    g.a_scale = grad_scale(h, b_global);
    if (!lazy) return run_gemm(h, T_GEMM_GUB, T_RED_GUB, g, false, true, nullptr, 0, 0, nullptr, h->defer_gub ? &gub : nullptr);
    const GemmPlan pl = plan_gemm(h, T_GEMM_GUB, g, false, true, nullptr);
    float* fin = nullptr;
    TRY(lazy_block(h, (size_t)nb * h->ldk, &fin));
    g.C = fin;
    gub = SlabRef{fin, 1, 0};
    float* const slab2 = h->slab2;
    const size_t slab2_elems = h->slab2_elems;
    if (pl.nsplit > 1 && h->defer_gub) {
      const size_t elems = gemm_slab_elems(pl, g.M, g.ldc, 1);
      float* blk = nullptr;
      TRY(lazy_block(h, elems, &blk));
      h->slab2 = blk; h->slab2_elems = elems;
    }
    const int rc = run_gemm(h, T_GEMM_GUB, T_RED_GUB, g, false, true, nullptr, 0, 0, nullptr, h->defer_gub ? &gub : nullptr, nullptr, nullptr, &pl);
    h->slab2 = slab2; h->slab2_elems = slab2_elems;
    return rc;
  };
  auto gemm_gV = [&]() -> int {
    GemmP g{};
    g.A = h->dF; g.lda = h->ldN; g.B = h->Ub; g.ldb = h->ldk;
    g.C = h->V.g; g.ldc = h->ldk; g.M = N; g.N = k; g.K = nb; g.epi.kind = EPI_STORE;
    g.a_scale = grad_scale(h, b_global);
    if (fused) {
      g.epi.kind = EPI_ADAM; g.epi.adam_theta = h->V.p; g.epi.adam_m = h->V.m; g.epi.adam_v = h->V.v;
      g.epi.adam_alpha = h->scal + h->g_alpha; g.epi.adam_reg = h->cfg.g_reg;
      g.epi.sq_partials = reg ? reg_v : nullptr;
      g.adam_touch = adam_touch_for(h, g.M, g.ldc);
    }
    GemmTune ft;
    ft.tile = 64; ft.ring = 2; ft.nsplit = 1;
    ft.mode = h->tune.mode != MFMA_AUTO ? h->tune.mode : h->fused_mode;
    ft.bk = h->fused_bk;
    const long long gv_tiles = (long long)((N + 63) / 64) * ((k + 63) / 64);
    const bool staged_gv = experiment_int("GANMF_GV_STAGED", gv_tiles >= 2 * GEMM_CUS ? 1 : 0) != 0;
    TRY(run_gemm(h, T_GEMM_GV, T_RED_GV, g, true, true, regn_v, fused ? 24.0 * h->V.count() : 0, 0, staged_gv ? &ft : nullptr));
    if (!fused) *regn_v = ADAM_GRID;
    return 0;
  };
  bool paired = false, pair_armed = false;
  const bool v_inline = dist && lazy;
  if (nb > 0 && (fused || dist) && (h->multi & 2) && h->defer_gub && h->V_alt) {
    if (dist) TRY(dp_join(h));
    GemmP g0{}, g1{};
    g0.A = h->dF; g0.lda = h->ldN; g0.B = h->V.p; g0.ldb = h->ldk;
    g0.C = h->gUb; g0.ldc = h->ldk; g0.M = nb; g0.N = k; g0.K = N; g0.epi.kind = EPI_STORE; g0.nbatch = 1;
    g0.zero_page = h->zero_page; g0.a_scale = grad_scale(h, b_global);
    g1.A = h->dF; g1.lda = h->ldN; g1.B = h->Ub; g1.ldb = h->ldk;
    g1.C = h->V.g; g1.ldc = h->ldk; g1.M = N; g1.N = k; g1.K = nb; g1.nbatch = 1;
    g1.zero_page = h->zero_page; g1.a_scale = grad_scale(h, b_global);
    g1.epi.kind = EPI_STORE;
    if (fused) {
      g1.epi.kind = EPI_ADAM; g1.epi.adam_theta = h->V.p; g1.epi.adam_theta_out = h->V_alt; g1.epi.adam_m = h->V.m; g1.epi.adam_v = h->V.v;
      g1.epi.adam_alpha = h->scal + h->g_alpha; g1.epi.adam_reg = h->cfg.g_reg;
      g1.epi.sq_partials = reg ? reg_v : nullptr;
    }
    GemmPlan p0 = gemm_plan(g0.M, g0.N, g0.K, 1, false, h->tune);
    GemmPlan p1 = gemm_plan(g1.M, g1.N, g1.K, 1, g1.epi.sq_partials != nullptr, h->tune, true);
    const bool pair_lp = (h->x3kg & 4) && low_precision(h) && plan_is_lp_64(p0) && plan_is_lp_64(p1) && p0.mode == p1.mode;
    if (((plan_is_f32_64_kg(p0, 4) && plan_is_f32_64_kg(p1, 4)) || pair_lp) && p1.nsplit == 1 &&
        reduce_groups((long long)g0.M * ((g0.N + 3) >> 2), p0.nsplit) == 1) {
      if (p0.nsplit > 1) {
        const size_t elems = gemm_slab_elems(p0, g0.M, g0.ldc, 1);
        float* dst = nullptr;
        if (lazy) TRY(lazy_block(h, elems, &dst));
        else { TRY(ensure_slab(h, elems, 1)); dst = h->slab2; }
        g0.C = dst; g0.c_split_stride = (long long)g0.M * g0.ldc;
        gub = SlabRef{dst, p0.nsplit, (long long)g0.M * g0.ldc};
      } else if (lazy) {
        float* dst = nullptr;
        TRY(lazy_block(h, (size_t)g0.M * g0.ldc, &dst));
        g0.C = dst;
        gub = SlabRef{dst, 1, 0};
      }
      g0.c_batch_stride = (long long)g0.M * g0.ldc;
      fill_plan(g0, p0);
      fill_plan(g1, p1);
      if (fused && (h->adam_nfast & 2)) g1.n_fastest = 1;
      if (fused) g1.adam_touch = adam_touch_for(h, g1.M, g1.ldc);
      if (fused) *regn_v = p1.sq_count;
      const int n0 = p0.tiles_m * p0.tiles_n * p0.nsplit, n1 = p1.tiles_m * p1.tiles_n;
      {
        Scope s(h, T_PAIR, gemm_flops(g0.M, g0.N, g0.K) + gemm_flops(g1.M, g1.N, g1.K),
                gemm_bytes(g0.M, g0.N, g0.K) + gemm_bytes(g1.M, g1.N, g1.K) + (fused ? 24.0 * h->V.count() : 0));
        pair_armed = dist && !v_inline && fork_arm(h);
#ifdef GANMF_PERSIST_DIAG_BUILD
        static unsigned long long* pst = nullptr;
        static int pst_n = 0;
        const bool pstamp = !pair_lp && env_int("GANMF_PAIR_STAMPS", 0) != 0 && pst_n < 30;
        if (pstamp) {
          if (!pst) HIP_TRY(hipMalloc((void**)&pst, (size_t)4096 * 32));
          HIP_TRY(hipMemsetAsync(pst, 0, (size_t)(n0 + n1) * 32, h->st));
          g0.stamps = pst; g1.stamps = pst + (size_t)n0 * 4;
        }
#endif
        if (pair_lp && p0.mode == MFMA_F16) GANMF_LAUNCH(pair_lp_kernel<true>, dim3(n0 + n1), dim3(1024), 0, h->st, g0, g1);
        else if (pair_lp) GANMF_LAUNCH(pair_lp_kernel<false>, dim3(n0 + n1), dim3(1024), 0, h->st, g0, g1);
        else if (h->pair_kg == 1) GANMF_LAUNCH((pair_kernel<1, 2>), dim3(n0 + n1), dim3(256), 0, h->st, g0, g1);
        else if (h->pair_ring == 2) GANMF_LAUNCH((pair_kernel<4, 2>), dim3(n0 + n1), dim3(1024), 0, h->st, g0, g1);
        else GANMF_LAUNCH((pair_kernel<4, 3>), dim3(n0 + n1), dim3(1024), 0, h->st, g0, g1);
        HIP_TRY(hipGetLastError());
#ifdef GANMF_PERSIST_DIAG_BUILD
        if (pstamp && ++pst_n >= 28) {
          HIP_TRY(hipStreamSynchronize(h->st));
          std::vector<unsigned long long> hs((size_t)(n0 + n1) * 4);
          HIP_TRY(hipMemcpy(hs.data(), pst, hs.size() * 8, hipMemcpyDeviceToHost));
          unsigned long long t0 = ~0ull;
          for (int b = 0; b < n0 + n1; ++b) if (hs[(size_t)b * 4]) t0 = std::min(t0, hs[(size_t)b * 4]);
          auto med = [&](int lo, int hi, int i) { std::vector<double> v; for (int b = lo; b < hi; ++b) v.push_back((double)(hs[(size_t)b * 4 + i] - t0) * 0.01); std::sort(v.begin(), v.end()); return std::make_pair(v[v.size() / 2], v.back()); };
          for (int half = 0; half < 2; ++half) {
            const int lo = half ? n0 : 0, hi = half ? n0 + n1 : n0;
            fprintf(stderr, "[pair stamps] %s (%d workgroups): entry median %.2f max %.2f | first K-tile %.2f | K loop done %.2f | exit median %.2f max %.2f us after the launch's first entry\n",
                    half ? "gV + Adam" : "gUb", hi - lo, med(lo, hi, 0).first, med(lo, hi, 0).second, med(lo, hi, 1).first, med(lo, hi, 2).first, med(lo, hi, 3).first, med(lo, hi, 3).second);
          }
        }
#endif
      }
      if (fused) std::swap(h->V.p, h->V_alt);
      paired = true;
    }
  }
  if (dist && paired && v_inline) {
    TRY(dp_update(h, T_ADAM_V, h->V, h->g_alpha, h->cfg.g_reg, reg ? reg_v : nullptr, 0));
  } else if (dist && paired) {
    TRY(fork_wait(h, pair_armed));
    TRY(dp_update(h, T_ADAM_V, h->V, h->g_alpha, h->cfg.g_reg, reg ? reg_v : nullptr, 1));
  } else if (dist) {
    TRY(dp_join(h));
    if (nb > 0) TRY(gemm_gV());
    else HIP_TRY(hipMemsetAsync(h->V.g, 0, h->V.cap * sizeof(float), h->st));
    TRY(lane_fork(h));
    TRY(reduce_scatter(h, h->V.g, h->V.cap, 1, T_COLL_V));
    if (nb > 0) TRY(gemm_gUb());
    TRY(lane_fork(h));
    const size_t slice = h->V.cap / (size_t)h->cfg.world_size, off = (size_t)h->cfg.rank * slice;
    TRY(adam_dense(h, T_ADAM_V, h->V, h->V.g, h->g_alpha, h->cfg.g_reg, reg ? reg_v : nullptr, 1, off, slice));
    TRY(all_gather(h, h->V.p, h->V.cap, 1, T_COLL_V));
  } else if (nb > 0) {
    if (!paired) {
      TRY(gemm_gUb());
      TRY(gemm_gV());
    }
  } else {
    HIP_TRY(hipMemsetAsync(h->V.g, 0, h->V.padded() * sizeof(float), h->st));
  }
  if (lazy) {
    h->lazy_steps[h->lazy_step] = LazyStep{gub.p, gub.split_stride, gub.nsplit, start, nb};
  } else {
    Scope s(h, T_ADAM_U, 0, 24.0 * h->Ue.count());
    GANMF_LAUNCH(adam_rows_kernel, dim3(ADAM_GRID), dim3(256), 0, h->st, h->Ue.p, h->Ue.m, h->Ue.v, gub.p,
                       gub.nsplit, gub.split_stride, h->pos, start, nb, h->U, h->ldk, h->scal, h->g_alpha, h->cfg.g_reg,
                       reg ? reg_u : nullptr);
    HIP_TRY(hipGetLastError());
  }
  if (dist) {
    if (!(paired && v_inline)) { Scope s(h, T_JOIN_V, 0, 0); TRY(lane_join(h)); }
  } else if (!fused) TRY(adam_dense(h, T_ADAM_V, h->V, h->V.g, h->g_alpha, h->cfg.g_reg, reg ? reg_v : nullptr));
  return 0;
}

int g_step(ganmf_handle* h, const int* rows_dev, int nb, int start, int b_global, float* parts, float* arena) {
  const size_t cap = h->reg_cap;
  const int N = h->N, e = h->e;
  const float alpha = h->cfg.recon_coefficient;
  const float inv_bn = 1.0f / ((float)b_global * (float)N);
  int sqn = 0, fmn = 0;
  if (nb > 0) {
    TRY(step_front(h, rows_dev, nb, 1));
    TRY(dp_join(h, PEND_WD));
    {
      GemmP g{};
      g.A = h->E + (size_t)nb * h->lde; g.lda = h->lde; g.B = h->Wd.p; g.ldb = h->ldN;
      g.C = h->Dl; g.ldc = h->ldN; g.M = nb; g.N = N; g.K = e + 1;
      g.epi.kind = EPI_SUB_AUX_SQ; g.epi.aux = h->XF + (size_t)nb * h->ldN; g.epi.ldaux = h->ldN;
      g.epi.sq_partials = arena;
      TRY(run_gemm(h, T_GEMM_DEC, T_RED_DEC, g, false, true, &sqn, 4.0 * nb * N));
    }
    const float rsv = (1.0f - alpha) * (2.0f * inv_bn);
    const float cfm = alpha * 2.0f / ((float)b_global * (float)e);
    {
      GemmP g{};
      g.A = h->Dl; g.lda = h->ldN; g.B = h->Wd.p; g.ldb = h->ldN;
      g.C = h->dE; g.ldc = h->lde; g.M = nb; g.N = e; g.K = N;
      g.epi.kind = EPI_G_DE; g.epi.c = rsv; g.epi.cfm = cfm;
      g.epi.er = h->E; g.epi.ef = h->E + (size_t)nb * h->lde; g.epi.sq_partials = arena + cap;
      TRY(run_gemm(h, T_GEMM_DE, T_RED_DE, g, false, false, &fmn));
    }
    {
      GemmP g{};
      g.A = h->dE; g.lda = h->lde; g.B = h->We.p; g.ldb = h->lde;
      g.C = h->dF; g.ldc = h->ldN; g.M = nb; g.N = N; g.K = e;
      g.epi.kind = EPI_SUB_SCALED_AUX; g.epi.c = rsv; g.epi.aux = h->Dl; g.epi.ldaux = h->ldN;
      g.a_scale = grad_scale(h, b_global);
      TRY(run_gemm(h, T_GEMM_DF, T_RED_DF, g, false, false, nullptr, 4.0 * nb * N));
    }
  } else if (!h->lazy_pass) {
    GANMF_LAUNCH(open_step_kernel, dim3(1), dim3(64), 0, h->st, h->scal, 1, h->g_alpha, h->cfg.g_lr);
    HIP_TRY(hipGetLastError());
  }
  const bool reg = h->cfg.g_reg != 0.f;
  int regn_v = ADAM_GRID;
  TRY(gen_update(h, nb, start, b_global, &regn_v, arena + 2 * cap, arena + 3 * cap));
  (void)parts; (void)reg; (void)sqn; (void)fmn;
  return 0;
}
```

Baseline: 9772.

## Pre-split frozen discriminator weights into bf16x3 pieces once per generator pass

After: 9824 (median of 6 runs). Within noise of the previous version (+0.5%).

```diff
diff --git a/ganmf_amd/csrc/gemm_bf16k.hpp b/ganmf_amd/csrc/gemm_bf16k.hpp
--- a/ganmf_amd/csrc/gemm_bf16k.hpp
+++ b/ganmf_amd/csrc/gemm_bf16k.hpp
@@ -4,6 +4,7 @@
 namespace ganmf {
 
 typedef float f32x4k __attribute__((ext_vector_type(4)));
+typedef float f32x2k __attribute__((ext_vector_type(2)));
 
 struct SplitItemK {
   const float* zp;
diff --git a/ganmf_amd/csrc/gemm_bf16w.hpp b/ganmf_amd/csrc/gemm_bf16w.hpp
--- a/ganmf_amd/csrc/gemm_bf16w.hpp
+++ b/ganmf_amd/csrc/gemm_bf16w.hpp
@@ -18,6 +18,15 @@
 #undef GANMF_BF16W_WAIT
   return tok;
 }
+__device__ __forceinline__ int bf16w_wait_vm4(int n, const f32x4k& v0, const f32x4k& v1, const f32x4k& v2, const f32x2k& v3) {
+  int tok;
+#define GANMF_BF16W_WAIT(N) asm volatile("s_waitcnt vmcnt(" #N ")\n\ts_mov_b32 %0, 0" : "=s"(tok) : "v"(v0), "v"(v1), "v"(v2), "v"(v3))
+  if (n >= 8) GANMF_BF16W_WAIT(8);
+  else if (n >= 4) GANMF_BF16W_WAIT(4);
+  else GANMF_BF16W_WAIT(0);
+#undef GANMF_BF16W_WAIT
+  return tok;
+}
 
 template <int NPIECE> constexpr int bf16w_oper() { return NPIECE * (BF16W_PA + BF16W_PB); }
 template <int NPIECE> constexpr int bf16w_smem_dw() {
@@ -25,10 +34,12 @@
 }
 static_assert(bf16w_oper<3>() == BF16W_OPER && bf16w_smem_dw<3>() == 2 * BF16W_OPER && bf16w_smem_dw<1>() == BF16W_KG * BF16W_BM * BF16W_BN, "plane buffers");
 
-template <bool BKM, int NPIECE = 3, bool F16 = false>
+template <bool BKM, int NPIECE = 3, bool F16 = false, bool BPL = false>
 __device__ __forceinline__ void bf16w_mainloop(const GemmP& p, const int tm, const int tn, const int bz, float* __restrict__ smem, f32x16& acc_out) {
   static_assert(NPIECE == 3 || NPIECE == 1, "pieces per operand");
   static_assert(!F16 || NPIECE == 1, "fp16 pieces only in the single-piece mode");
+  static_assert(!BPL || NPIECE == 3, "B as pieces: the three-piece loop only");
+  constexpr int LPT = BPL ? 4 : 3;
   constexpr int BM = BF16W_BM, BN = BF16W_BN, BK = BF16W_BK, PD = BF16W_PD, PA = BF16W_PA, PB = BF16W_PB, OPER = bf16w_oper<NPIECE>();
   const float sa = (F16 && p.a_scale != 0.f) ? p.a_scale : 1.f, sb = (F16 && p.b_scale != 0.f) ? p.b_scale : 1.f;
   typedef unsigned u32x2 __attribute__((ext_vector_type(2)));
@@ -52,9 +63,11 @@
   const float* s0 = ok0 ? p.A + (size_t)bz * p.a_batch_stride + (size_t)(m0 + arow) * p.lda + 8 * c8 : zp;
   const int kb = tid >> 3, nq = tid & 7;
   const bool okn = n0 + 4 * nq < p.ldb;
-  const float* s2 = !BKM ? (ok2 ? p.B + (size_t)(n0 + row) * p.ldb + 4 * kq : zp) : (okn ? p.B + (size_t)kb * p.ldb + n0 + 4 * nq : zp);
+  const float* const bsrc = BPL ? reinterpret_cast<const float*>(p.b_quads) : p.B;
+  const size_t off2 = !BKM ? (size_t)(n0 + row) * p.ldb + 4 * kq : (size_t)kb * p.ldb + n0 + 4 * nq;
+  const float* s2 = (!BKM ? ok2 : okn) ? bsrc + (BPL ? off2 / 4 * 6 : off2) : zp;
   const int i0 = ok0 ? BK : 0;
-  const long long i2 = !BKM ? (ok2 ? BK : 0) : (okn ? (long long)BK * p.ldb : 0);
+  const long long i2 = (!BKM ? (ok2 ? BK : 0) : (okn ? (long long)BK * p.ldb : 0)) / (BPL ? 4 : 1) * (BPL ? 6 : 1);
   int kleft = p.K;
   const bool in_a = (nt - 1) * BK + 8 * c8 < p.lda, in_b = (nt - 1) * BK + 4 * kq < p.ldb;
   const int dsta = arow * (BK / 2) + ((c8 ^ (arow & 15)) << 2);
@@ -62,8 +75,9 @@
   const int dstb = !BKM ? dst : kb * (BN / 2) + 2 * nq;
 
   f32x4k rg[PD][3];
-#pragma unroll
-  for (int s = 0; s < PD; ++s) { rg[s][0] = f32x4k{0.f, 0.f, 0.f, 0.f}; rg[s][1] = rg[s][0]; rg[s][2] = rg[s][0]; }
+  f32x2k rq[PD];
+#pragma unroll
+  for (int s = 0; s < PD; ++s) { rg[s][0] = f32x4k{0.f, 0.f, 0.f, 0.f}; rg[s][1] = rg[s][0]; rg[s][2] = rg[s][0]; rq[s] = f32x2k{0.f, 0.f}; }
   int tload = 0;
   auto load_tile = [&](auto ss) {
     constexpr int s = decltype(ss)::value;
@@ -85,6 +99,11 @@
     asm volatile("global_load_dwordx4 %0, %1, off offset:16" : "=v"(l1) : "v"(a0) : "memory");
     asm volatile("global_load_dwordx4 %0, %1, off" : "=v"(l2) : "v"(b0) : "memory");
     rg[s][0] = l0; rg[s][1] = l1; rg[s][2] = l2;
+    if constexpr (BPL) {
+      f32x2k l3;
+      asm volatile("global_load_dwordx2 %0, %1, off offset:16" : "=v"(l3) : "v"(b0) : "memory");
+      rq[s] = l3;
+    }
     s0 += i0; s2 += i2;
     ++tload;
   };
@@ -98,9 +117,24 @@
     constexpr int s = decltype(ss)::value;
     constexpr int b = decltype(bb)::value;
     const f32x4k v0 = rg[s][0], v1 = rg[s][1], v2 = rg[s][2];
-    const int tok = bf16w_wait_vm(nwait, v0, v1, v2);
+    int tok;
+    if constexpr (BPL) tok = bf16w_wait_vm4(nwait, v0, v1, v2, rq[s]);
+    else tok = bf16w_wait_vm(nwait, v0, v1, v2);
     const unsigned o = st_a[b], ob = st_b[b];
-    if constexpr (NPIECE == 3) {
+    if constexpr (BPL) {
+      unsigned h0, m0_, l0, h1, m1, l1, h2, m2, l2, h3, m3, l3;
+      split_bf16x3_tok(v0.x, v0.y, h0, m0_, l0, tok); split_bf16x3_tok(v0.z, v0.w, h1, m1, l1, tok);
+      split_bf16x3_tok(v1.x, v1.y, h2, m2, l2, tok); split_bf16x3_tok(v1.z, v1.w, h3, m3, l3, tok);
+      lds_write<u32x4>(o, u32x4{h0, h1, h2, h3});
+      lds_write<u32x4>(o + 4u * PA, u32x4{m0_, m1, m2, m3});
+      lds_write<u32x4>(o + 8u * PA, u32x4{l0, l1, l2, l3});
+      unsigned obt = ob;
+      asm volatile("; B pieces behind wait token %1" : "+v"(obt) : "s"(tok));
+      const f32x2k v3 = rq[s];
+      lds_write<u32x2>(obt, u32x2{__float_as_uint(v2.x), __float_as_uint(v2.y)});
+      lds_write<u32x2>(obt + 4u * PB, u32x2{__float_as_uint(v2.z), __float_as_uint(v2.w)});
+      lds_write<u32x2>(obt + 8u * PB, u32x2{__float_as_uint(v3.x), __float_as_uint(v3.y)});
+    } else if constexpr (NPIECE == 3) {
       unsigned h0, m0_, l0, h1, m1, l1, h2, m2, l2, h3, m3, l3;
       split_bf16x3_tok(v0.x, v0.y, h0, m0_, l0, tok); split_bf16x3_tok(v0.z, v0.w, h1, m1, l1, tok);
       split_bf16x3_tok(v1.x, v1.y, h2, m2, l2, tok); split_bf16x3_tok(v1.z, v1.w, h3, m3, l3, tok);
@@ -123,8 +157,8 @@
     }
   };
   static_for<0, PD>([&](auto ss) { load_tile(ss); });
-  store_tile(std::integral_constant<int, 0>{}, std::integral_constant<int, 0>{}, 3 * (PD - 1));
-  asm volatile("s_waitcnt vmcnt(0)" :: "v"(rg[0][0]), "v"(rg[0][1]), "v"(rg[0][2]), "v"(rg[1][0]), "v"(rg[1][1]), "v"(rg[1][2]));
+  store_tile(std::integral_constant<int, 0>{}, std::integral_constant<int, 0>{}, LPT * (PD - 1));
+  asm volatile("s_waitcnt vmcnt(0)" :: "v"(rg[0][0]), "v"(rg[0][1]), "v"(rg[0][2]), "v"(rg[1][0]), "v"(rg[1][1]), "v"(rg[1][2]), "v"(rq[0]), "v"(rq[1]));
   static_assert(PD == 2, "the wait above names every prefetch register");
   __syncthreads();
 #ifdef GANMF_PERSIST_DIAG_BUILD
@@ -182,7 +216,7 @@
     } else {
       acc = __builtin_amdgcn_mfma_f32_32x32x16_bf16(__builtin_bit_cast(bf16x8, pa[0]), __builtin_bit_cast(bf16x8, pb[0]), acc, 0, 0, 0);
     }
-    if (t + 1 < nt) store_tile(std::integral_constant<int, s1_>{}, std::integral_constant<int, (s1_ & 1)>{}, 3 * (min(t + PD, nt - 1) - (t + 1)));
+    if (t + 1 < nt) store_tile(std::integral_constant<int, s1_>{}, std::integral_constant<int, (s1_ & 1)>{}, LPT * (min(t + PD, nt - 1) - (t + 1)));
     __syncthreads();
   };
   for (int t = 0; t < nt; t += PD)
@@ -195,7 +229,7 @@
   acc_out = acc;
 }
 
-template <bool BKM, int NPIECE = 3, bool F16 = false>
+template <bool BKM, int NPIECE = 3, bool F16 = false, bool BPL = false>
 __device__ __forceinline__ void gemm_bf16w_body(const GemmP& p, const int bid, const int nblk, float* __restrict__ smem) {
   int tm, tn, sp, bz;
   tile_coords(p, bid, nblk, tm, tn, sp, bz);
@@ -203,7 +237,7 @@
 #ifdef GANMF_PERSIST_DIAG_BUILD
   if (p.stamps && threadIdx.x == 0) p.stamps[(size_t)blockIdx.x * 4 + 0] = __builtin_amdgcn_s_memrealtime();
 #endif
-  bf16w_mainloop<BKM, NPIECE, F16>(p, tm, tn, bz, smem, acc[0][0]);
+  bf16w_mainloop<BKM, NPIECE, F16, BPL>(p, tm, tn, bz, smem, acc[0][0]);
 #ifdef GANMF_PERSIST_DIAG_BUILD
   if (p.stamps && threadIdx.x == 0) p.stamps[(size_t)blockIdx.x * 4 + 2] = __builtin_amdgcn_s_memrealtime();
 #endif
@@ -219,10 +253,25 @@
 #endif
 }
 
-template <bool BKM, int NPIECE = 3, bool F16 = false>
+template <bool BKM, int NPIECE = 3, bool F16 = false, bool BPL = false>
 __global__ __launch_bounds__(1024) void gemm_bf16w_mfma(const GemmP p) {
   __shared__ __attribute__((aligned(16))) float smem[bf16w_smem_dw<NPIECE>()];
-  gemm_bf16w_body<BKM, NPIECE, F16>(p, (int)blockIdx.x, (int)gridDim.x, smem);
+  gemm_bf16w_body<BKM, NPIECE, F16, BPL>(p, (int)blockIdx.x, (int)gridDim.x, smem);
+}
+
+struct QuadJob { const float* src; unsigned* dst; long long n4; };
+__global__ __launch_bounds__(256) void weight_quads_kernel(const QuadJob j0, const QuadJob j1, int blocks0) {
+  const bool second = (int)blockIdx.x >= blocks0;
+  const QuadJob& j = second ? j1 : j0;
+  const long long nblk = second ? (long long)gridDim.x - blocks0 : blocks0, blk = second ? (long long)blockIdx.x - blocks0 : blockIdx.x;
+  for (long long i = blk * 256 + threadIdx.x; i < j.n4; i += nblk * 256) {
+    const float4 v = *reinterpret_cast<const float4*>(j.src + 4 * i);
+    unsigned h0, m0, l0, h1, m1, l1;
+    split_bf16x3(v.x, v.y, h0, m0, l0);
+    split_bf16x3(v.z, v.w, h1, m1, l1);
+    uint2* const d = reinterpret_cast<uint2*>(j.dst + 6 * i);
+    d[0] = make_uint2(h0, h1); d[1] = make_uint2(m0, m1); d[2] = make_uint2(l0, l1);
+  }
 }
 
 inline bool gemm_bf16w_eligible(const GemmP& p, bool akm, bool bkm) {
@@ -269,6 +318,9 @@
   } else if (mode == MFMA_BF16) {
     if (bkm) GANMF_LAUNCH((gemm_bf16w_mfma<true, 1, false>), dim3(grid), dim3(1024), 0, st, p);
     else GANMF_LAUNCH((gemm_bf16w_mfma<false, 1, false>), dim3(grid), dim3(1024), 0, st, p);
+  } else if (p.b_quads) {
+    if (bkm) GANMF_LAUNCH((gemm_bf16w_mfma<true, 3, false, true>), dim3(grid), dim3(1024), 0, st, p);
+    else GANMF_LAUNCH((gemm_bf16w_mfma<false, 3, false, true>), dim3(grid), dim3(1024), 0, st, p);
   } else {
     if (bkm) GANMF_LAUNCH(gemm_bf16w_mfma<true>, dim3(grid), dim3(1024), 0, st, p);
     else GANMF_LAUNCH(gemm_bf16w_mfma<false>, dim3(grid), dim3(1024), 0, st, p);
diff --git a/ganmf_amd/csrc/gemm_f32.hpp b/ganmf_amd/csrc/gemm_f32.hpp
--- a/ganmf_amd/csrc/gemm_f32.hpp
+++ b/ganmf_amd/csrc/gemm_f32.hpp
@@ -257,6 +257,7 @@
   const unsigned short* a_planes;
   const unsigned short* b_planes;
   long long a_pstride, b_pstride;
+  const unsigned* b_quads;
   int n_fastest;
   int adam_touch;
 };
diff --git a/ganmf_amd/csrc/lib/abi_core.inc b/ganmf_amd/csrc/lib/abi_core.inc
--- a/ganmf_amd/csrc/lib/abi_core.inc
+++ b/ganmf_amd/csrc/lib/abi_core.inc
@@ -106,6 +106,7 @@
   constexpr int kAsmPrefetchDefault = 1;
 #endif
   h->bf16w = tune_env_int("bf16w", kAsmPrefetchDefault);
+  h->g_planes = tune_env_int("g_planes", kAsmPrefetchDefault) & 1;
   h->wgrad_xb = std::max(0, tune_env_int("wgrad_xb", 16));
   h->wd_lane = std::max(0, tune_env_int("wd_lane", 0));
   h->g_rows_staged = std::max(0, std::min(2, tune_env_int("g_rows_staged", 1)));
@@ -269,7 +270,7 @@
   hipFree(h->test_indptr); hipFree(h->test_indices); hipFree(h->test_gain); hipFree(h->eval_buf);
   hipFree(h->cand_indptr); hipFree(h->cand_indices);
   hipFree(h->test_rating); hipFree(h->eval_w); hipFree(h->eval_rmse); hipFree(h->eval_counts); hipFree(h->eval_grp);
-  hipFree(h->XF_own); hipFree(h->XF_pass); hipFree(h->Ub_pass); hipFree(h->Ub_own); hipFree(h->Ub_sched); hipFree(h->lazy_tab);
+  hipFree(h->wq_e); hipFree(h->wq_d); hipFree(h->XF_own); hipFree(h->XF_pass); hipFree(h->Ub_pass); hipFree(h->Ub_own); hipFree(h->Ub_sched); hipFree(h->lazy_tab);
   for (auto& ch : h->lazy_chunks) hipFree(ch.first);
   if (h->lazy_stage) hipHostFree(h->lazy_stage);
   h->lazy_chunks.clear();
diff --git a/ganmf_amd/csrc/lib/abi_misc.inc b/ganmf_amd/csrc/lib/abi_misc.inc
--- a/ganmf_amd/csrc/lib/abi_misc.inc
+++ b/ganmf_amd/csrc/lib/abi_misc.inc
@@ -134,6 +134,17 @@
     g.a_planes = plA; g.a_pstride = (long long)ea; g.b_planes = plB; g.b_pstride = (long long)eb;
   }
 #endif
+  float* quads = nullptr;
+  if ((tune_env_int("g_planes", 0) & 1) && pl.wide32 && pl.mode == MFMA_BF16X3) {
+    const long long n4 = (long long)br * ldb / 4;
+    TRY(dalloc(&quads, (size_t)n4 * 6));
+    const QuadJob jq{dB, reinterpret_cast<unsigned*>(quads), n4};
+    const int qgrid = (int)std::min<long long>(1024, (n4 + 255) / 256);
+    GANMF_LAUNCH(weight_quads_kernel, dim3(qgrid), dim3(256), 0, (hipStream_t) nullptr, jq, jq, qgrid);
+    HIP_TRY(hipDeviceSynchronize());
+    g.b_quads = reinterpret_cast<const unsigned*>(quads);
+    if (env_int("GANMF_DEBUG_PLAN", 0)) fprintf(stderr, "[ganmf plan] ganmf_gemm_f32: B as weight quads\n");
+  }
   const size_t slab_elems = gemm_slab_elems(pl, g.M, ldc, 1);
   if (slab_elems) TRY(dalloc(&slab, slab_elems));
   unsigned* counters = nullptr;
@@ -156,7 +167,7 @@
   }
   HIP_TRY(hipMemcpy2D(C, (size_t)N * 4, dC, (size_t)ldc * 4, (size_t)N * 4, M, hipMemcpyDeviceToHost));
   if (adam_m) HIP_TRY(hipMemcpy2D(adam_m, (size_t)N * 4, dMom, (size_t)ldc * 4, (size_t)N * 4, M, hipMemcpyDeviceToHost));
-  hipFree(dA); hipFree(dB); hipFree(dC); hipFree(zp); hipFree(plA); hipFree(plB); hipFree(dIds); hipFree(dMom); hipFree(dAlpha);
+  hipFree(dA); hipFree(dB); hipFree(dC); hipFree(zp); hipFree(plA); hipFree(plB); hipFree(quads); hipFree(dIds); hipFree(dMom); hipFree(dAlpha);
   if (slab) hipFree(slab);
   if (counters) hipFree(counters);
   return 0;
diff --git a/ganmf_amd/csrc/lib/abi_train.inc b/ganmf_amd/csrc/lib/abi_train.inc
--- a/ganmf_amd/csrc/lib/abi_train.inc
+++ b/ganmf_amd/csrc/lib/abi_train.inc
@@ -85,7 +85,7 @@
     ganmf_handle* h;
     bool g_opened_early = false;
     ~PassGuard() {
-      h->front_staged = false; h->x_staged = false; h->XF = h->XF_own; h->d_alpha = S_ALPHA_D;
+      h->front_staged = false; h->x_staged = false; h->XF = h->XF_own; h->d_alpha = S_ALPHA_D; h->wq_live = false;
       if (h->lazy_pass) lazy_pass_abort(h);
       if (g_opened_early) {
         GANMF_LAUNCH(restore_g_powers_kernel, dim3(1), dim3(64), 0, h->st, h->scal);
@@ -122,6 +122,7 @@
   if (staged) { h->front_staged = false; h->XF = h->XF_own; h->d_alpha = S_ALPHA_D; }
   idx = 0;
   for (int p = 0; p < g_steps; ++p) {
+    TRY(weight_quads_begin(h));
     if (lazy) TRY(lazy_pass_begin(h, p, per_pass, n, staged && p == 0));
     guard.g_opened_early = false;
     for (int64_t i = 0; i < per_pass; ++i, ++idx) {
@@ -135,7 +136,7 @@
     }
     if (lazy) TRY(lazy_pass_end(h, p, per_pass));
   }
-  h->x_staged = false; h->XF = h->XF_own;
+  h->x_staged = false; h->XF = h->XF_own; h->wq_live = false;
   TRY(dp_join(h));
   TRY(arenas_finish(h, nd, ng));
   if (dist && nd > 0) {
diff --git a/ganmf_amd/csrc/lib/handle.inc b/ganmf_amd/csrc/lib/handle.inc
--- a/ganmf_amd/csrc/lib/handle.inc
+++ b/ganmf_amd/csrc/lib/handle.inc
@@ -156,6 +156,10 @@
   bool skinny_n = true;
   bool pass_stage = true;
   bool pass_buffers_tried = false;
+  int g_planes = 1;
+  float *wq_e = nullptr, *wq_d = nullptr;
+  size_t wq_e_elems = 0, wq_d_elems = 0;
+  bool wq_live = false;
   bool x_staged = false;
   bool front_staged = false;
   int tab_cap = 0;
diff --git a/ganmf_amd/csrc/lib/step_ganmf.inc b/ganmf_amd/csrc/lib/step_ganmf.inc
--- a/ganmf_amd/csrc/lib/step_ganmf.inc
+++ b/ganmf_amd/csrc/lib/step_ganmf.inc
@@ -43,9 +43,55 @@
   size_t free_b = 0, total_b = 0;
   return hipMemGetInfo(&free_b, &total_b) == hipSuccess && bytes <= free_b / 4;
 }
+GemmP g_decode_gemm(const ganmf_handle* h, int nb, float* arena) {
+  GemmP g{};
+  g.A = h->E + (size_t)nb * h->lde; g.lda = h->lde; g.B = h->Wd.p; g.ldb = h->ldN;
+  g.C = h->Dl; g.ldc = h->ldN; g.M = nb; g.N = h->N; g.K = h->e + 1;
+  g.epi.kind = EPI_SUB_AUX_SQ; g.epi.aux = h->XF + (size_t)nb * h->ldN; g.epi.ldaux = h->ldN;
+  g.epi.sq_partials = arena;
+  if (h->wq_live) g.b_quads = reinterpret_cast<const unsigned*>(h->wq_d);
+  return g;
+}
+GemmP g_df_gemm(const ganmf_handle* h, int nb, int b_global, float rsv) {
+  GemmP g{};
+  g.A = h->dE; g.lda = h->lde; g.B = h->We.p; g.ldb = h->lde;
+  g.C = h->dF; g.ldc = h->ldN; g.M = nb; g.N = h->N; g.K = h->e;
+  g.epi.kind = EPI_SUB_SCALED_AUX; g.epi.c = rsv; g.epi.aux = h->Dl; g.epi.ldaux = h->ldN;
+  g.a_scale = grad_scale(h, b_global);
+  if (h->wq_live) g.b_quads = reinterpret_cast<const unsigned*>(h->wq_e);
+  return g;
+}
+bool weight_quads_planned(const ganmf_handle* h) {
+  if (!h->g_planes || h->cfg.model != GANMF_MODEL_GANMF || (h->has_comm && h->cfg.world_size > 1)) return false;
+  const GemmPlan pd = plan_gemm(h, T_GEMM_DEC, g_decode_gemm(h, h->B, h->zero_page), false, true, nullptr);
+  const GemmPlan pf = plan_gemm(h, T_GEMM_DF, g_df_gemm(h, h->B, h->B, 0.f), false, false, nullptr);
+  return pd.wide32 && pd.mode == MFMA_BF16X3 && pf.wide32 && pf.mode == MFMA_BF16X3;
+}
+int weight_quads_begin(ganmf_handle* h) {
+  h->wq_live = false;
+  if (!h->wq_e || !h->wq_d) return 0;
+  TRY(dp_join(h));
+  const QuadJob je{h->We.p, reinterpret_cast<unsigned*>(h->wq_e), (long long)(h->We.padded() / 4)};
+  const QuadJob jd{h->Wd.p, reinterpret_cast<unsigned*>(h->wq_d), (long long)(h->Wd.padded() / 4)};
+  const int be = (int)std::min<long long>(1024, (je.n4 + 255) / 256), bd = (int)std::min<long long>(1024, (jd.n4 + 255) / 256);
+  GANMF_LAUNCH(weight_quads_kernel, dim3(be + bd), dim3(256), 0, h->st, je, jd, be);
+  HIP_TRY(hipGetLastError());
+  if (h->debug_plan) fprintf(stderr, "[ganmf plan] generator pass: weight quads of We_ext (%lld) and Wd_ext (%lld quads) written\n", je.n4, jd.n4);
+  h->wq_live = true;
+  return 0;
+}
+
 void prealloc_pass_buffers(ganmf_handle* h, bool ragged) {
   if (h->pass_buffers_tried) return;
   h->pass_buffers_tried = true;
+  if (weight_quads_planned(h)) {
+    BestEffort guard;
+    const size_t ne = h->We.padded() / 4 * 6, nd = h->Wd.padded() / 4 * 6;
+    if (fits_quarter_of_free((ne + nd) * sizeof(float)) && dalloc(&h->wq_e, ne) == 0) {
+      if (dalloc(&h->wq_d, nd) == 0) { h->wq_e_elems = ne; h->wq_d_elems = nd; }
+      else { hipFree(h->wq_e); h->wq_e = nullptr; h->wq_d = nullptr; }
+    } else h->wq_e = nullptr;
+  }
   const int64_t nfull = h->U / std::max(h->B, 1);
   if (nfull < 4) return;
   BestEffort guard;
@@ -895,14 +941,7 @@
   if (nb > 0) {
     TRY(step_front(h, rows_dev, nb, 1));
     TRY(dp_join(h, PEND_WD));
-    {
-      GemmP g{};
-      g.A = h->E + (size_t)nb * h->lde; g.lda = h->lde; g.B = h->Wd.p; g.ldb = h->ldN;
-      g.C = h->Dl; g.ldc = h->ldN; g.M = nb; g.N = N; g.K = e + 1;
-      g.epi.kind = EPI_SUB_AUX_SQ; g.epi.aux = h->XF + (size_t)nb * h->ldN; g.epi.ldaux = h->ldN;
-      g.epi.sq_partials = arena;
-      TRY(run_gemm(h, T_GEMM_DEC, T_RED_DEC, g, false, true, &sqn, 4.0 * nb * N));
-    }
+    TRY(run_gemm(h, T_GEMM_DEC, T_RED_DEC, g_decode_gemm(h, nb, arena), false, true, &sqn, 4.0 * nb * N));
     const float rsv = (1.0f - alpha) * (2.0f * inv_bn);
     const float cfm = alpha * 2.0f / ((float)b_global * (float)e);
     {
@@ -913,14 +952,7 @@
       g.epi.er = h->E; g.epi.ef = h->E + (size_t)nb * h->lde; g.epi.sq_partials = arena + cap;
       TRY(run_gemm(h, T_GEMM_DE, T_RED_DE, g, false, false, &fmn));
     }
-    {
-      GemmP g{};
-      g.A = h->dE; g.lda = h->lde; g.B = h->We.p; g.ldb = h->lde;
-      g.C = h->dF; g.ldc = h->ldN; g.M = nb; g.N = N; g.K = e;
-      g.epi.kind = EPI_SUB_SCALED_AUX; g.epi.c = rsv; g.epi.aux = h->Dl; g.epi.ldaux = h->ldN;
-      g.a_scale = grad_scale(h, b_global);
-      TRY(run_gemm(h, T_GEMM_DF, T_RED_DF, g, false, false, nullptr, 4.0 * nb * N));
-    }
+    TRY(run_gemm(h, T_GEMM_DF, T_RED_DF, g_df_gemm(h, nb, b_global, rsv), false, false, nullptr, 4.0 * nb * N));
   } else if (!h->lazy_pass) {
     GANMF_LAUNCH(open_step_kernel, dim3(1), dim3(64), 0, h->st, h->scal, 1, h->g_alpha, h->cfg.g_lr);
     HIP_TRY(hipGetLastError());
```
